# dflemin3/approxposterior

Hardware: AMD Instinct MI355X
Metric: GP-predict+acquisition candidates/sec (N_train, D fixed) (higher is better)
Workload: dtype f64

## Files before the change

### approxposterior_amd/_lib.py

```python
import ctypes
import os

_HERE = os.path.dirname(os.path.abspath(__file__))
LIB_PATH = os.path.join(_HERE, "csrc", "libapgp.so")
ABI_VERSION = 8
MAX_DIM = 32
MAX_FANTASY = 32
MAX_DRAWS = 32
MAX_FEATURES = 65536
MAX_REFS = 4096
INTEGRATED_MAX_DIM = 16

UTIL_AGP, UTIL_BAPE, UTIL_JONES, UTIL_NONE = 0, 1, 2, 3
UTIL_NEG_MEAN = 4
NM_MAX_RESTARTS = 4096
NM_MAX_FEV = 1 << 20
NM_STEPS = {1: "reflect", 2: "expand", 3: "reflect_exp", 4: "contract_out", 5: "contract_in",
            6: "shrink_out", 7: "shrink_in", 8: "maxfev"}
GMM_EM, GMM_SCORE, GMM_KMEANS = 0, 1, 2
GMM_MAX_COMP = 16
IMP_BLOCK = 256
IMP_MAX_BLOCKS = 2048


class ApgpError(RuntimeError):
    pass


class KernelStruct(ctypes.Structure):
    _fields_ = [("ndim", ctypes.c_int32), ("lin_order", ctypes.c_int32),
                ("amp", ctypes.c_double), ("diag_add", ctypes.c_double),
                ("inv_metric", ctypes.c_double * MAX_DIM), ("lin_coef", ctypes.c_double)]


class BestStruct(ctypes.Structure):
    _fields_ = [("u", ctypes.c_double), ("index", ctypes.c_int64)]


class NmOptions(ctypes.Structure):
    _fields_ = [("kind", ctypes.c_int32), ("maxiter", ctypes.c_int32), ("maxfev", ctypes.c_int32),
                ("reserved", ctypes.c_int32), ("zeta", ctypes.c_double), ("ybest", ctypes.c_double),
                ("xatol", ctypes.c_double), ("fatol", ctypes.c_double), ("rho", ctypes.c_double),
                ("chi", ctypes.c_double), ("psi", ctypes.c_double), ("sigma", ctypes.c_double)]


class EnsMove(ctypes.Structure):
    _fields_ = [("kind", ctypes.c_int32), ("weight", ctypes.c_double), ("p0", ctypes.c_double), ("p1", ctypes.c_double)]


ENS_MOVE_STRETCH, ENS_MOVE_DE, ENS_MOVE_SNOOKER = 0, 1, 2
ENS_MAX_MOVES = 8
PT_MAX_TEMPS = 64
HMC_MAX_LEAP = 1024
HMC_G_ROWS = (1, 4)
NESTED_MAX_LIVE = 4096
NESTED_MAX_BATCH = 16


class HmcOptions(ctypes.Structure):
    _fields_ = [("eps", ctypes.c_double), ("jitter", ctypes.c_double), ("nleap", ctypes.c_int32),
                ("g_rows", ctypes.c_int32), ("iteration0", ctypes.c_int64), ("mass", ctypes.c_double * MAX_DIM)]

_P = ctypes.c_void_p
_I64 = ctypes.c_int64
_I32 = ctypes.c_int32
_F64 = ctypes.c_double
_KP = ctypes.POINTER(KernelStruct)

SIGNATURES = {
    "apgp_abi_version": (ctypes.c_int, []),
    "apgp_last_error": (ctypes.c_char_p, []),
    "apgp_npad": (_I64, [_I64]),
    "apgp_packed_linv_len": (_I64, [_I64]),
    "apgp_acquire_work_len": (_I64, [_I64, _I64]),
    "apgp_packed_train_len": (_I64, [_I64, _I32]),
    "apgp_trtri_work_len": (_I64, [_I64]),
    "apgp_grad_work_len": (_I64, [_I64]),
    "apgp_gram": (ctypes.c_int, [_P, _I64, _KP, _P, _I64, _P]),
    "apgp_kernel_cross": (ctypes.c_int, [_P, _I64, _P, _I64, _KP, _P, _I64, _P]),
    "apgp_potrf": (ctypes.c_int, [_P, _I64, _I64, _P, _F64, _P, _P, _P]),
    "apgp_logdet": (ctypes.c_int, [_P, _I64, _I64, _P, _P]),
    "apgp_fit_summary": (ctypes.c_int, [_P, _I64, _I64, _P, _P, _P, _P]),
    "apgp_nll_eval": (ctypes.c_int, [_P, _I64, _KP, _P, _F64, _P, _P, _P, _P, _P, _P]),
    "apgp_potrf_mode": (ctypes.c_int, [ctypes.c_int]),
    "apgp_potrf_fallbacks": (_I64, []),
    "apgp_potrf_backoff_skips": (_I64, []),
    "apgp_nll_side_batches": (_I64, []),
    "apgp_nll_eval_batch": (ctypes.c_int, [_P, _I64, _I64, _P, _P, _P, _P, _P, _P, _P, _P, _P]),
    "apgp_trsv": (ctypes.c_int, [_P, _I64, _I64, _P, _F64, ctypes.c_int, _P, _P, _P]),
    "apgp_trsv_ex": (ctypes.c_int, [_P, _I64, _I64, _P, _F64, ctypes.c_int, _P, _P, ctypes.c_int, _P]),
    "apgp_trsv_mode": (ctypes.c_int, [ctypes.c_int]),
    "apgp_append_diag": (ctypes.c_int, [_P, _P, _F64, _P, _I64, _P]),
    "apgp_winv_apply_work_len": (_I64, [_I64]),
    "apgp_winv_apply": (ctypes.c_int, [_P, _I64, _I64, _P, _F64, ctypes.c_int, _P, _P, _P, _P]),
    "apgp_trtri_pack": (ctypes.c_int, [_P, _I64, _I64, _P, _P, _P, _P]),
    "apgp_pack_train": (ctypes.c_int, [_P, _P, _I64, _KP, _P, _P]),
    "apgp_acquire": (ctypes.c_int, [_P, _I64, _I64, _P, _P, _I64, _KP, _F64, _I32,
                                    ctypes.POINTER(_F64), ctypes.POINTER(_F64), _P,
                                    _F64, _F64, _P, _P, _P, _P, _P, _P]),
    "apgp_packed_lsolve_len": (_I64, [_I64]),
    "apgp_pack_lsolve": (ctypes.c_int, [_P, _I64, _I64, _P, _P]),
    "apgp_acquire_solve": (ctypes.c_int, [_P, _I64, _I64, _P, _P, _I64, _KP, _F64, _I32,
                                          ctypes.POINTER(_F64), ctypes.POINTER(_F64), _P,
                                          _F64, _F64, _P, _P, _P, _P, _P, _P]),
    "apgp_set_sweep_prune": (ctypes.c_int, [ctypes.c_int]),
    "apgp_get_sweep_prune": (ctypes.c_int, []),
    "apgp_set_seed_rowsplit": (ctypes.c_int, [ctypes.c_int]),
    "apgp_get_seed_rowsplit": (ctypes.c_int, []),
    "apgp_set_seed_park": (ctypes.c_int, [ctypes.c_int]),
    "apgp_get_seed_park": (ctypes.c_int, []),
    "apgp_set_seed_first": (ctypes.c_int, [ctypes.c_int]),
    "apgp_get_seed_first": (ctypes.c_int, []),
    "apgp_set_seed_parts": (ctypes.c_int, [ctypes.c_int]),
    "apgp_get_seed_parts": (ctypes.c_int, []),
    "apgp_sweep_prune_counts_offset": (_I64, [_I64, _I64]),
    "apgp_sweep_prune_select": (ctypes.c_int, [_P, _I64, _P, _P, _F64, _P, _P]),
    "apgp_prune_bounds": (ctypes.c_int, [_P, _I64, _P, _I64, _KP, _F64, _I32, ctypes.POINTER(_F64), ctypes.POINTER(_F64),
                                         _P, _F64, _F64, ctypes.c_int, _P, _P]),
    "apgp_sweep_prune_seeds": (ctypes.c_int, [_P, _I64, _P, _P, _P]),
    "apgp_prune_rows_len": (_I64, [_I64, _I32]),
    "apgp_pack_prune_rows": (ctypes.c_int, [_P, _I64, _KP, _P, _P]),
    "apgp_acquire_rows": (ctypes.c_int, [_P, _I64, _I64, _P, _P, _I64, _KP, _F64, _I32,
                                         ctypes.POINTER(_F64), ctypes.POINTER(_F64), _P,
                                         _F64, _F64, _P, _P, _P, _P, _P, _P, _P]),
    "apgp_acquire_solve_rows": (ctypes.c_int, [_P, _I64, _I64, _P, _P, _I64, _KP, _F64, _I32,
                                               ctypes.POINTER(_F64), ctypes.POINTER(_F64), _P,
                                               _F64, _F64, _P, _P, _P, _P, _P, _P, _P]),
    "apgp_prune_bounds_rows": (ctypes.c_int, [_P, _I64, _P, _I64, _KP, _F64, _I32, ctypes.POINTER(_F64),
                                              ctypes.POINTER(_F64), _P, _F64, _F64, ctypes.c_int, _P, _P, _P]),
    "apgp_acquire_fantasy_work_len": (_I64, [_I64]),
    "apgp_acquire_fantasy": (ctypes.c_int, [_P, _I64, _I64, _P, _I64, _KP, _P, _I64, _I32, _P, _I64,
                                            _P, _P, _P, _I32, ctypes.POINTER(_F64), ctypes.POINTER(_F64), _P,
                                            _F64, _F64, _P, _P, _P, _P]),
    "apgp_path_draws_work_len": (_I64, [_I64, _I32]),
    "apgp_path_draws_mode": (ctypes.c_int, [ctypes.c_int]),
    "apgp_path_draws": (ctypes.c_int, [_P, _I64, _I64, _P, _I64, _KP, _F64, _P, _P, _P, _P, _P, _I32, _I32,
                                       ctypes.POINTER(_F64), ctypes.POINTER(_F64), _P, _P, _P, _P, _P]),
    "apgp_integrated_work_len": (_I64, [_I64, _I32]),
    "apgp_integrated_mode": (ctypes.c_int, [ctypes.c_int]),
    "apgp_acquire_integrated": (ctypes.c_int, [_P, _I64, _I64, _P, _I64, _KP, _P, _I32, _P, _P, _P,
                                               ctypes.POINTER(_F64), ctypes.POINTER(_F64), _P, _P, _I64, _P, _P, _P, _P]),
    "apgp_predict1_work_len": (_I64, [_I64]),
    "apgp_predict1_host": (ctypes.c_int, [_P, _P, _I64, _KP, _F64, _P, _I64, _P, _I64, _P, _P, _P]),
    "apgp_nm_search_work_len": (_I64, [_I64, _I64]),
    "apgp_nm_search": (ctypes.c_int, [_P, _I64, _P, _I64, _KP, _F64, _P, _I64, _P, _I64,
                                      ctypes.POINTER(_F64), ctypes.POINTER(_F64), ctypes.POINTER(NmOptions),
                                      _P, _P, _P, _P, _P, _P, _P]),
    "apgp_predict_grad_work_len": (_I64, [_I64, _I64]),
    "apgp_predict_grad": (ctypes.c_int, [_P, _I64, _P, _I64, _KP, _F64, _P, _I64, _P, _I64, _I32,
                                         ctypes.POINTER(_F64), ctypes.POINTER(_F64), _F64, _F64,
                                         _P, _P, _P, _P, _P, _P, _P, _P]),
    "apgp_predict_mean": (ctypes.c_int, [_P, _I64, _P, _I64, _KP, _F64, _P, _P]),
    "apgp_predict_mean_host": (ctypes.c_int, [_P, _I64, _P, _I64, _KP, _F64, _P, _P, _P]),
    "apgp_ensemble_sample": (ctypes.c_int, [_P, _I64, _KP, _F64, ctypes.POINTER(_F64), ctypes.POINTER(_F64),
                                            _I32, _I32, _I64, _F64, ctypes.c_uint64, _P, _P, _P, _P, _P, _P]),
    "apgp_ensemble_sample_ex": (ctypes.c_int, [_P, _I64, _KP, _F64, ctypes.POINTER(_F64), ctypes.POINTER(_F64),
                                               _I32, _I32, _I64, _F64, ctypes.c_uint64, _P, _P, _P, _P, _P, ctypes.c_int, _P]),
    "apgp_ensemble_sample_moves": (ctypes.c_int, [_P, _I64, _KP, _F64, ctypes.POINTER(_F64), ctypes.POINTER(_F64),
                                                  _I32, _I32, _I64, _F64, ctypes.c_uint64, _P, _P, _P, _P, _P, ctypes.c_int,
                                                  ctypes.POINTER(EnsMove), _I32, _P]),
    "apgp_ensemble_mode": (ctypes.c_int, [ctypes.c_int]),
    "apgp_tempered_work_len": (_I64, [_I32, _I32, _I32, _I32]),
    "apgp_tempered_sample": (ctypes.c_int, [_P, _I64, _KP, _F64, ctypes.POINTER(_F64), ctypes.POINTER(_F64), _I32, _I32, _I32,
                                            ctypes.POINTER(_F64), _I64, _I64, ctypes.c_uint64, _P, _P, _P, _I32, _P, _P, _P,
                                            _P, _P, ctypes.POINTER(EnsMove), _I32, _P, _P]),
    "apgp_hmc_sample": (ctypes.c_int, [_P, _I64, _KP, _F64, ctypes.POINTER(_F64), ctypes.POINTER(_F64), _I32, _I64,
                                       ctypes.POINTER(HmcOptions), ctypes.c_uint64, _P, _P, _P, _P, _P, _P, _P, _P, _P, _P, _P]),
    "apgp_hmc_rule": (ctypes.c_int, [_I32, _I64, _I32]),
    "apgp_nested_work_len": (_I64, [_I32, _I32, _I32]),
    "apgp_nested_xlds": (ctypes.c_int, [_I64, _I32]),
    "apgp_nested_sample": (ctypes.c_int, [_P, _I64, _KP, _F64, ctypes.POINTER(_F64), ctypes.POINTER(_F64), _I32, _I32, _I32,
                                          _I32, _F64, _F64, _F64, _I32, ctypes.c_uint64, _P, _P, _P, _P, _P, _P, _P, _P, _P]),
    "apgp_box_candidates": (ctypes.c_int, [_P, _I64, _I32, ctypes.POINTER(_F64), ctypes.POINTER(_F64), ctypes.c_uint64,
                                           _I64, _P]),
    "apgp_prior_candidates": (ctypes.c_int, [_P, _I64, _I32, _P, _P, _P, ctypes.c_uint64, _I64, _P]),
    "apgp_prior_lnprior": (ctypes.c_int, [_P, _I64, _I32, _P, _P, _P, _P, _P]),
    "apgp_release_scratch": (ctypes.c_int, [_P]),
    "apgp_kinv_solve_work_len": (_I64, [_I64]),
    "apgp_kinv_solve": (ctypes.c_int, [_P, _I64, _I64, _P, _P, _P]),
    "apgp_grad_loglik": (ctypes.c_int, [_P, _P, _P, _I64, _I64, _KP, _P, _P, _P]),
    "apgp_gmm_params_len": (_I64, [_I32, _I32]),
    "apgp_gmm_stats_len": (_I64, [_I32, _I32]),
    "apgp_gmm_pass": (ctypes.c_int, [_P, _I64, _I32, _I32, _P, _I32, _P, _P, _P, _P]),
    "apgp_mix_params_len": (_I64, [_I32, _I32]),
    "apgp_mix_candidates": (ctypes.c_int, [_P, _P, _I64, _I32, _I32, _P, ctypes.c_uint64, _I64, _P]),
    "apgp_sobol_direction": (_I32, [_I32, _I32]),
    "apgp_sobol_box_candidates": (ctypes.c_int, [_P, _I64, _I32, ctypes.POINTER(_F64), ctypes.POINTER(_F64), ctypes.c_uint64,
                                                 _I32, _I32, _I64, _P]),
    "apgp_sobol_prior_candidates": (ctypes.c_int, [_P, _I64, _I32, _P, _P, _P, ctypes.c_uint64, _I32, _I32, _I64, _P]),
    "apgp_sobol_mix_candidates": (ctypes.c_int, [_P, _P, _I64, _I32, _I32, _P, ctypes.c_uint64, _I32, _I32, _I64, _P]),
    "apgp_importance_stats_len": (_I64, [_I32]),
    "apgp_importance_work_len": (_I64, [_I64]),
    "apgp_importance_pass": (ctypes.c_int, [_P, _I64, _P, _P, _I64, _KP, _F64, ctypes.POINTER(_F64), ctypes.POINTER(_F64),
                                            _P, _P, _P, _P, _P]),
    "apgp_path_importance_work_len": (_I64, [_I64, _I32]),
    "apgp_path_importance": (ctypes.c_int, [_P, _I64, _P, _P, _I64, _KP, _F64, _P, _P, _P, _P, _P, _I32, _I32,
                                            ctypes.POINTER(_F64), ctypes.POINTER(_F64), _P, _P, _P, _P, _P]),
    "apgp_autocorr_work_len": (_I64, [_I64, _I64, _I32]),
    "apgp_autocorr_block": (ctypes.c_int, [_P, _I64, _I64, _I32, _I64, _I64, _I64, _I64, _I32, _P, _P, _P]),
}

_lib = None


def load():
    global _lib
    if _lib is not None:
        return _lib
    if not os.path.exists(LIB_PATH):
        raise ApgpError(
            "libapgp.so not found at %s -- build it with "
            "`make -C approxposterior_amd/csrc` (or __graft_entry__.build()). "
            "There is no CPU fallback." % LIB_PATH)
    import torch
    lib = ctypes.CDLL(LIB_PATH)
    for name, (res, args) in SIGNATURES.items():
        fn = getattr(lib, name)
        fn.restype = res
        fn.argtypes = args
    v = lib.apgp_abi_version()
    if v != ABI_VERSION:
        raise ApgpError("libapgp.so ABI %d != expected %d" % (v, ABI_VERSION))
    _lib = lib
    return lib


def check(status, what):
    if status != 0:
        msg = load().apgp_last_error()
        raise ApgpError("%s failed (%d): %s" % (what, status, msg.decode() if msg else ""))
```

### approxposterior_amd/csrc/prune_mm32.h

```cpp
#pragma once
#include <utility>

#ifndef PMM_G
#define PMM_G 4
#endif
#define PMM_ROWS 128
typedef float f32x16 __attribute__((ext_vector_type(16)));
typedef __bf16 bf16x8 __attribute__((ext_vector_type(8)));

struct PmmSlot { int e, pp, qp; };

template <int DPAD>
struct PmmShape {
    static constexpr int K = DPAD + 2;
    static constexpr int NS = 5 * DPAD + 4;
    static constexpr int NIS = (NS + 15) / 16, NI = NIS + 1;
    static constexpr int PITCH = 16 * NI + 8;
    static_assert(K <= 16, "the big products stand in one instruction");
    static constexpr int XPIECES = PMM_ROWS * PITCH / 8, APIECES = PMM_ROWS / 4, PIECES = XPIECES + APIECES;
    static constexpr PmmSlot slot(int i) {
        if (i >= 16 * NIS) return i - 16 * NIS < K ? PmmSlot{i - 16 * NIS, 0, 0} : PmmSlot{-1, 0, 0};
        if (i < 2 * DPAD) return PmmSlot{2 + i / 2, (i & 1) ? 2 : 0, (i & 1) ? 0 : 2};
        i -= 2 * DPAD;
        if (i < 2) return i == 0 ? PmmSlot{0, 2, 0} : PmmSlot{1, 0, 2};
        i -= 2;
        if (i < DPAD) return PmmSlot{2 + i, 1, 1};
        i -= DPAD;
        if (i < 2 * DPAD) return PmmSlot{2 + i / 2, (i & 1) ? 1 : 0, (i & 1) ? 0 : 1};
        i -= 2 * DPAD;
        if (i < 2) return i == 0 ? PmmSlot{0, 1, 0} : PmmSlot{1, 0, 1};
        return PmmSlot{-1, 0, 0};
    }
};

template <int PART>
__device__ __forceinline__ float pmm_part(float p) {
    const float h = (float)(__bf16)p;
    if constexpr (PART == 0) return h;
    const float r = p - h, m = (float)(__bf16)r;
    return PART == 1 ? m : r - m;
}

template <int DPAD, int SIDE, int I>
__device__ __forceinline__ __bf16 pmm_slot_value(const float (&entry)[DPAD + 2]) {
    constexpr PmmSlot s = PmmShape<DPAD>::slot(I);
    if constexpr (s.e < 0) return (__bf16)0.0f;
    else return (__bf16)pmm_part<SIDE ? s.qp : s.pp>(entry[s.e]);
}
template <int DPAD, int SIDE, int F, int... J>
__device__ __forceinline__ bf16x8 pmm_frag(const float (&entry)[DPAD + 2], std::integer_sequence<int, J...>) {
    return bf16x8{pmm_slot_value<DPAD, SIDE, 8 * F + J>(entry)...};
}
template <int DPAD, int... F>
__device__ __forceinline__ void pmm_store_row(__bf16* dst, const float (&entry)[DPAD + 2],
                                              std::integer_sequence<int, F...>) {
    ((*(bf16x8*)(dst + 8 * F) = pmm_frag<DPAD, 0, F>(entry, std::make_integer_sequence<int, 8>{})), ...);
}
template <int DPAD, int... T>
__device__ __forceinline__ void pmm_cand(bf16x8 (&qop)[PmmShape<DPAD>::NI], const float (&entry)[DPAD + 2], int h,
                                         std::integer_sequence<int, T...>) {
    ((qop[T] = h ? pmm_frag<DPAD, 1, 2 * T + 1>(entry, std::make_integer_sequence<int, 8>{})
                 : pmm_frag<DPAD, 1, 2 * T>(entry, std::make_integer_sequence<int, 8>{})), ...);
}

template <int DPAD>
__global__ __launch_bounds__(PR_THREADS) void pmm_pack_rows_kernel(const double* xs, long long n, unsigned char* rows) {
    using SH = PmmShape<DPAD>;
    constexpr int XS = DPAD + 2, PITCH = SH::PITCH;
    const double kappa = PR32_KAPPA;
    __shared__ double wmax[PR_THREADS / 64], wsal[PR_THREADS / 64];
    const int tid = threadIdx.x, lane = tid & 63, w = tid >> 6, h = lane >> 5, l32 = lane & 31;
    double cen[DPAD];
#pragma unroll
    for (int d = 0; d < DPAD; ++d) cen[d] = xs[d];
    double sal = 0.0, bm2 = 0.0;
    const long long ntile = (n + PMM_ROWS - 1) / PMM_ROWS;
    const int srow = w * 32 + l32;
    if (h == 0) {
        for (long long ti = 0; ti < ntile; ++ti) {
            const f64x2* src = (const f64x2*)(xs + (ti * PMM_ROWS + srow) * XS);
            f64x2 pre[XS / 2];
#pragma unroll
            for (int i = 0; i < XS / 2; ++i) pre[i] = src[i];
            const bool in = ti * PMM_ROWS + srow < n;
            unsigned char* tile = rows + 16 + ti * (16ll * SH::PIECES);
            __bf16* xrow = (__bf16*)tile + srow * PITCH;
            float pe[DPAD + 2];
            double n2 = 0.0, b2 = 0.0;
#pragma unroll
            for (int d = 0; d < DPAD; ++d) {
                const double x = (d & 1) ? pre[d >> 1].y : pre[d >> 1].x;
                const double df = x - cen[d];
                b2 = fma(df, df, b2);
                const float bf = in ? (float)(df * kappa) : 0.0f;
                n2 = fma((double)bf, (double)bf, n2);
                pe[d + 2] = 2.0f * bf;
            }
            if (in) { bm2 = fmax(bm2, b2); sal += fabs(pre[DPAD / 2].x); }
            pe[0] = -(float)n2;
            pe[1] = 1.0f;
            pmm_store_row<DPAD>(xrow, pe, std::make_integer_sequence<int, 2 * SH::NI>{});
            ((float*)(tile + 16 * SH::XPIECES))[srow] = in ? (float)pre[DPAD / 2].x : 0.0f;
            *(bf16x8*)(xrow + 16 * SH::NI) = bf16x8{(__bf16)0.0f, (__bf16)0.0f, (__bf16)0.0f, (__bf16)0.0f,
                                                    (__bf16)0.0f, (__bf16)0.0f, (__bf16)0.0f, (__bf16)0.0f};
        }
    }
    for (int o = 32; o > 0; o >>= 1) { bm2 = fmax(bm2, __shfl_xor(bm2, o)); sal += __shfl_xor(sal, o); }
    if (lane == 0) { wmax[w] = bm2; wsal[w] = sal; }
    __syncthreads();
    if (tid == 0) {
        sal = 0.0;
#pragma unroll
        for (int i = 0; i < PR_THREADS / 64; ++i) { bm2 = fmax(bm2, wmax[i]); sal += wsal[i]; }
        ((double*)rows)[0] = bm2;
        ((double*)rows)[1] = sal;
    }
}

template <int DPAD, bool PRE = false>
__global__ __launch_bounds__(PR_THREADS, PMM_G <= 4 ? 2 : 1) void prune_bound_mm32_kernel(PruneArgs a) {
    using SH = PmmShape<DPAD>;
    constexpr int XS = DPAD + 2;
    constexpr int K = SH::K, NI = SH::NI, PITCH = SH::PITCH, G = PMM_G;
    static_assert(PMM_G % 2 == 0 && PMM_ROWS == 32 * (PR_THREADS / 64), "one 32-row tile staged per wavefront");
    const double kappa = PR32_KAPPA;
    static_assert(SH::XPIECES * 8 == PMM_ROWS * PITCH && SH::APIECES * 4 == PMM_ROWS, "the stream's tile is the LDS image");
    constexpr int NB = PRE ? 2 : 1;
    __shared__ __attribute__((aligned(16))) __bf16 xt[NB * PMM_ROWS * PITCH];
    __shared__ __attribute__((aligned(16))) float at[NB * PMM_ROWS];
    __shared__ double wmax[PR_THREADS / 64], wsal[PR_THREADS / 64];
    const int tid = threadIdx.x, lane = tid & 63, w = tid >> 6, h = lane >> 5, l32 = lane & 31;
    const long long blk0 = ((long long)blockIdx.x * (PR_THREADS / 64) + w) * (G / 2);
    double cen[DPAD], c2 = 0.0;
#pragma unroll
    for (int d = 0; d < DPAD; ++d) { cen[d] = a.xs[d]; c2 = fma(cen[d], cen[d], c2); }
    const double cn = sqrt(c2);
    bf16x8 qop[G][NI];
    double an[G];
    bool adm[G];
#pragma unroll
    for (int g = 0; g < G; ++g) {
        const long long blk = blk0 + (g >> 1);
        const long long row = blk * SW_CAND + (g & 1) * 32 + l32;
        const bool live = blk < a.ncb && row < a.m;
        bool ok = live, has_nan = false;
        double a2 = 0.0, ce[DPAD];
#pragma unroll
        for (int d = 0; d < DPAD; ++d) {
            double v = 0.0;
            if (live && d < a.ndim) {
                v = a.T[row * a.ndim + d];
                if (a.has_box && !(v >= a.lo[d] && v <= a.hi[d])) ok = false;
                if (v != v) has_nan = true;
            }
            ce[d] = v * a.sc[d] - cen[d];
            a2 = fma(ce[d], ce[d], a2);
        }
        if (live && a.mask && a.mask[row] == 0) ok = false;
        adm[g] = ok && !has_nan;
        an[g] = sqrt(a2);
        const bool use = live && !has_nan && a2 <= 0x1p100;
        float q[K];
        double n2 = 0.0;
#pragma unroll
        for (int d = 0; d < DPAD; ++d) {
            q[d + 2] = use ? (float)(ce[d] * kappa) : 0.0f;
            n2 = fma((double)q[d + 2], (double)q[d + 2], n2);
        }
        q[0] = 1.0f;
        q[1] = -(float)n2;
        pmm_cand<DPAD>(qop[g], q, h, std::make_integer_sequence<int, NI>{});
    }
    double accm[G], accs[G], sal = 0.0, bm2 = 0.0;
#pragma unroll
    for (int g = 0; g < G; ++g) { accm[g] = 0.0; accs[g] = 0.0; }
    const long long ntile = (a.n + PMM_ROWS - 1) / PMM_ROWS;
    auto consume = [&](int xo, int ao) {
#pragma unroll 1
        for (int rt = 0; rt < PMM_ROWS / 32; ++rt) {
            const __bf16* xr = xt + xo + (rt * 32 + l32) * PITCH + 8 * h;
            bf16x8 pop[NI];
#pragma unroll
            for (int t = 0; t < NI; ++t) pop[t] = *(const bf16x8*)(xr + 16 * t);
            float al[16];
#pragma unroll
            for (int q = 0; q < 4; ++q) *(f32x4*)(al + 4 * q) = *(const f32x4*)(at + ao + rt * 32 + 8 * q + 4 * h);
            auto product = [&](int g) {
                f32x16 c = {0.0f, 0.0f, 0.0f, 0.0f, 0.0f, 0.0f, 0.0f, 0.0f, 0.0f, 0.0f, 0.0f, 0.0f, 0.0f, 0.0f, 0.0f, 0.0f};
#pragma unroll
                for (int t = 0; t < NI; ++t) c = __builtin_amdgcn_mfma_f32_32x32x16_bf16(pop[t], qop[g][t], c, 0, 0, 0);
                return c;
            };
            f32x16 cur = product(0);
#pragma unroll
            for (int g = 0; g < G; ++g) {
                f32x16 nxt = cur;
                if (g + 1 < G) nxt = product(g + 1);
                float ps = 0.0f, pS = 0.0f;
#pragma unroll
                for (int r = 0; r < 16; ++r) {
                    const float k = __builtin_amdgcn_exp2f(cur[r]);
                    ps = fmaf(k, al[r], ps);
                    pS = fmaf(k, fabsf(al[r]), pS);
                }
                accm[g] += (double)ps;
                accs[g] += (double)pS;
                cur = nxt;
            }
        }
    };
    if constexpr (PRE) {
        typedef unsigned int u32x4 __attribute__((ext_vector_type(4)));
        constexpr int NPC = SH::PIECES, NL = (NPC + PR_THREADS - 1) / PR_THREADS;
        const u32x4* img = (const u32x4*)((const unsigned char*)a.prune_rows + 16);
        u32x4 pre[NL];
        auto fetch = [&](long long ti) {
            const u32x4* src = img + ti * NPC;
#pragma unroll
            for (int j = 0; j < NL; ++j) {
                const int e = tid + j * PR_THREADS;
                pre[j] = src[e < NPC ? e : NPC - 1];
            }
        };
        auto put = [&](int b) {
            u32x4* xd = (u32x4*)(xt + b * PMM_ROWS * PITCH);
            u32x4* ad = (u32x4*)(at + b * PMM_ROWS);
#pragma unroll
            for (int j = 0; j < NL; ++j) {
                const int e = tid + j * PR_THREADS;
                if ((j + 1) * PR_THREADS <= SH::XPIECES || e < SH::XPIECES) xd[e] = pre[j];
                else if (e < NPC) ad[e - SH::XPIECES] = pre[j];
            }
        };
        fetch(0);
        put(0);
        __syncthreads();
        for (long long ti = 0; ti < ntile; ++ti) {
            const int b = (int)(ti & 1);
            fetch(ti + 1 < ntile ? ti + 1 : ntile - 1);
            consume(b * PMM_ROWS * PITCH, b * PMM_ROWS);
            put(b ^ 1);
            __syncthreads();
        }
        bm2 = ((const double*)a.prune_rows)[0];
        sal = ((const double*)a.prune_rows)[1];
    } else {
        const bool stager = h == 0;
        const int srow = w * 32 + l32;
        f64x2 pre[XS / 2];
        auto fetch = [&](long long ti) {
            const f64x2* src = (const f64x2*)(a.xs + (ti * PMM_ROWS + srow) * XS);
#pragma unroll
            for (int i = 0; i < XS / 2; ++i) pre[i] = stager ? src[i] : f64x2{0.0, 0.0};
        };
        fetch(0);
        for (long long ti = 0; ti < ntile; ++ti) {
            if (stager) {
                const bool in = ti * PMM_ROWS + srow < a.n;
                float pe[K];
                double n2 = 0.0, b2 = 0.0;
#pragma unroll
                for (int d = 0; d < DPAD; ++d) {
                    const double x = (d & 1) ? pre[d >> 1].y : pre[d >> 1].x;
                    const double df = x - cen[d];
                    b2 = fma(df, df, b2);
                    const float bf = in ? (float)(df * kappa) : 0.0f;
                    n2 = fma((double)bf, (double)bf, n2);
                    pe[d + 2] = 2.0f * bf;
                }
                if (in) { bm2 = fmax(bm2, b2); sal += fabs(pre[DPAD / 2].x); }
                pe[0] = -(float)n2;
                pe[1] = 1.0f;
                pmm_store_row<DPAD>(xt + srow * PITCH, pe, std::make_integer_sequence<int, 2 * NI>{});
                at[srow] = in ? (float)pre[DPAD / 2].x : 0.0f;
            }
            __syncthreads();
            if (ti + 1 < ntile) fetch(ti + 1);
            consume(0, 0);
            __syncthreads();
        }
        for (int o = 32; o > 0; o >>= 1) { bm2 = fmax(bm2, __shfl_xor(bm2, o)); sal += __shfl_xor(sal, o); }
        if (lane == 0) { wmax[w] = bm2; wsal[w] = sal; }
        __syncthreads();
        sal = 0.0;
#pragma unroll
        for (int i = 0; i < PR_THREADS / 64; ++i) { bm2 = fmax(bm2, wmax[i]); sal += wsal[i]; }
    }
    const double bn = sqrt(bm2);
    const double u32 = 0x1p-24, eps = 0x1p-53;
    const double sa = sal * (1.0 + 0x1p-16);
    double bb = INFINITY, bbe = INFINITY;
#pragma unroll
    for (int g = 0; g < G; ++g) {
        const double sm = accm[g] + __shfl_xor(accm[g], 32);
        const double s32 = (accs[g] + __shfl_xor(accs[g], 32)) * (1.0 + 0x1p-16);
        const double ktt = a.amp;
        const double mu = fma(a.amp, sm, a.mean);
        double b = util_value(a.kind, mu, ktt, a.zeta, a.ybest);
        const double ab = an[g] + bn;
        const double eta = (DPAD + 10.0) * u32 * ab * ab + 2.5 * eps * ab * (cn + an[g]) + 24.0 * u32;
        double e32 = a.amp * (expm1(eta) * (1.0 + 0x1p-20) * s32 + 0x1p-120 * (sa + (double)a.n));
        if (!(eta <= 0x1p-8)) e32 = INFINITY;
        bbe = fmin(bbe, pr_block_min<32>(b, adm[g]));
        bb = fmin(bb, pr_block_min<32>(b - pr_slack<DPAD>(a, 2.0 * e32, a.amp * sa, mu, ktt, b), adm[g]));
        if (g & 1) {
            const long long blk = blk0 + (g >> 1);
            if (lane == 0 && blk < a.ncb) pr_store_block<true>(a, blk, bb, bbe);
            bb = INFINITY; bbe = INFINITY;
        }
    }
}
```

### approxposterior_amd/csrc/sweep.hip

```cpp
#include "apgp_common.h"
#include "mma16.h"
#include "scratch.h"
#include "util_value.h"
#include <mutex>
#include <stdlib.h>
#include <string.h>

#define SW_ROWS APGP_ROW_BLOCK
#define SW_KC APGP_K_CHUNK
#define SW_TILE (SW_ROWS * SW_KC)
#define SW_CAND 64
#define SW_GRID 256
#define SW_BCH 1024
typedef unsigned int u32x4 __attribute__((ext_vector_type(4)));
#ifndef SW_KAUX
#define SW_KAUX 0
#endif

struct SweepArgs {
    const double* T;
    const double* linv;
    const double* xs;
    const unsigned char* mask;
    double* mu;
// ... 1001 lines not shown
        qr[1] = fma(v0.y, v0.y, qr[1]);
        qr[2] = fma(v1.x, v1.x, qr[2]);
        qr[3] = fma(v1.y, v1.y, qr[3]);
    }
    double qtot = 0.0;
    qtot += s2_q_gather(qr, lane);
    if ((lane >> 4) == 0) a.sp_q[((long long)pos * SW_CAND + w * 16 + (lane & 15)) * a.nrb + jb] = qtot;
}

#define SP_NCH 4
template <int DPAD>
__global__ __launch_bounds__(256) void seed_park_kernel(SweepArgs a) {
#pragma clang fp contract(off)
    constexpr int XS = DPAD + 2;
    constexpr int NKK = SW_KC / 4;
    __shared__ double Etab[APGP_EXP_TAB_N];
    const int ngrp = a.ncache / SP_NCH;
    const int pos = S2W_P0(a.split) + (int)blockIdx.x / ngrp, kc0 = (int)blockIdx.x % ngrp * SP_NCH;
    const long long cnt = *a.blk_count;
    if (cnt <= a.list_lo || cnt > a.list_hi || pos >= cnt) return;
    if (s2_wave_skip(a, a.nrb, S2W_P0(a.split), pos)) return;
    apgp_exp_tab_load(Etab);
    __syncthreads();
    const int ht = threadIdx.x, lane = ht & 63, hw = ht >> 6;
    const int cl = lane & 15, kq = lane >> 4;
    const long long blk = a.blk_list[pos];
    const long long crow = blk * SW_CAND + hw * 16 + cl;
    const bool inb = blk < a.blk_end && crow < a.m;
    double tv[DPAD], tt[DPAD];
#pragma unroll
    for (int d = 0; d < DPAD; ++d) {
        double v = 0.0;
        if (inb && d < a.ndim) v = a.T[crow * a.ndim + d];
        tv[d] = v;
        tt[d] = v * a.sc[d];
    }
    for (int kc = kc0; kc < kc0 + SP_NCH; ++kc) {
        const double* Xb = a.xs + (long long)kc * (SW_KC * XS);
        double s2[NKK], s3[NKK];
#pragma unroll
        for (int kk = 0; kk < NKK; ++kk) { s2[kk] = 0.0; s3[kk] = 0.0; }
#pragma unroll
        for (int d = 0; d < DPAD; d += 2)
#pragma unroll
            for (int kk = 0; kk < NKK; ++kk) {
                const f64x2 xa = *(const f64x2*)(Xb + (kk * 4 + kq) * XS + d);
                double df0, df1;
                if (kc == 0) { df0 = fma(tv[d], a.sc[d], -xa.x); df1 = fma(tv[d + 1], a.sc[d + 1], -xa.y); }
                else { df0 = tt[d] - xa.x; df1 = tt[d + 1] - xa.y; }
                s2[kk] = fma(df0, df0, s2[kk]);
                s3[kk] = fma(df1, df1, s3[kk]);
            }
        double ex[NKK], bfv[NKK];
#pragma unroll
        for (int kk = 0; kk < NKK; ++kk) ex[kk] = -(s2[kk] + s3[kk]);
        apgp_exp4(ex, bfv, Etab);
#pragma unroll
        for (int kk = 0; kk < NKK; ++kk) bfv[kk] = bfv[kk] * a.amp;
        f64x2* dst = (f64x2*)(a.kcache + ((long long)pos * a.ncache + kc) * SW_BCH) + ht;
        f64x2 q0, q1;
        q0.x = bfv[0]; q0.y = bfv[1]; q1.x = bfv[2]; q1.y = bfv[3];
        dst[0] = q0; dst[256] = q1;
    }
}


static inline int s2_nrb(int64_t n) { return (int)((n + S2_ROWS - 1) / S2_ROWS); }
static inline long long s2_ncache(int64_t n) { return (long long)S2_CPB * (s2_nrb(n) - 1); }

template <int DPAD>
static constexpr size_t s2_lds_bytes() {
    return (3 * S2_TILE + 2 * 4 * 256 + 3 * ((SW_KC * (DPAD + 2) * 8 + 1023) / 1024 * 128) + APGP_EXP_TAB_N + SW_CAND + 8 +
            4 * APGP_MAX_DIM) * sizeof(double);
}

template <int DPAD>
static int s2_prepare_device() {
    static ApgpLdsOnce once;
    int dev = 0;
    if (hipGetDevice(&dev) != hipSuccess || dev < 0 || dev >= 64) {
        apgp_set_error("apgp_acquire: hipGetDevice failed");
        return -2;
    }
    return apgp_raise_lds(once, "apgp_acquire", dev, (int)s2_lds_bytes<DPAD>(),
                          {(const void*)sweep2_kernel<DPAD, false, 0>, (const void*)sweep2_kernel<DPAD, true, 0>,
                           (const void*)sweep2_kernel<DPAD, false, 1>, (const void*)sweep2_kernel<DPAD, true, 1>,
                           (const void*)sweep2_kernel<DPAD, false, 2>, (const void*)sweep2_kernel<DPAD, true, 2>,
                           (const void*)sweep2_kernel<DPAD, false, 0, true>, (const void*)sweep2_kernel<DPAD, true, 0, true>,
                           (const void*)sweep2_kernel<DPAD, false, 1, true>, (const void*)sweep2_kernel<DPAD, true, 1, true>,
                           (const void*)sweep2_kernel<DPAD, false, 2, true>, (const void*)sweep2_kernel<DPAD, true, 2, true>,
                           (const void*)sweep2_kernel<DPAD, false, 0, true, true>, (const void*)sweep2_kernel<DPAD, true, 0, true, true>});
}

template <int DPAD, bool LIST>
static void s2_launch(const SweepArgs& a, hipStream_t s, bool solve, unsigned grid) {
    const size_t lds = s2_lds_bytes<DPAD>();
    if (solve && a.nrb <= S2_STATIC_DIAG_NRB) {
        if (a.lin_coef != 0.0)
            hipLaunchKernelGGL((sweep2_kernel<DPAD, true, 2, LIST>), dim3(grid), dim3(S2_THREADS), lds, s, a);
        else
            hipLaunchKernelGGL((sweep2_kernel<DPAD, false, 2, LIST>), dim3(grid), dim3(S2_THREADS), lds, s, a);
    } else if (solve) {
        if (a.lin_coef != 0.0)
            hipLaunchKernelGGL((sweep2_kernel<DPAD, true, 1, LIST>), dim3(grid), dim3(S2_THREADS), lds, s, a);
        else
            hipLaunchKernelGGL((sweep2_kernel<DPAD, false, 1, LIST>), dim3(grid), dim3(S2_THREADS), lds, s, a);
    } else if (a.lin_coef != 0.0)
        hipLaunchKernelGGL((sweep2_kernel<DPAD, true, 0, LIST>), dim3(grid), dim3(S2_THREADS), lds, s, a);
    else
        hipLaunchKernelGGL((sweep2_kernel<DPAD, false, 0, LIST>), dim3(grid), dim3(S2_THREADS), lds, s, a);
}

template <int DPAD>
static int launch_sweep(const SweepArgs& a0, hipStream_t s, bool solve) {
    const int rc = s2_prepare_device<DPAD>();
    if (rc != 0) return rc;
    SweepArgs a = a0;
    const long long ncb = (a.m + SW_CAND - 1) / SW_CAND;
    const int nrb2 = s2_nrb(a.n);
    a.nrb = nrb2;
    long long rest = ncb % SW_GRID;
    if (solve || nrb2 < 2 || rest > S2_SPLIT_MAX || a.sp_q == NULL) rest = 0;
    const long long full = ncb - rest;
    if (full > 0) {
        a.blk_begin = 0; a.blk_end = full; a.split = 0;
        s2_launch<DPAD, false>(a, s, solve, (unsigned)(full < SW_GRID ? full : SW_GRID));
    }
    if (rest > 0) {
        a.blk_begin = full; a.blk_end = ncb; a.split = 1;
        a.ncache = 0;
        a.kslot_bytes = SW_BCH * 8;
        s2_launch<DPAD, false>(a, s, solve, (unsigned)(rest * nrb2));
        hipLaunchKernelGGL(sweep_finish_kernel, dim3((unsigned)rest), dim3(64), 0, s, a);
    }
    return 0;
}

static int g_seed_rowsplit = -1;

extern "C" int apgp_set_seed_rowsplit(int v) {
    return __atomic_exchange_n(&g_seed_rowsplit, v < 0 ? -1 : v, __ATOMIC_RELAXED);
}

extern "C" int apgp_get_seed_rowsplit(void) { return __atomic_load_n(&g_seed_rowsplit, __ATOMIC_RELAXED); }

static int g_seed_park = 1;

extern "C" int apgp_set_seed_park(int v) { return __atomic_exchange_n(&g_seed_park, v != 0 ? 1 : 0, __ATOMIC_RELAXED); }

extern "C" int apgp_get_seed_park(void) { return __atomic_load_n(&g_seed_park, __ATOMIC_RELAXED); }

#define S2_SEED_FIRST 4
static int g_seed_first = -1;

extern "C" int apgp_set_seed_first(int v) {
    return __atomic_exchange_n(&g_seed_first, v < 1 ? -1 : (v > 16 ? 16 : v), __ATOMIC_RELAXED);
}

extern "C" int apgp_get_seed_first(void) { return __atomic_load_n(&g_seed_first, __ATOMIC_RELAXED); }

static int g_seed_parts = -1;

extern "C" int apgp_set_seed_parts(int v) {
    return __atomic_exchange_n(&g_seed_parts, (v == 8 || v == 4 || v == 2 || v == 1) ? v : -1, __ATOMIC_RELAXED);
}

extern "C" int apgp_get_seed_parts(void) { return __atomic_load_n(&g_seed_parts, __ATOMIC_RELAXED); }

static long long seed_launch_cost(int nrb, int cap, int n, int j0, int lg, bool parked) {
    static const int gen[4] = {S2P_WHOLE_GEN, S2P_HALF_GEN, S2P_PAIR2_GEN, S2P_PAIR1_GEN};
    static const int park[4] = {S2P_WHOLE_PARK, S2P_HALF_PARK, S2P_PAIR2_PARK, S2P_PAIR1_PARK};
    long long load[SW_GRID] = {0};
    const int nitem = s2_nitems(nrb, j0, n, lg);
    long long last = 0;
    for (int i = 0; i < nitem; ++i) {
        int jb = 0, h = -1;
        s2_row_item(i, nrb, j0, n, lg, jb, h);
        const int kind = h >= 0 ? lg : (n - S2_ROWS * jb <= S2_ROWS / 2 ? 1 : 0);
        const int nkc = s2_nkc_of(jb, n), nre = S2_CPB * jb < nkc ? S2_CPB * jb : nkc;
        const long long c = parked ? (long long)gen[kind] * (nkc - nre) + (long long)park[kind] * nre
                                   : (long long)s2_part_cost(kind) * nkc;
        for (int k = 0; k < cap; ++k) {
            int best = 0;
            for (int q = 1; q < SW_GRID; ++q)
                if (load[q] < load[best]) best = q;
            load[best] += c;
            if (load[best] > last) last = load[best];
        }
    }
    return last;
}

struct SeedPlan { int j0, lg; long long cost; };
static SeedPlan seed_plan(int nrb, int cap, int n, bool parked) {
    const int v = apgp_get_seed_rowsplit(), fp = apgp_get_seed_parts();
    const int flg = fp == 8 ? 0 : fp == 4 ? 1 : fp == 2 ? 2 : fp == 1 ? 3 : -1;
    struct Memo { int nrb, cap, n, parked, v, flg; SeedPlan plan; };
    static std::mutex mu;
    static Memo memo[8];
    static int nmemo = 0, next = 0;
    std::lock_guard<std::mutex> g(mu);
    for (int i = 0; i < nmemo; ++i) {
        const Memo& e = memo[i];
        if (e.nrb == nrb && e.cap == cap && e.n == n && e.parked == (int)parked && e.v == v && e.flg == flg) return e.plan;
    }
    SeedPlan best = {nrb, 1, 0};
    long long best_c = -1;
    for (int lg = 1; lg <= (parked ? 2 : 1); ++lg) {
        if (flg >= 0 && lg != 1) continue;
        const int l = flg >= 0 ? flg : lg;
        for (int j0 : {nrb, nrb / 2, 0}) {
            if (v >= 0 && j0 != nrb) continue;
            const int j = v >= 0 ? (v < nrb ? v : nrb) : j0;
            if (lg > 1 && j == nrb) continue;
            const long long c = seed_launch_cost(nrb, cap, n, j, l, parked);
            if (best_c < 0 || c < best_c) { best = {j, l, c}; best_c = c; }
        }
    }
    memo[next] = {nrb, cap, n, (int)parked, v, flg, best};
    next = (next + 1) % 8;
    if (nmemo < 8) ++nmemo;
    return best;
}

template <int DPAD>
static void launch_sweep_list(const SweepArgs& a0, hipStream_t s, bool solve, const long long* list,
                              const long long* count, long long max_count, long long cap, bool rowsplit = false) {
    SweepArgs a = a0;
    const int nrb2 = s2_nrb(a.n);
    a.nrb = nrb2;
    a.blk_list = list; a.blk_count = count;
    a.blk_begin = 0; a.blk_end = (a.m + SW_CAND - 1) / SW_CAND;
    const bool can_split = !solve && nrb2 >= 2 && a.sp_q != NULL;
    if (cap > max_count) cap = max_count;
    if (can_split) {
        SweepArgs b = a;
        b.split = 1; b.ncache = 0; b.kslot_bytes = SW_BCH * 8;
        b.list_lo = 0; b.list_hi = cap;
        const bool parked = rowsplit && b.lin_coef == 0.0 && apgp_get_seed_park() != 0;
        int first = (int)cap;
        if (rowsplit && b.lin_coef == 0.0) {
            const int v = apgp_get_seed_first();
            first = v > 0 ? v : S2_SEED_FIRST;
            if (first > (int)cap) first = (int)cap;
            if (v <= 0 && first < (int)cap &&
                seed_plan(nrb2, (int)cap, b.n, true).cost - seed_plan(nrb2, first, b.n, true).cost <= S2P_WAVE2)
                first = (int)cap;
        }
        for (int wave = 0; wave < (first < (int)cap ? 2 : 1); ++wave) {
            const int p0 = wave ? first : 0, p1 = wave ? (int)cap : first, nw = p1 - p0;
            const SeedPlan plan = rowsplit ? seed_plan(nrb2, nw, b.n, parked) : SeedPlan{nrb2, 0, 0};
            const int nitem = s2_nitems(nrb2, plan.j0, b.n, plan.lg);
            b.split = S2W_WORD(plan.j0, plan.lg, p0, p1);
            if (parked) {
                b.ncache = (int)s2_ncache(b.n);
                b.kslot_bytes = (unsigned)(b.ncache * (SW_BCH * 8));
                hipLaunchKernelGGL(seed_park_kernel<DPAD>, dim3((unsigned)(nw * (b.ncache / SP_NCH))), dim3(256), 0, s, b);
            }
            if (nitem > nrb2 || parked || first < (int)cap) {
                const size_t lds = s2_lds_bytes<DPAD>();
                const unsigned grid = (unsigned)(nw * nitem);
                if (b.lin_coef != 0.0)
                    hipLaunchKernelGGL((sweep2_kernel<DPAD, true, 0, true, true>), dim3(grid), dim3(S2_THREADS), lds, s, b);
                else
                    hipLaunchKernelGGL((sweep2_kernel<DPAD, false, 0, true, true>), dim3(grid), dim3(S2_THREADS), lds, s, b);
                if (nitem > nrb2) hipLaunchKernelGGL(sweep_fold_kernel, dim3((unsigned)(nw * nrb2)), dim3(256), 0, s, b);
            } else {
                b.split = 1;
                s2_launch<DPAD, true>(b, s, solve, (unsigned)(cap * nrb2));
            }
            SweepArgs f = b;
            f.split = rowsplit ? (S2W_WORD(plan.j0, plan.lg, p0, p1) | S2W_SEED) : 1;
            hipLaunchKernelGGL(sweep_finish_kernel, dim3((unsigned)nw), dim3(64), 0, s, f);
        }
    }
    if (!can_split || max_count > cap) {
        a.split = 0;
        a.list_lo = can_split ? cap : 0; a.list_hi = APGP_MAX_M;
        s2_launch<DPAD, true>(a, s, solve, (unsigned)(max_count < SW_GRID ? max_count : SW_GRID));
    }
}

#define PR_THREADS 256
#define PR_CPT 2
#define PR_ROWS 128
#define PR_SEED 16
static inline int64_t pr_min_m(int64_t n) { return n >= 4096 ? 16384 : 65536; }

struct PruneArgs {
    const double* T;
    const double* xs;
    const unsigned char* mask;
    double* bmin;
    double* part_u;
    long long* part_i;
    long long m, ncb, n;
    int ndim, kind, has_box, lin_order;
    double mean, amp, lin_coef, zeta, ybest;
    double sc[APGP_MAX_DIM], lw[APGP_MAX_DIM], lo[APGP_MAX_DIM], hi[APGP_MAX_DIM];
    const long long* blk_list;
    const long long* blk_count;
    double* est;
    const void* prune_rows;
};

template <int DPAD>
__device__ __forceinline__ double pr_slack(const PruneArgs& a, double base, double S, double mu, double ktt, double b) {
    const double eps = 0x1p-53;
    double slack = base + 2.0 * (4.0 * (double)(a.n + 16) + 8.0 * DPAD + 32.0) * eps * S +
                   64.0 * eps * (1.0 + fabs(mu) + fabs(a.ybest) + fabs(a.zeta) + ktt + fabs(b));
    if (a.kind == APGP_UTIL_BAPE) slack += 16.0 * eps / (1.0 - exp(0.0 - ktt));
    return slack;
}

template <int W>
__device__ __forceinline__ double pr_block_min(double b, bool adm) {
    if (!(b == b)) b = -INFINITY;
    if (!adm) b = INFINITY;
    for (int o = W / 2; o > 0; o >>= 1) b = fmin(b, __shfl_xor(b, o));
    return b;
}

__device__ __forceinline__ void pr_prefill(const PruneArgs& a, long long blk) {
    if (a.part_u) {
        a.part_u[blk] = INFINITY;
        a.part_i[blk] = -1;
    }
}

template <bool PREFILL>
__device__ __forceinline__ void pr_store_block(const PruneArgs& a, long long blk, double b, double be) {
    a.bmin[blk] = b;
    if (a.est) a.est[blk] = be;
    if (PREFILL) pr_prefill(a, blk);
}

template <int DPAD, bool LIST = false>
__global__ __launch_bounds__(PR_THREADS) void prune_bound_kernel(PruneArgs a) {
    constexpr int XS = DPAD + 2;
    constexpr int PIECES = PR_ROWS * XS / 2;
    __shared__ double etab[APGP_EXP_TAB_N];
    __shared__ __attribute__((aligned(16))) double tile[PR_ROWS * XS];
    long long lst_count = 0;
    if (LIST) {
        lst_count = *a.blk_count;
        if ((long long)blockIdx.x * (PR_THREADS / 64) * PR_CPT >= lst_count) return;
    }
    apgp_exp_tab_load(etab);
    const int tid = threadIdx.x, lane = tid & 63, w = tid >> 6;
    const long long blk0 = ((long long)blockIdx.x * (PR_THREADS / 64) + w) * PR_CPT;
    long long blk[PR_CPT];
#pragma unroll
    for (int c = 0; c < PR_CPT; ++c) blk[c] = !LIST ? blk0 + c : (blk0 + c < lst_count ? a.blk_list[blk0 + c] : a.ncb);
    double tt[PR_CPT][DPAD], ktt[PR_CPT];
    bool adm[PR_CPT];
#pragma unroll
    for (int c = 0; c < PR_CPT; ++c) {
        const long long row = blk[c] * SW_CAND + lane;
        const bool live = blk[c] < a.ncb && row < a.m;
        bool ok = live, has_nan = false;
        double ktl = a.lin_order == 0 ? (double)a.ndim : 0.0;
#pragma unroll
        for (int d = 0; d < DPAD; ++d) {
            double v = 0.0;
            if (live && d < a.ndim) {
                v = a.T[row * a.ndim + d];
                if (a.has_box && !(v >= a.lo[d] && v <= a.hi[d])) ok = false;
                if (v != v) has_nan = true;
            }
            tt[c][d] = v * a.sc[d];
            if (a.lin_coef != 0.0 && a.lin_order > 0) {
                const double p = v * v;
                double q = p;
                for (int e = 1; e < a.lin_order; ++e) q *= p;
                ktl += q;
            }
        }
        if (live && a.mask && a.mask[row] == 0) ok = false;
        adm[c] = ok && !has_nan;
        ktt[c] = a.lin_coef != 0.0 ? fma(a.lin_coef, ktl, a.amp) : a.amp;
    }
    double acc[PR_CPT][4], sab[PR_CPT][4];
#pragma unroll
    for (int c = 0; c < PR_CPT; ++c)
#pragma unroll
        for (int q = 0; q < 4; ++q) { acc[c][q] = 0.0; sab[c][q] = 0.0; }
    const long long ntile = (a.n + PR_ROWS - 1) / PR_ROWS;
    for (long long ti = 0; ti < ntile; ++ti) {
        __syncthreads();
        const double* src = a.xs + ti * (PR_ROWS * XS);
        for (int e = tid; e < PIECES; e += PR_THREADS) *((f64x2*)tile + e) = *((const f64x2*)src + e);
        __syncthreads();
        for (int r = 0; r < PR_ROWS; r += 4) {
#pragma unroll
            for (int c = 0; c < PR_CPT; ++c) {
                double ex[4], kv[4];
#pragma unroll
                for (int q = 0; q < 4; ++q) {
                    const double* xr = tile + (r + q) * XS;
                    double s2 = 0.0, s3 = 0.0;
#pragma unroll
                    for (int d = 0; d < DPAD; d += 2) {
                        const double df0 = tt[c][d] - xr[d];
                        const double df1 = tt[c][d + 1] - xr[d + 1];
                        s2 = fma(df0, df0, s2);
                        s3 = fma(df1, df1, s3);
                    }
                    ex[q] = -(s2 + s3);
                }
                apgp_exp4(ex, kv, etab);
#pragma unroll
                for (int q = 0; q < 4; ++q) {
                    const double* xr = tile + (r + q) * XS;
                    double k = kv[q] * a.amp, kabs = k;
                    if (a.lin_coef != 0.0) {
                        double ls = a.lin_order == 0 ? (double)a.ndim : 0.0, la = ls;
                        if (a.lin_order > 0)
#pragma unroll
                            for (int d = 0; d < DPAD; d += 2) {
                                const double p0 = tt[c][d] * xr[d] * a.lw[d], p1 = tt[c][d + 1] * xr[d + 1] * a.lw[d + 1];
                                double q0 = p0, q1 = p1;
                                for (int e = 1; e < a.lin_order; ++e) { q0 *= p0; q1 *= p1; }
                                ls += q0 + q1;
                                la += fabs(q0) + fabs(q1);
                            }
                        kabs = fma(a.lin_coef, la, k);
                        k = fma(a.lin_coef, ls, k);
                    }
                    acc[c][q] = fma(k, xr[DPAD], acc[c][q]);
                    sab[c][q] = fma(kabs, fabs(xr[DPAD]), sab[c][q]);
                }
            }
        }
    }
#pragma unroll
    for (int c = 0; c < PR_CPT; ++c) {
        const double mu = ((acc[c][0] + acc[c][1]) + (acc[c][2] + acc[c][3])) + a.mean;
        const double S = (sab[c][0] + sab[c][1]) + (sab[c][2] + sab[c][3]);
        double b = util_value(a.kind, mu, ktt[c], a.zeta, a.ybest);
        const double eps = 0x1p-53;
        double slack = 2.0 * (4.0 * (double)(a.n + 16) + 8.0 * DPAD + 32.0) * eps * S +
                       64.0 * eps * (1.0 + fabs(mu) + fabs(a.ybest) + fabs(a.zeta) + ktt[c] + fabs(b));
        if (a.kind == APGP_UTIL_BAPE) slack += 16.0 * eps / (1.0 - exp(0.0 - ktt[c]));
        b -= slack;
        b = pr_block_min<64>(b, adm[c]);
        if (lane == 0 && blk[c] < a.ncb) {
            if (LIST) {
                a.bmin[blk[c]] = fmax(a.bmin[blk[c]], b);
            } else {
                a.bmin[blk[c]] = b;
                if (a.part_u) {
                    a.part_u[blk[c]] = INFINITY;
                    a.part_i[blk[c]] = -1;
                }
            }
        }
    }
}

#define PR32_CPT 4
#define PR32_ROWS 128
#define PR32_FLUSH 8
typedef float f32x2 __attribute__((ext_vector_type(2)));
typedef float f32x4 __attribute__((ext_vector_type(4)));
static constexpr double PR32_KAPPA = 0x1.337cc2183b050p+0;
static constexpr int pr32_cpt(int dpad) { return dpad <= 8 ? PR32_CPT : dpad == 16 ? 2 : 1; }

template <int DPAD, bool REDO = false>
__global__ __launch_bounds__(PR_THREADS) void prune_bound32_kernel(PruneArgs a) {
    constexpr int XS = DPAD + 2;
    constexpr int PIECES = PR32_ROWS * XS / 2;
    constexpr int NP = (PIECES + PR_THREADS - 1) / PR_THREADS;
    constexpr int HD = DPAD / 2;
    constexpr int CPT = pr32_cpt(DPAD);
    if (REDO) {
        const long long wg0 = (long long)blockIdx.x * (PR_THREADS / 64) * CPT;
        bool any = false;
        for (int i = 0; i < (PR_THREADS / 64) * CPT; ++i) any |= wg0 + i < a.ncb && a.bmin[wg0 + i] == -INFINITY;
        if (!any) return;
    }
    const double kappa = PR32_KAPPA;
    __shared__ __attribute__((aligned(16))) float xt[PR32_ROWS * DPAD];
    __shared__ __attribute__((aligned(16))) float at[PR32_ROWS];
    __shared__ double cen[DPAD];
    const int tid = threadIdx.x, lane = tid & 63, w = tid >> 6;
    if (tid < DPAD) cen[tid] = a.xs[tid];
    const long long blk0 = ((long long)blockIdx.x * (PR_THREADS / 64) + w) * CPT;
    f32x2 tt[CPT][HD];
    double ktt[CPT], an[CPT];
    bool adm[CPT], redo[CPT];
#pragma unroll
    for (int c = 0; c < CPT; ++c) {
        const long long row = (blk0 + c) * SW_CAND + lane;
        const bool live = blk0 + c < a.ncb && row < a.m;
        redo[c] = !REDO || (blk0 + c < a.ncb && a.bmin[blk0 + c] == -INFINITY);
        bool ok = live, has_nan = false;
        double a2 = 0.0;
#pragma unroll
        for (int d = 0; d < DPAD; ++d) {
            double v = 0.0;
            if (live && d < a.ndim) {
                v = a.T[row * a.ndim + d];
                if (a.has_box && !(v >= a.lo[d] && v <= a.hi[d])) ok = false;
                if (v != v) has_nan = true;
            }
            const double ce = v * a.sc[d] - a.xs[d];
            a2 = fma(ce, ce, a2);
            tt[c][d >> 1][d & 1] = (float)(ce * kappa);
        }
        if (live && a.mask && a.mask[row] == 0) ok = false;
        adm[c] = ok && !has_nan;
        ktt[c] = a.amp;
        an[c] = sqrt(a2);
    }
    double acc[CPT], sal = 0.0, c2 = 0.0;
#pragma unroll
    for (int c = 0; c < CPT; ++c) acc[c] = 0.0;
#pragma unroll
    for (int d = 0; d < DPAD; ++d) c2 = fma(a.xs[d], a.xs[d], c2);
    const double cn = sqrt(c2);
    const long long ntile = (a.n + PR32_ROWS - 1) / PR32_ROWS;
    f64x2 pre[NP];
    auto fetch = [&](long long ti) {
        const f64x2* src = (const f64x2*)(a.xs + ti * (PR32_ROWS * XS));
#pragma unroll
        for (int i = 0; i < NP; ++i) {
            const int e = tid + i * PR_THREADS;
            pre[i] = e < PIECES ? src[e] : f64x2{0.0, 0.0};
        }
    };
    fetch(0);
    __syncthreads();
    for (long long ti = 0; ti < ntile; ++ti) {
#pragma unroll
        for (int i = 0; i < NP; ++i) {
            const int e = tid + i * PR_THREADS;
            if (e < PIECES) {
                const int r = (2 * e) / XS, col = (2 * e) % XS;
                if (col < DPAD)
                    *(f32x2*)(xt + r * DPAD + col) = f32x2{(float)((pre[i].x - cen[col]) * kappa),
                                                           (float)((pre[i].y - cen[col + 1]) * kappa)};
                else
                    at[r] = (float)pre[i].x;
            }
        }
        __syncthreads();
        if (ti + 1 < ntile) fetch(ti + 1);
        for (int r0 = 0; r0 < PR32_ROWS; r0 += PR32_FLUSH) {
            float al[PR32_FLUSH], ps[CPT], pa = 0.0f;
#pragma unroll
            for (int q = 0; q < PR32_FLUSH; q += 4) *(f32x4*)(al + q) = *(const f32x4*)(at + r0 + q);
#pragma unroll
            for (int c = 0; c < CPT; ++c) ps[c] = 0.0f;
#pragma unroll
            for (int q = 0; q < PR32_FLUSH; ++q) {
                f32x2 xr[HD];
                if constexpr (DPAD >= 4) {
#pragma unroll
                    for (int h = 0; h < HD; h += 2) {
                        const f32x4 v = *(const f32x4*)(xt + (r0 + q) * DPAD + 2 * h);
                        xr[h] = f32x2{v.x, v.y};
                        xr[h + 1] = f32x2{v.z, v.w};
                    }
                } else {
                    xr[0] = *(const f32x2*)(xt + (r0 + q) * DPAD);
                }
                pa += fabsf(al[q]);
#pragma unroll
                for (int c = 0; c < CPT; ++c) {
                    f32x2 s2 = f32x2{0.0f, 0.0f};
#pragma unroll
                    for (int h = 0; h < HD; ++h) {
                        const f32x2 df = tt[c][h] - xr[h];
                        s2 = __builtin_elementwise_fma(df, df, s2);
                    }
                    const float k = __builtin_amdgcn_exp2f(-(s2.x + s2.y));
                    ps[c] = fmaf(k, al[q], ps[c]);
                }
            }
#pragma unroll
            for (int c = 0; c < CPT; ++c) acc[c] += (double)ps[c];
            sal += (double)pa;
        }
        __syncthreads();
    }
    const double u32 = 0x1p-24, eps = 0x1p-53;
    const double sa = sal * (1.0 + 0x1p-16);
#pragma unroll
    for (int c = 0; c < CPT; ++c) {
        const double mu = fma(a.amp, acc[c], a.mean);
        double b = util_value(a.kind, mu, ktt[c], a.zeta, a.ybest);
        double e32 = a.amp * ((u32 * (4.0 * an[c] + 0.5 * DPAD + 18.0) + 2.0 * eps * (cn + an[c])) * sa +
                              0x1p-120 * (sa + (double)a.n));
        if (!(u32 * (8.0 * an[c] + DPAD + 8.0) + eps * (cn + an[c]) <= 0x1p-8)) e32 = INFINITY;
        const double be = pr_block_min<64>(b, adm[c]);
        b = pr_block_min<64>(b - pr_slack<DPAD>(a, 2.0 * e32, a.amp * sa, mu, ktt[c], b), adm[c]);
        if (lane == 0 && blk0 + c < a.ncb && redo[c]) pr_store_block<!REDO>(a, blk0 + c, b, be);
    }
}

#include "prune_mm32.h"

__device__ __forceinline__ bool pr_less(double v, long long i, double w, long long j) { return v < w || (v == w && i < j); }

#define PR_NONE 0x7fffffffffffffffll

template <int E>
__device__ __forceinline__ void pr_wave_select(double (&lv)[E], long long (&li)[E], double& mv, long long& mi) {
    const int lane = threadIdx.x & 63;
    mv = INFINITY; mi = PR_NONE;
    for (int r = 0; r < PR_SEED; ++r) {
        double hv = lv[0];
        long long hi = li[0];
#pragma unroll
        for (int j = 1; j < E; ++j)
            if (pr_less(lv[j], li[j], hv, hi)) { hv = lv[j]; hi = li[j]; }
        double bv = hv;
        long long bi = hi;
        for (int o = 32; o > 0; o >>= 1) {
            const double ov = __shfl_xor(bv, o);
            const long long oi = __shfl_xor(bi, o);
            if (pr_less(ov, oi, bv, bi)) { bv = ov; bi = oi; }
        }
        if (bi == PR_NONE) break;
        if (lane == r) { mv = bv; mi = bi; }
        if (hi == bi) {
#pragma unroll
            for (int j = 0; j < E; ++j)
                if (li[j] == bi) { lv[j] = INFINITY; li[j] = PR_NONE; }
        }
    }
}

#define PR_SEED_E 16
#define PR_LIST (16 * PR_SEED)

__global__ __launch_bounds__(1024) void prune_seed_kernel(const double* bmin, long long ncb, long long* seeds,
                                                          long long* counts) {
    __shared__ double sv[PR_LIST], wv[16];
    __shared__ long long si[PR_LIST], wi[16];
    __shared__ int cnt, nsel;
    const int tid = threadIdx.x, lane = tid & 63, w = tid >> 6;
    if (tid == 0) { cnt = 0; nsel = 0; }
    double tv = INFINITY;
    long long ti = PR_NONE;
    for (long long base = 0; base < ncb; base += PR_SEED_E * 1024) {
        double lv[PR_SEED_E], hv = INFINITY;
        long long hp = PR_NONE;
#pragma unroll
        for (int j = 0; j < PR_SEED_E; ++j) {
            const long long p = base + tid + 1024 * j;
            const double v = p < ncb ? bmin[p] : INFINITY;
            lv[j] = v < INFINITY ? v : INFINITY;
            if (lv[j] < hv) { hv = lv[j]; hp = p; }
        }
        for (int o = 32; o > 0; o >>= 1) {
            const double ov = __shfl_xor(hv, o);
            const long long op = __shfl_xor(hp, o);
            if (pr_less(ov, op, hv, hp)) { hv = ov; hp = op; }
        }
        __syncthreads();
        if (lane == 0) { wv[w] = hv; wi[w] = hp; }
        __syncthreads();
        double cv = wv[0];
        long long ci = wi[0];
#pragma unroll
        for (int i = 1; i < 16; ++i)
            if (pr_less(cv, ci, wv[i], wi[i])) { cv = wv[i]; ci = wi[i]; }
        if (pr_less(cv, ci, tv, ti)) { tv = cv; ti = ci; }
#pragma unroll
        for (int j = 0; j < PR_SEED_E; ++j) {
            const long long p = base + tid + 1024 * j;
            if (lv[j] < INFINITY && !pr_less(tv, ti, lv[j], p)) {
                const int slot = atomicAdd(&cnt, 1);
                if (slot < PR_LIST) { sv[slot] = lv[j]; si[slot] = p; }
            }
        }
    }
    __syncthreads();
    int n = cnt;
    if (n > PR_LIST) {
        double lv[PR_SEED_E + 1], mv = INFINITY;
        long long li[PR_SEED_E + 1], mi = PR_NONE;
        for (long long base = 0; base < ncb; base += PR_SEED_E * 1024) {
            const double qv = __shfl(mv, PR_SEED - 1);
            const long long qi = __shfl(mi, PR_SEED - 1);
            bool any = false;
#pragma unroll
            for (int j = 0; j < PR_SEED_E; ++j) {
                const long long p = base + tid + 1024 * j;
                const double v = p < ncb ? bmin[p] : INFINITY;
                const bool in = v < INFINITY && pr_less(v, p, qv, qi);
                lv[j] = in ? v : INFINITY; li[j] = in ? p : PR_NONE;
                any |= in;
            }
            if (!__any(any)) continue;
            lv[PR_SEED_E] = mv; li[PR_SEED_E] = mi;
            pr_wave_select(lv, li, mv, mi);
        }
        if (lane < PR_SEED) { sv[w * PR_SEED + lane] = mv; si[w * PR_SEED + lane] = mi; }
        n = PR_LIST;
        __syncthreads();
    }
    if (tid < n && si[tid] != PR_NONE) {
        const double v = sv[tid];
        const long long p = si[tid];
        int rank = 0;
        for (int e = 0; e < n; ++e) rank += pr_less(sv[e], si[e], v, p) ? 1 : 0;
        if (rank < PR_SEED) { seeds[rank] = p; atomicAdd(&nsel, 1); }
    }
    __syncthreads();
    if (tid == 0) { counts[0] = nsel; counts[1] = 0; counts[3] = 0; }
}

__global__ __launch_bounds__(1024) void prune_select_kernel(const double* bmin, long long ncb, const long long* seeds,
                                                            long long* counts, const double* part_u, double tau_in,
                                                            long long* list, long long* count2) {
    __shared__ long long sd[PR_SEED];
    __shared__ long long cnt[1024];
    const int t = threadIdx.x;
    const int ns = (int)counts[0];
    if (t < PR_SEED) sd[t] = t < ns ? seeds[t] : -1;
    __syncthreads();
    double tau = tau_in;
    if (part_u) {
        tau = INFINITY;
        for (int i = 0; i < ns; ++i) tau = fmin(tau, part_u[sd[i]]);
    }
    auto keep = [&](long long p) {
        const double v = bmin[p];
        if (!(v < INFINITY && v <= tau)) return false;
        for (int i = 0; i < ns; ++i)
            if (sd[i] == p) return false;
        return true;
    };
    const long long per = (ncb + 1023) / 1024;
    const long long p0 = (long long)t * per, p1 = p0 + per < ncb ? p0 + per : ncb;
    long long c = 0;
    for (long long p = p0; p < p1; ++p) c += keep(p) ? 1 : 0;
    cnt[t] = c;
    __syncthreads();
    for (int o = 1; o < 1024; o <<= 1) {
        const long long add = t >= o ? cnt[t - o] : 0;
        __syncthreads();
        cnt[t] += add;
        __syncthreads();
    }
    long long pos = cnt[t] - c;
    for (long long p = p0; p < p1; ++p)
        if (keep(p)) list[pos++] = p;
    if (t == 1023) {
        counts[1] = cnt[1023];
        counts[2] = __double_as_longlong(tau);
        if (count2) *count2 = cnt[1023];
    }
}

static int g_sweep_prune = 1;

extern "C" int apgp_set_sweep_prune(int v) {
    const int old = __atomic_exchange_n(&g_sweep_prune, v < 0 ? 0 : v, __ATOMIC_RELAXED);
    return old;
}

extern "C" int apgp_get_sweep_prune(void) { return __atomic_load_n(&g_sweep_prune, __ATOMIC_RELAXED); }

static inline long long pr_ncb(int64_t m) { return (m + SW_CAND - 1) / SW_CAND; }
static inline long long s2_work_len(int64_t m, int64_t n) {
    const long long ncb = pr_ncb(m);
    const long long slots = ncb < SW_GRID ? ncb : SW_GRID;
    return 2 * ncb + slots * s2_ncache(n) * SW_BCH + 2 * (long long)S2_SPLIT_MAX * SW_CAND * s2_nrb(n);
}

extern "C" int64_t apgp_sweep_prune_counts_offset(int64_t m, int64_t n) {
    if (m < 1 || n < 1 || m > APGP_MAX_M || n > APGP_MAX_N) return -1;
    return s2_work_len(m, n) + 2 * pr_ncb(m) + PR_SEED;
}

extern "C" int apgp_sweep_prune_select(const double* bmin, int64_t ncb, const int64_t* seeds, int64_t* counts,
                                       double tau, int64_t* list, void* stream) {
    APGP_CHECK_ARG(bmin && seeds && counts && list, "null pointer");
    APGP_CHECK_ARG(ncb >= 1 && ncb <= APGP_MAX_M / SW_CAND, "ncb >= 1 required");
    hipLaunchKernelGGL(prune_select_kernel, dim3(1), dim3(1024), 0, (hipStream_t)stream, bmin, (long long)ncb,
                       (const long long*)seeds, (long long*)counts, (const double*)NULL, tau, (long long*)list,
                       (long long*)NULL);
    APGP_CHECK_LAUNCH();
    return 0;
}

template <class Kern>
static PruneArgs pr_args(const double* T, int64_t m, const double* xs, int64_t n, const uint8_t* mask, const Kern& kern,
                         double mean, int32_t kind, const double* lo, const double* hi, double zeta, double ybest,
                         double* bmin, double* part_u, long long* part_i, const void* prune_rows) {
    PruneArgs p;
    p.T = T; p.xs = xs; p.mask = mask; p.bmin = bmin; p.part_u = part_u; p.part_i = part_i;
    p.m = m; p.ncb = pr_ncb(m); p.n = n;
    p.kind = kind; p.mean = mean; p.zeta = zeta; p.ybest = ybest;
    apgp_fill_kernel(p, kern);
    apgp_fill_box(p, p.ndim, lo, hi);
    p.blk_list = NULL; p.blk_count = NULL; p.est = NULL; p.prune_rows = prune_rows;
    return p;
}

template <int DPAD>
static void launch_bound(const PruneArgs& p, hipStream_t s, bool coarse) {
    auto grid_of = [&](int cpt) { return dim3((unsigned)((p.ncb + (PR_THREADS / 64) * cpt - 1) / ((PR_THREADS / 64) * cpt))); };
    const dim3 grid = grid_of(coarse ? pr32_cpt(DPAD) : PR_CPT);
    if (coarse) {
        if constexpr (DPAD <= 8) {
            const dim3 mm_grid = grid_of(PMM_G / 2);
            if (p.prune_rows)
                hipLaunchKernelGGL((prune_bound_mm32_kernel<DPAD, true>), mm_grid, dim3(PR_THREADS), 0, s, p);
            else
                hipLaunchKernelGGL((prune_bound_mm32_kernel<DPAD, false>), mm_grid, dim3(PR_THREADS), 0, s, p);
            hipLaunchKernelGGL((prune_bound32_kernel<DPAD, true>), grid, dim3(PR_THREADS), 0, s, p);
        } else {
            hipLaunchKernelGGL((prune_bound32_kernel<DPAD, false>), grid, dim3(PR_THREADS), 0, s, p);
        }
    } else if (p.blk_list)
        hipLaunchKernelGGL((prune_bound_kernel<DPAD, true>), grid, dim3(PR_THREADS), 0, s, p);
    else
        hipLaunchKernelGGL((prune_bound_kernel<DPAD, false>), grid, dim3(PR_THREADS), 0, s, p);
}

template <int DPAD>
static int launch_pruned(const SweepArgs& a, hipStream_t s, bool solve, void* part, const void* prune_rows) {
    const int rc = s2_prepare_device<DPAD>();
    if (rc != 0) return rc;
    const long long ncb = pr_ncb(a.m);
    double* bmin = (double*)part + s2_work_len(a.m, a.n);
    long long* list = (long long*)(bmin + ncb);
    long long* seeds = list + ncb;
    long long* counts = seeds + PR_SEED;
    const bool coarse = a.lin_coef == 0.0;
    PruneArgs p = pr_args(a.T, a.m, a.xs, a.n, a.mask, a, a.mean, a.kind, a.has_box ? a.lo : NULL, a.has_box ? a.hi : NULL,
                          a.zeta, a.ybest, bmin, a.part_u, a.part_i, prune_rows);
    if (coarse) p.est = (double*)(counts + 8);
    launch_bound<DPAD>(p, s, coarse);
    hipLaunchKernelGGL(prune_seed_kernel, dim3(1), dim3(1024), 0, s, coarse ? (const double*)p.est : (const double*)bmin, ncb,
                       seeds, counts);
    if (solve || s2_nrb(a.n) < 2 || a.sp_q == NULL) (void)hipMemsetAsync(counts + 4, 0, sizeof(long long), s);
    launch_sweep_list<DPAD>(a, s, solve, seeds, counts, ncb < PR_SEED ? ncb : PR_SEED, PR_SEED, true);
    hipLaunchKernelGGL(prune_select_kernel, dim3(1), dim3(1024), 0, s, bmin, ncb, seeds, counts, a.part_u, 0.0, list,
                       counts + 3);
    if (coarse) {
        p.blk_list = list; p.blk_count = counts + 3;
        launch_bound<DPAD>(p, s, false);
        hipLaunchKernelGGL(prune_select_kernel, dim3(1), dim3(1024), 0, s, bmin, ncb, seeds, counts, a.part_u, 0.0, list,
                           (long long*)NULL);
    }
    launch_sweep_list<DPAD>(a, s, solve, list, counts + 1, ncb, S2_SPLIT_MAX);
    return 0;
}

static_assert(S2_PRUNE_WORDS == PR_SEED + 8, "the fold inputs start behind the seed numbers and the counters");
static inline long long pr_work_len(int64_t m, int64_t n) {
    return s2_work_len(m, n) - 2ll * S2_SPLIT_MAX * SW_CAND * s2_nrb(n) + s2_fold_off(s2_nrb(n), pr_ncb(m));
}

extern "C" int64_t apgp_acquire_work_len(int64_t m, int64_t n) {
    if (m < 1 || n < 1) return 0;
    if (m > APGP_MAX_M || n > APGP_MAX_N) return -1;
    return pr_work_len(m, n) + (s2_nrb(n) >= 2 ? (long long)PR_SEED * s2_nrb(n) * (S2_HQ_PRE + S2_HQ_ACC) : 0);
}

static int acquire_impl(bool solve, const double* T, int64_t m, int64_t idx_offset, const double* packed_linv,
                        const double* xs, int64_t n, const apgp_kernel_t* kern, double mean,
                        int32_t kind, const double* lo, const double* hi, const uint8_t* mask,
                        double zeta, double ybest, double* mu, double* var, double* u, void* part,
                        apgp_best_t* best, const void* prune_rows, void* stream) {
    APGP_CHECK_ARG(T && packed_linv && xs && kern, "null pointer");
    APGP_CHECK_ARG(m >= 1 && m <= APGP_MAX_M && n >= 1 && n <= APGP_MAX_N, "m >= 1 and n >= 1 required");
    APGP_CHECK_ARG(kind >= APGP_UTIL_AGP && kind <= APGP_UTIL_NONE, "unknown utility kind");
    APGP_CHECK_ARG(kind == APGP_UTIL_NONE || best, "best required for an acquisition");
    APGP_CHECK_ARG(part || (kind == APGP_UTIL_NONE && n <= S2_ROWS),
                   "part (apgp_acquire_work_len doubles) required");
    APGP_CHECK_ARG((lo == NULL) == (hi == NULL), "lo and hi must be given together");
    KernConst kc;
    APGP_CHECK_ARG(apgp_make_kernconst(kern, &kc) == 0, "kernel parameters");
    SweepArgs a;
    a.T = T; a.linv = packed_linv; a.xs = xs; a.mask = mask;
    a.mu = mu; a.var = var; a.u = u;
    const long long nblk = (m + SW_CAND - 1) / SW_CAND;
    const long long slots = nblk < SW_GRID ? nblk : SW_GRID;
    a.part_u = (double*)part;
    a.part_i = part ? (long long*)((double*)part + nblk) : NULL;
    a.ncache = (int)s2_ncache(n);
    a.kcache = a.ncache > 0 ? (double*)part + 2 * nblk : (double*)packed_linv;
    a.sp_q = part ? (double*)part + 2 * nblk + slots * s2_ncache(n) * SW_BCH : NULL;
    a.sp_mu = a.sp_q ? a.sp_q + (long long)S2_SPLIT_MAX * SW_CAND * s2_nrb(n) : NULL;
    a.blk_begin = 0; a.blk_end = nblk; a.split = 0;
    {
        const long long wb = apgp_packed_linv_len(n) * 8, xb = apgp_packed_train_len(n, kc.ndim) * 8;
        const long long kb = (long long)(a.ncache > 0 ? a.ncache : 1) * SW_BCH * 8;
        APGP_CHECK_ARG(wb < (1ll << 31) && kb < (1ll << 31), "n too large for the sweep's 32-bit stream offsets");
        a.linv_bytes = (unsigned)wb; a.xs_bytes = (unsigned)xb; a.kslot_bytes = (unsigned)kb;
    }
    a.m = m; a.idx_offset = idx_offset;
    a.nrb = s2_nrb(n); a.kind = kind; a.n = (int)n;
    a.mean = mean; a.zeta = zeta; a.ybest = ybest;
    apgp_fill_kernel(a, kc);
    apgp_fill_box(a, kc.ndim, lo, hi);
    a.blk_list = NULL; a.blk_count = NULL; a.list_lo = 0; a.list_hi = 0;
    hipStream_t s = (hipStream_t)stream;
    const int pr_mode = apgp_get_sweep_prune();
    const bool prune = pr_mode > 0 && kind != APGP_UTIL_NONE && !mu && !var && !u && part &&
                       m >= (pr_mode == 1 ? pr_min_m(n) : (int64_t)pr_mode);
    const int rc = apgp_by_dpad(kc.dpad, [&](auto dp) {
        return prune ? launch_pruned<decltype(dp)::value>(a, s, solve, part, prune_rows)
                     : launch_sweep<decltype(dp)::value>(a, s, solve);
    });
    if (rc != 0) return rc;
    if (kind != APGP_UTIL_NONE)
        hipLaunchKernelGGL(argmin_final_kernel, dim3(1), dim3(1024), 0, s, a.part_u, a.part_i, nblk, best);
    APGP_CHECK_LAUNCH();
    return 0;
}

extern "C" int apgp_acquire(const double* T, int64_t m, int64_t idx_offset, const double* packed_linv,
                            const double* xs, int64_t n, const apgp_kernel_t* kern, double mean,
                            int32_t kind, const double* lo, const double* hi, const uint8_t* mask,
                            double zeta, double ybest, double* mu, double* var, double* u, void* part,
                            apgp_best_t* best, void* stream) {
    return acquire_impl(false, T, m, idx_offset, packed_linv, xs, n, kern, mean, kind, lo, hi, mask, zeta, ybest,
                        mu, var, u, part, best, NULL, stream);
}

extern "C" int apgp_acquire_rows(const double* T, int64_t m, int64_t idx_offset, const double* packed_linv,
                                 const double* xs, int64_t n, const apgp_kernel_t* kern, double mean,
                                 int32_t kind, const double* lo, const double* hi, const uint8_t* mask,
                                 double zeta, double ybest, double* mu, double* var, double* u, void* part,
                                 apgp_best_t* best, const void* prune_rows, void* stream) {
    return acquire_impl(false, T, m, idx_offset, packed_linv, xs, n, kern, mean, kind, lo, hi, mask, zeta, ybest,
                        mu, var, u, part, best, prune_rows, stream);
}

extern "C" int64_t apgp_prune_rows_len(int64_t n, int32_t ndim) {
    if (n < 0 || n > APGP_MAX_N || ndim < 1 || ndim > APGP_MAX_DIM) return -1;
    const int dpad = apgp_dpad(ndim);
    if (n == 0 || dpad > 8) return 0;
    const int64_t ntile = (n + PMM_ROWS - 1) / PMM_ROWS;
    return apgp_by_dpad(dpad, [&](auto dp) -> int64_t {
        if constexpr (decltype(dp)::value <= 8) return 2 + ntile * 2 * PmmShape<decltype(dp)::value>::PIECES;
        else return 0;
    });
}

extern "C" int apgp_pack_prune_rows(const double* xs, int64_t n, const apgp_kernel_t* kern, void* rows, void* stream) {
    APGP_CHECK_ARG(xs && kern && rows, "null pointer");
    APGP_CHECK_ARG(n >= 1 && n <= APGP_MAX_N, "n >= 1 required");
    KernConst kc;
    APGP_CHECK_ARG(apgp_make_kernconst(kern, &kc) == 0, "kernel parameters");
    APGP_CHECK_ARG(kc.dpad <= 8, "no pre-split rows beyond 8 dimensions (apgp_prune_rows_len is 0)");
    apgp_by_dpad(kc.dpad, [&](auto dp) {
        if constexpr (decltype(dp)::value <= 8)
            hipLaunchKernelGGL(pmm_pack_rows_kernel<decltype(dp)::value>, dim3(1), dim3(PR_THREADS), 0, (hipStream_t)stream,
                               xs, (long long)n, (unsigned char*)rows);
    });
    APGP_CHECK_LAUNCH();
    return 0;
}

static int prune_bounds_impl(const char* who, const double* T, int64_t m, const double* xs, int64_t n,
                             const apgp_kernel_t* kern, double mean, int32_t kind, const double* lo, const double* hi,
                             const uint8_t* mask, double zeta, double ybest, int coarse, double* bmin_out,
                             const void* prune_rows, void* stream) {
#define PB_CHECK_ARG(cond, msg)                                     \
    do {                                                            \
        if (!(cond)) {                                              \
            apgp_set_error("%s: bad argument: %s", who, msg);       \
            return -1;                                              \
        }                                                           \
    } while (0)
    PB_CHECK_ARG(T && xs && kern && bmin_out, "null pointer");
    PB_CHECK_ARG(m >= 1 && m <= APGP_MAX_M && n >= 1 && n <= APGP_MAX_N, "m >= 1 and n >= 1 required");
    PB_CHECK_ARG(kind >= APGP_UTIL_AGP && kind < APGP_UTIL_NONE, "unknown utility kind");
    PB_CHECK_ARG((lo == NULL) == (hi == NULL), "lo and hi must be given together");
    KernConst kc;
    PB_CHECK_ARG(apgp_make_kernconst(kern, &kc) == 0, "kernel parameters");
    PB_CHECK_ARG(!coarse || kc.lin_coef == 0.0, "the coarse bound takes pure squared-exponential kernels only");
#undef PB_CHECK_ARG
    const PruneArgs p = pr_args(T, m, xs, n, mask, kc, mean, kind, lo, hi, zeta, ybest, bmin_out, NULL, NULL, prune_rows);
    hipStream_t s = (hipStream_t)stream;
    apgp_by_dpad(kc.dpad, [&](auto dp) { launch_bound<decltype(dp)::value>(p, s, coarse != 0); });
    APGP_CHECK_LAUNCH();
    return 0;
}

extern "C" int apgp_prune_bounds(const double* T, int64_t m, const double* xs, int64_t n, const apgp_kernel_t* kern,
                                 double mean, int32_t kind, const double* lo, const double* hi, const uint8_t* mask,
                                 double zeta, double ybest, int coarse, double* bmin_out, void* stream) {
    return prune_bounds_impl(__func__, T, m, xs, n, kern, mean, kind, lo, hi, mask, zeta, ybest, coarse, bmin_out, NULL,
                             stream);
}

extern "C" int apgp_prune_bounds_rows(const double* T, int64_t m, const double* xs, int64_t n, const apgp_kernel_t* kern,
                                      double mean, int32_t kind, const double* lo, const double* hi, const uint8_t* mask,
                                      double zeta, double ybest, int coarse, double* bmin_out, const void* prune_rows,
                                      void* stream) {
    return prune_bounds_impl(__func__, T, m, xs, n, kern, mean, kind, lo, hi, mask, zeta, ybest, coarse, bmin_out,
                             prune_rows, stream);
}

extern "C" int apgp_sweep_prune_seeds(const double* bmin, int64_t ncb, int64_t* seeds, int64_t* counts, void* stream) {
    APGP_CHECK_ARG(bmin && seeds && counts, "null pointer");
    APGP_CHECK_ARG(ncb >= 1 && ncb <= APGP_MAX_M / SW_CAND, "ncb >= 1 required");
    hipLaunchKernelGGL(prune_seed_kernel, dim3(1), dim3(1024), 0, (hipStream_t)stream, bmin, (long long)ncb,
                       (long long*)seeds, (long long*)counts);
    APGP_CHECK_LAUNCH();
    return 0;
}

extern "C" int apgp_acquire_solve(const double* T, int64_t m, int64_t idx_offset, const double* packed_lsolve,
                                  const double* xs, int64_t n, const apgp_kernel_t* kern, double mean,
                                  int32_t kind, const double* lo, const double* hi, const uint8_t* mask,
                                  double zeta, double ybest, double* mu, double* var, double* u, void* part,
                                  apgp_best_t* best, void* stream) {
    return acquire_impl(true, T, m, idx_offset, packed_lsolve, xs, n, kern, mean, kind, lo, hi, mask, zeta, ybest,
                        mu, var, u, part, best, NULL, stream);
}

extern "C" int apgp_acquire_solve_rows(const double* T, int64_t m, int64_t idx_offset, const double* packed_lsolve,
                                       const double* xs, int64_t n, const apgp_kernel_t* kern, double mean,
                                       int32_t kind, const double* lo, const double* hi, const uint8_t* mask,
                                       double zeta, double ybest, double* mu, double* var, double* u, void* part,
                                       apgp_best_t* best, const void* prune_rows, void* stream) {
    return acquire_impl(true, T, m, idx_offset, packed_lsolve, xs, n, kern, mean, kind, lo, hi, mask, zeta, ybest,
                        mu, var, u, part, best, prune_rows, stream);
}

#define FT_THREADS 256
#define FT_ROWS 128

struct FantasyArgs {
    const double* T;
    const double* xs;
    const double* beta;
    double* C;
    const double* mu;
    const double* var_in;
    double* var_out;
    double* u;
    const unsigned char* mask;
    double* part_u;
    long long* part_i;
    long long m, idx_offset, ldc, pick_row, n;
    int ndim, j, kind, has_box, lin_order;
    double amp, diag_add, lin_coef, zeta, ybest;
    double sc[APGP_MAX_DIM], lw[APGP_MAX_DIM], lo[APGP_MAX_DIM], hi[APGP_MAX_DIM];
};

template <int DPAD>
__global__ __launch_bounds__(FT_THREADS) void fantasy_kernel(FantasyArgs a) {
    constexpr int XS = DPAD + 2;
    constexpr int PIECES = FT_ROWS * XS / 2;
    __shared__ double etab[APGP_EXP_TAB_N];
    __shared__ __attribute__((aligned(16))) double tile[FT_ROWS * XS];
    __shared__ double cx[APGP_MAX_FANTASY];
    __shared__ double su[FT_THREADS / 64];
    __shared__ long long si[FT_THREADS / 64];
    apgp_exp_tab_load(etab);
    const int tid = threadIdx.x;
    if (tid < a.j - 1) cx[tid] = a.C[(long long)tid * a.ldc + a.pick_row];
    const long long row = (long long)blockIdx.x * FT_THREADS + tid;
    const bool live = row < a.m;
    double tt[DPAD];
#pragma unroll
    for (int d = 0; d < DPAD; ++d) tt[d] = (live && d < a.ndim) ? a.T[row * a.ndim + d] * a.sc[d] : 0.0;
    double acc[4] = {0.0, 0.0, 0.0, 0.0};
    const long long ntile = (a.n + FT_ROWS - 1) / FT_ROWS;
    for (long long ti = 0; ti < ntile; ++ti) {
        __syncthreads();
        const long long r0 = ti * FT_ROWS;
        for (int e = tid; e < PIECES; e += FT_THREADS) {
            const int r = e / (XS / 2), p = e - r * (XS / 2);
            f64x2 v;
            if (p == DPAD / 2) {
                v.x = (r0 + r < a.n) ? a.beta[r0 + r] : 0.0;
                v.y = 0.0;
            } else {
                v = *(const f64x2*)(a.xs + (r0 + r) * XS + 2 * p);
            }
            *(f64x2*)(tile + r * XS + 2 * p) = v;
        }
        __syncthreads();
        for (int r = 0; r < FT_ROWS; r += 4) {
            double ex[4], kv[4];
#pragma unroll
            for (int q = 0; q < 4; ++q) {
                const double* xr = tile + (r + q) * XS;
                double s = 0.0, s3 = 0.0;
#pragma unroll
                for (int d = 0; d < DPAD; d += 2) {
                    const double df0 = tt[d] - xr[d];
                    const double df1 = tt[d + 1] - xr[d + 1];
                    s = fma(df0, df0, s);
                    s3 = fma(df1, df1, s3);
                }
                ex[q] = -(s + s3);
            }
            apgp_exp4(ex, kv, etab);
#pragma unroll
            for (int q = 0; q < 4; ++q) {
                const double* xr = tile + (r + q) * XS;
                double k = a.amp * kv[q];
                if (a.lin_coef != 0.0) {
                    double ls;
                    APGP_LIN_SUM(ls, DPAD, a.ndim, a.lin_order, tt[d_] * xr[d_] * a.lw[d_]);
                    k = fma(a.lin_coef, ls, k);
                }
                acc[q] = fma(k, xr[DPAD], acc[q]);
            }
        }
    }
    double bu = INFINITY;
    long long bi = -1;
    if (live) {
        double xj[DPAD];
#pragma unroll
        for (int d = 0; d < DPAD; ++d) xj[d] = d < a.ndim ? a.T[a.pick_row * a.ndim + d] * a.sc[d] : 0.0;
        double s = 0.0, s3 = 0.0;
#pragma unroll
        for (int d = 0; d < DPAD; d += 2) {
            const double df0 = tt[d] - xj[d];
            const double df1 = tt[d + 1] - xj[d + 1];
            s = fma(df0, df0, s);
            s3 = fma(df1, df1, s3);
        }
        double kx = a.amp * apgp_exp(-(s + s3), etab);
        if (a.lin_coef != 0.0) {
            double ls;
            APGP_LIN_SUM(ls, DPAD, a.ndim, a.lin_order, tt[d_] * xj[d_] * a.lw[d_]);
            kx = fma(a.lin_coef, ls, kx);
        }
        double c = kx - ((acc[0] + acc[1]) + (acc[2] + acc[3]));
        for (int i = 0; i < a.j - 1; ++i) c = fma(-a.C[(long long)i * a.ldc + row], cx[i], c);
        const double ch = c / sqrt(a.var_in[a.pick_row] + a.diag_add);
        a.C[(long long)(a.j - 1) * a.ldc + row] = ch;
        const double v = fma(-ch, ch, a.var_in[row]);
        a.var_out[row] = v;
        bool adm = !(a.mask && a.mask[row] == 0);
        if (a.has_box)
            for (int d = 0; d < a.ndim; ++d) {
                const double x = a.T[row * a.ndim + d];
                if (!(x >= a.lo[d] && x <= a.hi[d])) adm = false;
            }
#pragma unroll
        for (int d = 0; d < DPAD; ++d)
            if (tt[d] != tt[d]) adm = false;
        const double uu = adm ? util_value(a.kind, a.mu[row], v, a.zeta, a.ybest) : INFINITY;
        if (a.u) a.u[row] = uu;
        best_merge(bu, bi, uu, a.idx_offset + row);
    }
    for (int o = 32; o > 0; o >>= 1) {
        double ou = __shfl_xor(bu, o);
        long long oi = __shfl_xor(bi, o);
        best_merge(bu, bi, ou, oi);
    }
    if ((tid & 63) == 0) { su[tid >> 6] = bu; si[tid >> 6] = bi; }
    __syncthreads();
    if (tid == 0) {
        for (int w = 1; w < FT_THREADS / 64; ++w) best_merge(bu, bi, su[w], si[w]);
        a.part_u[blockIdx.x] = bu;
        a.part_i[blockIdx.x] = bi;
    }
}

extern "C" int64_t apgp_acquire_fantasy_work_len(int64_t m) {
    if (m < 1) return 0;
    if (m > APGP_MAX_M) return -1;
    return 2 * ((m + FT_THREADS - 1) / FT_THREADS);
}

extern "C" int apgp_acquire_fantasy(const double* T, int64_t m, int64_t idx_offset, const double* xs, int64_t n,
                                    const apgp_kernel_t* kern, const double* beta, int64_t pick_row, int32_t j,
                                    double* C, int64_t ldc, const double* mu, const double* var_in, double* var_out,
                                    int32_t kind, const double* lo, const double* hi, const uint8_t* mask,
                                    double zeta, double ybest, double* u, void* part, apgp_best_t* best,
                                    void* stream) {
    APGP_CHECK_ARG(T && xs && kern && beta && C && mu && var_in && var_out && part && best, "null pointer");
    APGP_CHECK_ARG(m >= 1 && m <= APGP_MAX_M && n >= 1 && n <= APGP_MAX_N, "m >= 1 and n >= 1 required");
    APGP_CHECK_ARG((m + FT_THREADS - 1) / FT_THREADS < (1ll << 31), "m too large for one grid");
    APGP_CHECK_ARG(j >= 1 && j < APGP_MAX_FANTASY, "1 <= j < APGP_MAX_FANTASY required");
    APGP_CHECK_ARG(pick_row >= 0 && pick_row < m, "0 <= pick_row < m required");
    APGP_CHECK_ARG(ldc >= m, "ldc >= m required");
    APGP_CHECK_ARG(var_in + m <= var_out || var_out + m <= var_in, "var_in and var_out must not overlap");
    APGP_CHECK_ARG(kind >= APGP_UTIL_AGP && kind <= APGP_UTIL_JONES, "kind must be AGP, BAPE or JONES");
    APGP_CHECK_ARG((lo == NULL) == (hi == NULL), "lo and hi must be given together");
    KernConst kc;
    APGP_CHECK_ARG(apgp_make_kernconst(kern, &kc) == 0, "kernel parameters");
    FantasyArgs a;
    a.T = T; a.xs = xs; a.beta = beta; a.C = C; a.mu = mu; a.var_in = var_in; a.var_out = var_out; a.u = u;
    a.mask = mask;
    const long long nblk = (m + FT_THREADS - 1) / FT_THREADS;
    a.part_u = (double*)part;
    a.part_i = (long long*)((double*)part + nblk);
    a.m = m; a.idx_offset = idx_offset; a.ldc = ldc; a.pick_row = pick_row; a.n = n;
    a.j = j; a.kind = kind; a.diag_add = kc.diag_add; a.zeta = zeta; a.ybest = ybest;
    apgp_fill_kernel(a, kc);
    apgp_fill_box(a, kc.ndim, lo, hi);
    hipStream_t s = (hipStream_t)stream;
    const dim3 grid((unsigned)nblk), block(FT_THREADS);
    apgp_by_dpad(kc.dpad, [&](auto dp) { hipLaunchKernelGGL(fantasy_kernel<decltype(dp)::value>, grid, block, 0, s, a); });
    hipLaunchKernelGGL(argmin_final_kernel, dim3(1), dim3(1024), 0, s, a.part_u, a.part_i, nblk, best);
    APGP_CHECK_LAUNCH();
    return 0;
}

__global__ __launch_bounds__(256) void pack_lsolve_kernel(const double* L, long long ldl, long long n,
                                                          double* packed) {
    constexpr int CPB = APGP_ROW_BLOCK / APGP_K_CHUNK;
    const long long tile = blockIdx.x;
    long long ib = (long long)((sqrt(8.0 * (double)tile / CPB + 1.0) - 1.0) * 0.5);
    while (CPB * (ib + 1) * (ib + 2) / 2 <= tile) ++ib;
    while (CPB * ib * (ib + 1) / 2 > tile) --ib;
    const long long kc = tile - CPB * ib * (ib + 1) / 2;
    double* out = packed + tile * (long long)(APGP_ROW_BLOCK * APGP_K_CHUNK);
    const long long sdiag = kc - ib * CPB;
    for (int e = threadIdx.x; e < APGP_ROW_BLOCK * APGP_K_CHUNK; e += 256) {
        const int s = e >> 8;
        double v = 0.0;
        if (s == sdiag) {
            const int f = e & 255, q = f >> 6, q2 = (f >> 4) & 3, i = (f >> 2) & 3, k = f & 3;
            const long long r0 = kc * APGP_K_CHUNK + 4 * q, c0 = kc * APGP_K_CHUNK + 4 * q2;
            if (q2 < q) {
                if (r0 + i < n) v = -L[(r0 + i) * ldl + c0 + k];
            } else if (q2 == q && k <= i && r0 + i < n) {
                double x[4] = {0.0, 0.0, 0.0, 0.0};
                x[k] = 1.0 / L[(r0 + k) * ldl + r0 + k];
                for (int r = k + 1; r <= i; ++r) {
                    double sacc = 0.0;
                    for (int c = k; c < r; ++c) sacc = fma(L[(r0 + r) * ldl + r0 + c], x[c], sacc);
                    x[r] = -sacc * (1.0 / L[(r0 + r) * ldl + r0 + r]);
                }
                v = x[i];
            }
        } else {
            const int q = e & 1, lane = (e >> 1) & 63, kp = (e >> 7) & 1;
            const int kk = 2 * kp + q;
            const long long row = ib * APGP_ROW_BLOCK + 16 * s + (lane & 15);
            const long long col = kc * APGP_K_CHUNK + 4 * kk + (lane >> 4);
            if (row < n && (col >> 4) < (row >> 4)) v = -L[row * ldl + col];
        }
        out[e] = v;
    }
}

extern "C" int64_t apgp_packed_lsolve_len(int64_t n) { return apgp_packed_linv_len(n); }

extern "C" int apgp_pack_lsolve(const double* L, int64_t n, int64_t ldl, double* packed, void* stream) {
    APGP_CHECK_ARG(L && packed, "null pointer");
    APGP_CHECK_ARG(n >= 1 && n <= APGP_MAX_N && ldl >= n, "n >= 1 and ldl >= n required");
    const long long nrb = apgp_npad(n) / APGP_ROW_BLOCK;
    const long long ntiles = (APGP_ROW_BLOCK / APGP_K_CHUNK) * nrb * (nrb + 1) / 2;
    hipLaunchKernelGGL(pack_lsolve_kernel, dim3((unsigned)ntiles), dim3(256), 0, (hipStream_t)stream, L,
                       (long long)ldl, (long long)n, packed);
    APGP_CHECK_LAUNCH();
    return 0;
}

struct MeanArgs {
    const double* T;
    const double* xs;
    double* mu;
    long long m, npad;
    int ndim, lin_order;
    double mean, amp, lin_coef;
    double sc[APGP_MAX_DIM], lw[APGP_MAX_DIM];
};

template <int DPAD>
__global__ __launch_bounds__(256) void predict_mean_kernel(MeanArgs a) {
    constexpr int XS = DPAD + 2;
    __shared__ double etab[APGP_EXP_TAB_N];
    apgp_exp_tab_load(etab);
    __syncthreads();
    const int lane = threadIdx.x & 63, w = threadIdx.x >> 6;
    const long long row = (long long)blockIdx.x * 4 + w;
    if (row >= a.m) return;
    double tt[DPAD];
#pragma unroll
    for (int d = 0; d < DPAD; ++d) tt[d] = d < a.ndim ? a.T[row * a.ndim + d] * a.sc[d] : 0.0;
    double acc = 0.0;
    for (long long k = lane; k < a.npad; k += 64) {
        const double* xr = a.xs + k * XS;
        double s = 0.0, s3 = 0.0;
#pragma unroll
        for (int d = 0; d < DPAD; d += 2) {
            double df0 = tt[d] - xr[d];
            double df1 = tt[d + 1] - xr[d + 1];
            s = fma(df0, df0, s);
            s3 = fma(df1, df1, s3);
        }
        double kv = a.amp * apgp_exp(-(s + s3), etab);
        if (a.lin_coef != 0.0) {
            double ls;
            APGP_LIN_SUM(ls, DPAD, a.ndim, a.lin_order, tt[d_] * xr[d_] * a.lw[d_]);
            kv = fma(a.lin_coef, ls, kv);
        }
        acc = fma(kv, xr[DPAD], acc);
    }
    for (int o = 32; o > 0; o >>= 1) acc += __shfl_xor(acc, o);
    bool bad = false;
    for (int d = 0; d < DPAD; ++d) bad = bad || (tt[d] != tt[d]);
    if (lane == 0) a.mu[row] = bad ? NAN : acc + a.mean;
}

extern "C" int apgp_predict_mean(const double* T, int64_t m, const double* xs, int64_t n,
                                 const apgp_kernel_t* kern, double mean, double* mu, void* stream) {
    APGP_CHECK_ARG(T && xs && kern && mu, "null pointer");
    APGP_CHECK_ARG(m >= 1 && m <= APGP_MAX_M && n >= 1 && n <= APGP_MAX_N, "m >= 1 and n >= 1 required");
    KernConst kc;
    APGP_CHECK_ARG(apgp_make_kernconst(kern, &kc) == 0, "kernel parameters");
    MeanArgs a;
    a.T = T; a.xs = xs; a.mu = mu; a.m = m; a.npad = apgp_npad(n); a.mean = mean;
    apgp_fill_kernel(a, kc);
    dim3 grid((unsigned)((m + 3) / 4)), block(256);
    hipStream_t s = (hipStream_t)stream;
    apgp_by_dpad(kc.dpad, [&](auto dp) { hipLaunchKernelGGL(predict_mean_kernel<decltype(dp)::value>, grid, block, 0, s, a); });
    APGP_CHECK_LAUNCH();
    return 0;
}

__global__ void mailbox_post_kernel(double* mail, long long seq) {
    __hip_atomic_store((long long*)(mail + 5), seq, __ATOMIC_RELEASE, __HIP_MEMORY_SCOPE_SYSTEM);
}

extern "C" int apgp_predict_mean_host(const double* T_host, int64_t m, const double* xs, int64_t n,
                                      const apgp_kernel_t* kern, double mean, double* mu_host,
                                      double* work, void* stream) {
    APGP_CHECK_ARG(T_host && mu_host && work && kern, "null pointer");
// ... 41 lines not shown
```

### approxposterior_amd/gp.py

```python

import collections
import ctypes
import math
from operator import is_

import numpy as np
from numpy.linalg import LinAlgError
from scipy.linalg import solve_triangular

from . import _lib
from .george_extras import GeorgeExtras

__all__ = ["GP", "ExpSquaredKernel", "ConstantKernel", "Product", "ConstantModel",
           "kernels", "UTILITY_KINDS", "sobolSample"]

UTILITY_KINDS = {"agp": _lib.UTIL_AGP, "bape": _lib.UTIL_BAPE, "jones": _lib.UTIL_JONES}
SEARCH_KINDS = dict(UTILITY_KINDS, negmean=_lib.UTIL_NEG_MEAN)
NM_OPTIONS = ("adaptive", "maxiter", "maxfev", "xatol", "fatol")


def nm_coefficients(ndim, adaptive):
    if adaptive:
        dim = float(ndim)
        return 1.0, 1 + 2 / dim, 0.75 - 1 / (2 * dim), 1 - 1 / dim
# ... 75 lines not shown
        if not hasattr(other, "is_kernel"):
            raise NotImplementedError("only kernel + kernel sums are on the MI355X hot path")
        return Sum(other, self)

    def __len__(self):
        return len(self.get_parameter_vector())


class ConstantKernel(Kernel):
    def __init__(self, log_constant, ndim=1):
        self.log_constant = float(log_constant)
        self.ndim = int(ndim)
        self.dirty = True

    def get_parameter_names(self):
        return ("log_constant",)

    def get_parameter_vector(self):
        return np.array([self.log_constant])

    def set_parameter_vector(self, v):
        self.log_constant = float(v[0])
        self.dirty = True

    def __len__(self):
        return 1


class ExpSquaredKernel(Kernel):

    def __init__(self, metric, ndim=1):
        self.ndim = int(ndim)
        metric = np.atleast_1d(np.asarray(metric, dtype=np.float64))
        if metric.size == 1 and self.ndim > 1:
            metric = np.full(self.ndim, float(metric[0]))
        if metric.size != self.ndim:
            raise ValueError("Dimension mismatch")
        self.log_M = np.log(metric)
        self.dirty = True

    def get_parameter_names(self):
        return tuple("metric:log_M_%d_%d" % (d, d) for d in range(self.ndim))

    def get_parameter_vector(self):
        return np.array(self.log_M)

    def set_parameter_vector(self, v):
        self.log_M = np.array(v, dtype=np.float64)
        self.dirty = True

    def __len__(self):
        return len(self.log_M)


class LinearKernel(Kernel):

    def __init__(self, log_gamma2=None, order=None, bounds=None, ndim=1, axes=None):
        if log_gamma2 is None or order is None:
            raise ValueError("log_gamma2 and order are required")
        if axes is not None:
            raise NotImplementedError("axes subsets are not on the MI355X hot path")
        if int(order) != order or order < 0 or order > 16:
            raise NotImplementedError("LinearKernel order must be an integer in [0, 16] on the device path")
        self.log_gamma2 = float(log_gamma2)
        self.order = int(order)
        self.ndim = int(ndim)
        self.dirty = True

    def get_parameter_names(self):
        return ("log_gamma2",)

    def get_parameter_vector(self):
        return np.array([self.log_gamma2])

    def set_parameter_vector(self, v):
        self.log_gamma2 = float(v[0])
        self.dirty = True

    def __len__(self):
        return 1


class Product(Kernel):
    def __init__(self, k1, k2):
        self.k1 = k1
        self.k2 = k2
        self.ndim = k2.ndim

    @property
    def dirty(self):
        return self.k1.dirty or self.k2.dirty

    @dirty.setter
    def dirty(self, v):
        self.k1.dirty = v
        self.k2.dirty = v

    def get_parameter_names(self):
        return tuple(["k1:" + n for n in self.k1.get_parameter_names()] +
                     ["k2:" + n for n in self.k2.get_parameter_names()])

    def get_parameter_vector(self):
        return np.concatenate([self.k1.get_parameter_vector(),
                               self.k2.get_parameter_vector()])

    def set_parameter_vector(self, v):
        n1 = len(self.k1)
        self.k1.set_parameter_vector(v[:n1])
        self.k2.set_parameter_vector(v[n1:])

    def __len__(self):
        return len(self.k1) + len(self.k2)


class Sum(Product):
    """george.kernels.Sum: same parameter protocol as Product (k1:..., k2:...)."""


class _KernelsNamespace(object):
    ExpSquaredKernel = ExpSquaredKernel
    ConstantKernel = ConstantKernel
    LinearKernel = LinearKernel
    Product = Product
    Sum = Sum


kernels = _KernelsNamespace()


def _flatten_term(kernel):
    amp, se, lin = 1.0, None, None
    stack = [kernel]
    while stack:
        k = stack.pop()
        if isinstance(k, Sum):
            raise NotImplementedError("nested kernel sums are not on the MI355X hot path")
        if isinstance(k, Product):
            stack += [k.k1, k.k2]
        elif isinstance(k, ConstantKernel):
            amp *= k.ndim * np.exp(k.log_constant)
        elif isinstance(k, ExpSquaredKernel):
            if se is not None or lin is not None:
                raise NotImplementedError("product of two non-constant kernels")
            se = k
        elif isinstance(k, LinearKernel):
            if se is not None or lin is not None:
                raise NotImplementedError("product of two non-constant kernels")
            lin = k
        else:
            raise NotImplementedError("kernel type %r is not on the MI355X hot path" % type(k))
    return float(amp), se, lin


def _flatten_kernel(kernel, with_linear=False):
    tk = type(kernel)
    if tk is ExpSquaredKernel:
        return (1.0, kernel.log_M, 0.0, 0) if with_linear else (1.0, kernel.log_M)
    if tk is Product and type(kernel.k1) is ConstantKernel and type(kernel.k2) is ExpSquaredKernel:
        amp = float(kernel.k1.ndim * np.exp(kernel.k1.log_constant))
        return (amp, kernel.k2.log_M, 0.0, 0) if with_linear else (amp, kernel.k2.log_M)
    terms = [kernel.k1, kernel.k2] if isinstance(kernel, Sum) else [kernel]
    amp = log_M = None
    lin_coef, lin_order = 0.0, 0
    for term in terms:
        c, se, lin = _flatten_term(term)
        if se is not None:
            if amp is not None:
                raise NotImplementedError("sum of two ExpSquaredKernel terms")
            amp, log_M = c, np.asarray(se.log_M, dtype=np.float64)
        elif lin is not None:
            if lin_coef != 0.0:
                raise NotImplementedError("sum of two LinearKernel terms")
            lin_coef, lin_order = c * float(np.exp(-lin.log_gamma2)), lin.order
        else:
            raise NotImplementedError("a purely constant kernel term is not on the MI355X hot path")
    if amp is None:
        raise NotImplementedError("an ExpSquaredKernel term is required")
    if with_linear:
        return amp, log_M, float(lin_coef), int(lin_order)
    return amp, log_M


class _Replay(object):
    __slots__ = ("fn", "args", "data", "device", "stream", "ybytes", "n", "deps", "current_device", "raw_stream")

    def __init__(self, fn, args, device, stream, y, deps, queries, data=None):
        self.fn, self.args, self.data = fn, args, data
        self.device, self.stream = device, stream
        self.ybytes, self.n = y.tobytes(), y.size
        self.deps = deps
        self.current_device, self.raw_stream = queries

    def fits(self, y, deps):
        if not all(map(is_, deps, self.deps)):
            return False
        if type(y) is not np.ndarray or y.dtype != _F64 or y.size != self.n or not y.flags.c_contiguous:
            return False
        cur = self.current_device()
        if cur != self.device or self.raw_stream is None or self.raw_stream(cur) != self.stream:
            return False
        return y.tobytes() == self.ybytes


def _box(bounds, D, optional=True):
    if bounds is None and optional:
        return None, None
    b = np.asarray(bounds, dtype=np.float64).reshape(-1, 2)
    if len(b) != D:
        raise ValueError("bounds must have one (lo, hi) pair per dimension")
    arr = ctypes.c_double * _lib.MAX_DIM
    return arr(*b[:, 0]), arr(*b[:, 1])


def _triu_colmajor(D):
    j = np.repeat(np.arange(D), np.arange(1, D + 1))
    i = np.concatenate([np.arange(c + 1) for c in range(D)])
    return i, j


def _seed64(seed):
    return int(seed) & 0xFFFFFFFFFFFFFFFF


def _ptr(tensor):
    return None if tensor is None else tensor.data_ptr()


def _best_record(best):
    bb = best.cpu().numpy()
    return int(bb[1:2].view(np.int64)[0]), float(bb[0])


_Swept = collections.namedtuple("_Swept", "best mu var u")

_BatchWork = collections.namedtuple("_BatchWork", "x x_d stream ybytes y_d bufs means")


def _records_nll(o, n):
    with np.errstate(all="ignore"):
        ll = (-0.5 * (n * _LOG_2PI + o[:, 0])) - 0.5 * o[:, 3]
    bad = (o[:, 4] != 0.0) | ~np.isfinite(o[:, 0]) | ~np.isfinite(ll)
    return np.where(bad, np.inf, -ll)


class PathDraws(object):

    def __init__(self, gp, Z, b, W, Wl):
        self.gp, self.Z, self.b, self.W, self.Wl, self.V = gp, Z, b, W, Wl, None
        self.size, self.nFeatures = int(W.shape[0]), int(W.shape[1])
        if Z.shape != (self.nFeatures, gp.kernel.ndim) or b.shape != (self.nFeatures,) \
                or Wl.shape != (self.size, gp.kernel.ndim):
            raise ValueError("Z (R, D), b (R,), W (S, R) and Wl (S, D) do not fit together")
        self.ks = gp._kernel_struct()
        self.mean = float(gp.mean.value)
        self._key, self._x = (gp._factor_key(), self.mean), gp._x

    def _check_current(self):
        gp = self.gp
        if not gp.computed or gp._x is not self._x or (gp._factor_key(), float(gp.mean.value)) != self._key:
            raise RuntimeError("these draws belong to a factor the GP no longer holds: call sample_paths again")

    def _call(self, t, bounds, mask, idx_offset, with_f):
        gp = self.gp
        self._check_current()
        lo, hi = _box(bounds, gp.kernel.ndim)
        T = gp._candidates(t)
        mask_d = mask if hasattr(mask, "data_ptr") else gp._mask(mask, T.shape[0])
        if mask_d is not None and (tuple(mask_d.shape) != (T.shape[0],) or str(mask_d.dtype) != "torch.uint8"):
            raise ValueError("a device mask must be a (M,) uint8 tensor")
        if T.shape[0] == 0:
            return np.empty((self.size, 0)), np.full(self.size, -1, dtype=np.int64), np.full(self.size, np.inf)
        return gp._path_call(T, self.ks, self.mean, self, self.V, lo, hi, mask_d, idx_offset, with_f)

    def evaluate(self, t):
        F = self._call(t, None, None, 0, True)[0]
        return F if isinstance(F, np.ndarray) else F.cpu().numpy()

    def argmax(self, t, bounds=None, mask=None, idx_offset=0):
        _, idx, u = self._call(t, bounds, mask, idx_offset, False)
        return idx, -u



class GP(GeorgeExtras):

    def __init__(self, kernel=None, fit_kernel=True, mean=None, fit_mean=None,
                 white_noise=None, fit_white_noise=None, solver=None, device=None,
                 **kwargs):
        if kernel is None:
            raise ValueError("a kernel is required")
        self.kernel = kernel
        self.mean = _as_model(mean, 0.0)
        self.white_noise = _as_model(white_noise, np.log(1.25e-12))
        self.fit_mean = bool(fit_mean)
        self.fit_white_noise = bool(fit_white_noise)
        self._device_arg = device
        self.variance_mode = None
        self.extend_max_rows = None
        self.sweep_prune = None
        self.seed_rowsplit = None
        self.seed_park = None
        self.seed_first = None
        self.seed_parts = None
        self.sweep_prune_stats = False
        self.last_prune_counts = None
        self._computed = False
        self._x = None
        self._yerr2 = 0.0
        self._nllMemo = None
        self._rt_cache = None
        self._queries = None
        self._x_d = None
        self._mean_work = None
        self._p1_work = None
        self._imp_work = None
        self._pimp_work = None
        self._pg_work = None
        self._nll_scratch = None
        self._nll_stream = None
        self._batch = None
        self._replays = {}
        self._reset_device_state()

    def _reset_device_state(self):
        self._L = None
        self._L_store = None
        self._ld = None
        self._nll_owned = False
        self._alpha_y = None
        self._alpha_mean = None
        self._y_d = None
        self._ztz_host = None
        self._z = None
        self._alpha = None
        self._packed = None
        self._packed_solve = None
        self._work = None
        self._xs = None
        self._prune_rows = None
        self._xs_key = None
        for key in ("nll", "one", "mean", "pgrad"):
            self._replays.pop(key, None)
        self.cond_estimate = None
        self.log_determinant = None

    def _rt(self):
        if self._rt_cache is not None:
            return self._rt_cache
        import torch
        lib = _lib.load()
        if not torch.cuda.is_available():
            raise _lib.ApgpError("no MI355X visible: approxposterior_amd has no CPU fallback")
        dev = self._device_arg
        if dev is None:
            dev = torch.device("cuda", torch.cuda.current_device())
        elif not isinstance(dev, torch.device):
            dev = torch.device(dev)
        self._queries = (torch.cuda.current_device, getattr(torch._C, "_cuda_getCurrentRawStream", None))
        self._rt_cache = (torch, dev, lib)
        return self._rt_cache

    @staticmethod
    def _on(torch, dev):
        if torch.cuda.current_device() == dev.index:
            return _NULL_CONTEXT
        return torch.cuda.device(dev)

    @staticmethod
    def _stream(torch):
        raw = getattr(torch._C, "_cuda_getCurrentRawStream", None)
        if raw is not None:
            return ctypes.c_void_p(raw(torch.cuda.current_device()))
        return ctypes.c_void_p(torch.cuda.current_stream().cuda_stream)

    def _kernel_struct(self, ks=None):
        amp, log_M, lin_coef, lin_order = _flatten_kernel(self.kernel, with_linear=True)
        if ks is None:
            ks = _lib.KernelStruct()
        elif ks.ndim != len(log_M):
            raise ValueError("dimension mismatch")
        ks.ndim = len(log_M)
        ks.amp = amp
        ks.lin_coef = lin_coef
        ks.lin_order = lin_order
        ks.diag_add = float(self._yerr2) + float(np.exp(self.white_noise.value))
        ks.inv_metric[:len(log_M)] = np.exp(-np.asarray(log_M, dtype=np.float64)).tolist()
        return ks

    def get_parameter_names(self):
        names = []
        if self.fit_mean:
            names.append("mean:value")
        if self.fit_white_noise:
            names.append("white_noise:value")
        names += ["kernel:" + n for n in self.kernel.get_parameter_names()]
        return tuple(names)

    def get_parameter_vector(self):
        v = []
        if self.fit_mean:
            v.append(self.mean.value)
        if self.fit_white_noise:
            v.append(self.white_noise.value)
        return np.concatenate([np.array(v, dtype=np.float64),
                               self.kernel.get_parameter_vector()])

    def set_parameter_vector(self, p):
        p = np.asarray(p, dtype=np.float64).ravel()
        if len(p) != len(self):
            raise ValueError("dimension mismatch")
        n = 0
        if self.fit_mean:
            self.mean.value = float(p[n]); n += 1
        if self.fit_white_noise:
            self.white_noise.value = float(p[n]); n += 1
        self.kernel.set_parameter_vector(p[n:])
        self.kernel.dirty = True

    def __len__(self):
        return int(self.fit_mean) + int(self.fit_white_noise) + len(self.kernel)

    @property
    def computed(self):
        return self._computed and not self.kernel.dirty

    def parse_samples(self, t):
        t = np.atleast_1d(np.asarray(t, dtype=np.float64))
        if t.ndim == 1:
            t = t[:, None]
        if t.ndim != 2 or t.shape[1] != self.kernel.ndim:
            raise ValueError("Dimension mismatch")
        return np.ascontiguousarray(t)

    def _check_dimensions(self, y):
        y = np.atleast_1d(np.asarray(y, dtype=np.float64))
        if self._x is None or y.shape[0] != len(self._x):
            raise ValueError("Dimension mismatch")
        return np.ascontiguousarray(y)

    def compute(self, x, yerr=0.0, previous=None, **kwargs):
        x_in = x
        x = self.parse_samples(x)
        if x.shape[1] > _lib.MAX_DIM:
            raise ValueError("approxposterior_amd supports at most %d input dimensions (APGP_MAX_DIM in include/apgp.h: the "
                             "kernels keep a point's coordinates in registers); got %d" % (_lib.MAX_DIM, x.shape[1]))
        if not np.isfinite(x).all():
            raise ValueError("array must not contain infs or NaNs")
        if x is x_in or (isinstance(x_in, np.ndarray) and np.shares_memory(x, x_in)):
            x = x.copy()
        same_x = self._x is not None and self._x.shape == x.shape and np.array_equal(self._x, x)
        self._x = x
        self._nllMemo = None
        self._yerr2 = float(yerr) ** 2
        if previous is not None and self._try_extend(previous):
            return
        self._factor(None, upload_x=not same_x)

    def _trust_inverse(self):
        mode = (self.variance_mode or "").lower()
        if mode == "inverse":
            return True
        if mode == "solve":
            return False
        return self.cond_estimate is not None and self.cond_estimate <= COND_SOLVE

    def _factor_key(self):
        return bytes(self._kernel_struct())

    def _try_extend(self, prev):
        if getattr(prev, "_L", None) is None or getattr(prev, "_x", None) is None:
            return False
        if getattr(prev, "_factored_key", None) != self._factor_key():
            return False
        n0, n1 = len(prev._x), len(self._x)
        limit = self.extend_max_rows if self.extend_max_rows is not None else (1 if n1 >= 512 else 2)
        if not (0 < n0 < n1 and n1 - n0 <= min(64, int(limit)) and prev._x.shape[1] == self._x.shape[1]
                and np.array_equal(prev._x, self._x[:n0])):
            return False
        torch, dev, lib = self._rt()
        ks = self._kernel_struct()
        w_prev = None
        if getattr(prev, "_work", None) is not None and prev._trust_inverse():
            w_prev = prev._work
        prev_L, prev_store = prev._L, getattr(prev, "_L_store", None)
        self._reset_device_state()
        self._computed = False
        with self._on(torch, dev):
            st = self._stream(torch)
            self._x_d = torch.from_numpy(self._x).to(dev)
            if prev_store is not None and prev_store["used"] == n0 and prev_store["buf"].shape[0] >= n1:
                store = prev_store
            else:
                cap = ((max(n1 + 63, int(1.5 * n1)) + 63) // 64) * 64
                store = {"buf": torch.zeros((cap, cap), dtype=torch.float64, device=dev), "used": n0}
                store["buf"][:n0, :n0].copy_(prev_L[:n0, :n0])
            buf = store["buf"]
            ld = buf.shape[1]
            L = buf[:n1, :n1]
            row = torch.empty(n1, dtype=torch.float64, device=dev)
            ss = torch.empty(1, dtype=torch.float64, device=dev)
            info = torch.zeros(1, dtype=torch.int32, device=dev)
            for j in range(n0, n1):
                _lib.check(lib.apgp_kernel_cross(self._x_d[j:].data_ptr(), 1, self._x_d.data_ptr(), j,
                                                 ctypes.byref(ks), row.data_ptr(), n1, st), "apgp_kernel_cross")
                if j == n0 and w_prev is not None:
                    _lib.check(lib.apgp_winv_apply(w_prev.data_ptr(), (n0 + 63) // 64 * 64, n0, row.data_ptr(), 0.0,
                                                   0, L[j].data_ptr(), ss.data_ptr(), None, st),
                               "apgp_winv_apply(append)")
                else:
                    _lib.check(lib.apgp_trsv(L.data_ptr(), j, ld, row.data_ptr(), 0.0, 0, L[j].data_ptr(),
                                             ss.data_ptr(), st), "apgp_trsv(append)")
                kxx = ks.amp
                if ks.lin_coef != 0.0:
                    kxx += ks.lin_coef * float(np.sum((self._x[j] * self._x[j]) ** ks.lin_order))
                _lib.check(lib.apgp_append_diag(L[j, j:].data_ptr(), ss.data_ptr(), kxx + ks.diag_add,
                                                info.data_ptr(), j + 1, st), "apgp_append_diag")
            store["used"] = n1
            out5 = torch.empty(5, dtype=torch.float64, device=dev)
            _lib.check(lib.apgp_fit_summary(L.data_ptr(), n1, ld, None, info.data_ptr(), out5.data_ptr(), st),
                       "apgp_fit_summary")
            o = out5.cpu().numpy()
        try:
            self._take_record(o, n1, bytes(ks))
        except LinAlgError:
            store["used"] = -1
            self._reset_device_state()
            raise
        self._L = L
        self._L_store = store
        self._ld = ld
        return True

    def _take_record(self, o, n, key):
        if o[4] != 0.0:
            raise LinAlgError("%d-th leading minor of the array is not positive definite" % int(o[4]))
        if not math.isfinite(o[0]):
            raise LinAlgError("non-finite log-determinant")
        self.log_determinant = float(o[0])
        self.cond_estimate = float((o[2] / o[1]) ** 2)
        self._const = -0.5 * (n * _LOG_2PI + self.log_determinant)
        self._computed = True
        self.kernel.dirty = False
        self._factored_key = key

    def _factor(self, y, upload_x=False):
        r = self._replays.get("nll")
        if (r is not None and y is not None and not upload_x
                and r.fits(y, (self._x, self._x_d, self._y_d, self._L, self._z))):
            ks, o = r.data
            self._kernel_struct(ks)
            self._alpha = self._packed = self._packed_solve = self._work = self._xs = self._xs_key = None
            self._prune_rows = None
            self._computed = False
            r.args[4] = float(self.mean.value)
            try:
                _lib.check(r.fn(*r.args), "apgp_nll_eval")
                self._take_record(o, r.n, bytes(ks))
            except Exception:
                self._reset_device_state()
                raise
            self._ztz_host = float(o[3])
            self._alpha_mean = self.mean.value
            return
        torch, dev, lib = self._rt()
        x = self._x
        n = len(x)
        yv = None if y is None else self._check_dimensions(y)
        keep_x = None if upload_x else self._x_d
        keep_y = self._y_d if (yv is not None and self._alpha_y is not None
                               and np.array_equal(self._alpha_y, yv)) else None
        keep_nll = (self._L, self._z) if (self._L is not None and self._z is not None and self._L_store is None
                                          and self._nll_owned) else None
        keep_stream = self._nll_stream
        self._reset_device_state()
        self._computed = False
        ks = self._kernel_struct()
        with self._on(torch, dev):
            st = self._stream(torch)
            self._x_d = keep_x if keep_x is not None else torch.from_numpy(x).to(dev)
            reuse = keep_nll if (keep_nll is not None and yv is not None and keep_nll[0].shape[0] == n
                                 and keep_stream == st.value) else None
            if reuse is not None:
                K, z = reuse
            else:
                K = (torch.empty if (yv is not None and n <= 64) else torch.zeros)((n, n), dtype=torch.float64, device=dev)
                z = None
            y_d = None
            if yv is not None:
                y_d = keep_y if keep_y is not None else torch.from_numpy(yv).to(dev)
                if z is None:
                    z = torch.empty(n, dtype=torch.float64, device=dev)
            scr = self._nll_scratch
            if scr is None:
                scr = self._nll_scratch = (torch.empty(1, dtype=torch.int32, device=dev),
                                           torch.empty(5, dtype=torch.float64, device=dev))
            o = np.empty(5, dtype=np.float64)
            args = [self._x_d.data_ptr(), n, ctypes.byref(ks), y_d.data_ptr() if y_d is not None else None,
                    float(self.mean.value), K.data_ptr(), z.data_ptr() if yv is not None else None,
                    scr[0].data_ptr(), scr[1].data_ptr(), o.ctypes.data, st]
            _lib.check(lib.apgp_nll_eval(*args), "apgp_nll_eval")
            if yv is None:
                z = None
            L = K
        self._take_record(o, n, bytes(ks))
        self._L = L
        self._ld = n
        if z is not None:
            self._z = z
            self._ztz_host = float(o[3])
            self._y_d = y_d
            self._alpha_y = np.array(yv, copy=True)
            self._alpha_mean = self.mean.value
            self._nll_owned = True
            self._nll_stream = st.value
            self._replays["nll"] = _Replay(lib.apgp_nll_eval, args, dev.index, st.value or 0, yv,
                                           (x, self._x_d, y_d, K, z), self._queries, data=(ks, o))

    def recompute(self, quiet=False, **kwargs):
        if self.kernel.dirty or not self._computed:
            if self._x is None:
                raise RuntimeError("You need to compute the model first")
            try:
                self._factor(None)
            except (ValueError, LinAlgError):
                if quiet:
                    return False
                raise
        return True

    def _candidates(self, t):
        if hasattr(t, "data_ptr"):
            if t.dim() != 2 or t.shape[1] != self.kernel.ndim or not t.is_contiguous() \
                    or str(t.dtype) != "torch.float64" or not t.is_cuda:
                raise ValueError("device candidates must be a contiguous (M, D) float64 CUDA tensor")
            return t
        torch, dev, _ = self._rt()
        return torch.from_numpy(self.parse_samples(t)).to(dev)

    def _mask(self, mask, m):
        if mask is None:
            return None
        mk = np.ascontiguousarray(np.asarray(mask).astype(np.uint8))
        if mk.shape != (m,):
            raise ValueError("mask must have one entry per candidate")
        torch, dev, _ = self._rt()
        return torch.from_numpy(mk).to(dev)

    def _variance_operand(self, use_solve):
        if use_solve:
            return (None, 0, self._L.data_ptr(), self._ld), self._L
        return (self._work.data_ptr(), (len(self._x) + 63) // 64 * 64, None, 0), self._work

    def _trsv(self, st, src, shift, trans, dst, ss, what, retry_ss=None):
        lib = self._rt()[2]
        solve = (self._L.data_ptr(), len(self._x), self._ld, src.data_ptr(), shift, trans, dst.data_ptr())
        _lib.check(lib.apgp_trsv(*solve, ss.data_ptr(), st), "apgp_trsv(%s)" % what)
        norm2 = float(ss.item())
        if norm2 != norm2:
            _lib.check(lib.apgp_trsv_ex(*solve, _ptr(retry_ss), 1, st), "apgp_trsv(%s, multi-launch)" % what)
            if retry_ss is not None:
                norm2 = float(retry_ss.item())
        return norm2

    def _solve(self, y, need_alpha):
        torch, dev, lib = self._rt()
        y = self._check_dimensions(y)
        n = len(y)
        same = (self._alpha_y is not None and self._alpha_mean == self.mean.value
                and np.array_equal(self._alpha_y, y))
        trust_w = self._trust_inverse()
        need_solve = (not same or self._z is None) or (need_alpha and self._alpha is None)
        if trust_w and need_solve and need_alpha and self._work is None and n >= W_FIRST_MIN_N:
            self._ensure_linv()
        via_w = self._work is not None and trust_w
        np64 = (n + 63) // 64 * 64
        with self._on(torch, dev):
            st = self._stream(torch)
            if not same or self._z is None:
                self._y_d = torch.from_numpy(y).to(dev)
                self._z = torch.empty(n, dtype=torch.float64, device=dev)
                ztz = torch.empty(1, dtype=torch.float64, device=dev)
                if via_w:
                    _lib.check(lib.apgp_winv_apply(self._work.data_ptr(), np64, n, self._y_d.data_ptr(),
                                                   float(self.mean.value), 0, self._z.data_ptr(),
                                                   ztz.data_ptr(), None, st), "apgp_winv_apply(forward)")
                    self._ztz_host = float(ztz.item())
                else:
                    self._ztz_host = self._trsv(st, self._y_d, float(self.mean.value), 0, self._z, ztz, "forward",
                                                retry_ss=ztz)
                self._alpha = None
                self._xs = self._prune_rows = None
                self._alpha_y = np.array(y, copy=True)
                self._alpha_mean = self.mean.value
            if need_alpha and self._alpha is None:
                self._alpha = torch.empty(n, dtype=torch.float64, device=dev)
                if via_w:
                    wk = torch.empty(int(lib.apgp_winv_apply_work_len(n)), dtype=torch.float64, device=dev)
                    _lib.check(lib.apgp_winv_apply(self._work.data_ptr(), np64, n, self._z.data_ptr(), 0.0, 1,
                                                   self._alpha.data_ptr(), None, wk.data_ptr(), st),
                               "apgp_winv_apply(backward)")
                else:
                    self._trsv(st, self._z, 0.0, 1, self._alpha, torch.empty(1, dtype=torch.float64, device=dev), "backward")
                self._xs = self._prune_rows = None
        return self._ztz_host

    def log_likelihood(self, y, quiet=False):
        try:
            if self.kernel.dirty or not self._computed:
                if self._x is None:
                    raise RuntimeError("You need to compute the model first")
                self._factor(y)
                ztz = self._ztz_host
            else:
                ztz = self._solve(y, need_alpha=False)
            ll = self._const - 0.5 * ztz
        except (ValueError, LinAlgError):
            if quiet:
                return -np.inf
            raise
        return ll if np.isfinite(ll) else -np.inf

    lookahead = None

    def lookahead_width(self):
        if self.lookahead is not None:
            return int(self.lookahead)
        n = 0 if self._x is None else len(self._x)
        if n <= 0:
            return 0
        return 5 if n <= 1216 else (3 if n <= 1728 else (1 if n <= 2112 else 0))

    def _fast_structs(self, P, out):
        k = self.kernel
        tk = type(k)
        if tk is ExpSquaredKernel:
            amp_dim, d = 0, k.ndim
        elif tk is Product and type(k.k1) is ConstantKernel and type(k.k2) is ExpSquaredKernel:
            amp_dim, d = k.k1.ndim, k.k2.ndim
        else:
            return None
        at = 0
        if self.fit_mean:
            means = P[:, 0].copy(); at += 1
        else:
            means = np.full(len(P), float(self.mean.value))
        ints = out.view(np.int32)
        out[:] = 0.0
        ints[:, 0] = d
        c = at + int(self.fit_white_noise)
        if self.fit_white_noise:
            out[:, 2] = float(self._yerr2) + np.exp(np.ascontiguousarray(P[:, at]))
        else:
            out[:, 2] = float(self._yerr2) + float(np.exp(self.white_noise.value))
        if amp_dim:
            out[:, 1] = amp_dim * np.exp(np.ascontiguousarray(P[:, c]))
            c += 1
        else:
            out[:, 1] = 1.0
        out[:, 3:3 + d] = np.exp(-P[:, c:c + d])
        return means

    def nll_batch(self, P, y):
        torch, dev, lib = self._rt()
        if self._x is None:
            raise RuntimeError("You need to compute the model first")
        P = np.atleast_2d(np.asarray(P, dtype=np.float64))
        B, n = len(P), len(self._x)
        if P.shape[1] != len(self):
            raise ValueError("dimension mismatch")
        r = self._replays.get(("batch", B))
        if r is not None and r.fits(y, (self._x, self._batch)):
            karr, o = r.data
            means = self._fast_structs(P, karr)
            if means is not None:
                self._batch.means[:B] = means
                self.kernel.dirty = True
                self._computed = False
                _lib.check(r.fn(*r.args), "apgp_nll_eval_batch")
                return _records_nll(o, n)
        yv = self._check_dimensions(y)
        out = np.full(B, np.inf)
        saved = self.get_parameter_vector()
        structs, means, live = [], [], []
        try:
            for b in range(B):
                try:
                    self.set_parameter_vector(P[b])
                    ks = self._kernel_struct()
                except (LinAlgError, ValueError, OverflowError):
                    continue
                structs.append(ks)
                means.append(float(self.mean.value))
                live.append(b)
        finally:
            self.set_parameter_vector(saved)
        if not live:
            return out
        per = max(1, int((2 << 30) // (8 * n * n)))
        with self._on(torch, dev):
            st = self._stream(torch)
            if self._x_d is None:
                self._x_d = torch.from_numpy(self._x).to(dev)
            ybytes = yv.tobytes()
            work = self._batch
            if (work is None or work.x_d is not self._x_d or work.stream != (st.value or 0) or work.ybytes != ybytes
                    or work.x is not self._x):
                work = self._batch = _BatchWork(self._x, self._x_d, st.value or 0, ybytes, torch.from_numpy(yv).to(dev),
                                                {}, np.empty(8, dtype=np.float64))
                self._replays = {k: v for k, v in self._replays.items() if type(k) is not tuple}
            for c0 in range(0, len(live), per):
                idx = live[c0:c0 + per]
                nb = len(idx)
                karr = (_lib.KernelStruct * nb)(*structs[c0:c0 + nb])
                marr = np.array(means[c0:c0 + nb], dtype=np.float64)
                bufs = work.bufs.get(nb)
                if bufs is None:
                    bufs = (torch.empty((nb, n, n), dtype=torch.float64, device=dev),
                            torch.empty((nb, n), dtype=torch.float64, device=dev),
                            torch.empty(nb, dtype=torch.int32, device=dev),
                            torch.empty((nb, 5), dtype=torch.float64, device=dev))
                    if 8 * nb * n * n <= (256 << 20):
                        work.bufs[nb] = bufs
                K, z, info, o_d = bufs
                o = np.empty((nb, 5), dtype=np.float64)
                _lib.check(lib.apgp_nll_eval_batch(self._x_d.data_ptr(), n, nb, ctypes.addressof(karr),
                                                   work.y_d.data_ptr(), marr.ctypes.data, K.data_ptr(), z.data_ptr(),
                                                   info.data_ptr(), o_d.data_ptr(), o.ctypes.data, st),
                           "apgp_nll_eval_batch")
                if nb == B and B <= 8 and nb in work.bufs and ctypes.sizeof(_lib.KernelStruct) == 36 * 8:
                    ka = np.zeros((B, 36), dtype=np.float64)
                    oo = np.empty((B, 5), dtype=np.float64)
                    args = [self._x_d.data_ptr(), n, B, ka.ctypes.data, work.y_d.data_ptr(), work.means.ctypes.data,
                            K.data_ptr(), z.data_ptr(), info.data_ptr(), o_d.data_ptr(), oo.ctypes.data, st]
                    self._replays[("batch", B)] = _Replay(lib.apgp_nll_eval_batch, args, dev.index, st.value or 0, yv,
                                                          (self._x, work), self._queries, data=(ka, oo))
                out[idx] = _records_nll(o, n)
        return out

    def _ensure_linv(self):
        torch, dev, lib = self._rt()
        if self._packed is not None:
            return
        n = len(self._x)
        with self._on(torch, dev):
            st = self._stream(torch)
            self._work = torch.empty(lib.apgp_trtri_work_len(n), dtype=torch.float64, device=dev)
            self._packed = torch.empty(lib.apgp_packed_linv_len(n), dtype=torch.float64, device=dev)
            _lib.check(lib.apgp_trtri_pack(self._L.data_ptr(), n, self._ld, self._work.data_ptr(),
                                           self._packed.data_ptr(), None, st), "apgp_trtri_pack")

    def _ensure_lsolve(self):
        torch, dev, lib = self._rt()
        if self._packed_solve is not None:
            return
        n = len(self._x)
        with self._on(torch, dev):
            st = self._stream(torch)
            self._packed_solve = torch.empty(lib.apgp_packed_lsolve_len(n), dtype=torch.float64, device=dev)
            _lib.check(lib.apgp_pack_lsolve(self._L.data_ptr(), n, self._ld, self._packed_solve.data_ptr(), st),
                       "apgp_pack_lsolve")

    def _ensure_xs(self, y):
        torch, dev, lib = self._rt()
        self._solve(y, need_alpha=True)
        if self._xs is not None:
            return
        n = len(self._x)
        ks = self._kernel_struct()
        with self._on(torch, dev):
            st = self._stream(torch)
            self._xs = torch.empty(lib.apgp_packed_train_len(n, ks.ndim), dtype=torch.float64,
                                   device=dev)
            _lib.check(lib.apgp_pack_train(self._x_d.data_ptr(), self._alpha.data_ptr(), n,
                                           ctypes.byref(ks), self._xs.data_ptr(), st),
                       "apgp_pack_train")
            rows_len = int(lib.apgp_prune_rows_len(n, ks.ndim))
            self._prune_rows = None
            if rows_len > 0:
                self._prune_rows = torch.empty(rows_len, dtype=torch.float64, device=dev)
                _lib.check(lib.apgp_pack_prune_rows(self._xs.data_ptr(), n, ctypes.byref(ks),
                                                    self._prune_rows.data_ptr(), st), "apgp_pack_prune_rows")

    def predict(self, y, t, return_cov=True, return_var=False, cache=True, **kwargs):
        if (self._computed and not self.kernel.dirty and type(t) is np.ndarray and t.dtype == _F64
                and t.ndim == 2 and t.flags.c_contiguous):
            if return_var:
                r = self._replays.get("one")
                if (r is not None and t.shape == r.data[1] and r.args[4] == self.mean.value
                        and r.fits(y, (self._xs, self._p1_work, self._work if self._trust_inverse() else self._L))):
                    r.args[0] = t.ctypes.data
                    _lib.check(r.fn(*r.args), "apgp_predict1_host")
                    o2 = r.data[0]
                    return np.array([o2[0]]), np.array([o2[1]])
            elif not return_cov:
                r = self._replays.get("mean")
                m, d = t.shape
                if (r is not None and d == r.data[0] and 0 < m <= r.data[1] and r.args[5] == self.mean.value
                        and r.fits(y, (self._xs, self._mean_work))):
                    mu_h = np.empty(m)
                    r.args[0], r.args[1], r.args[6] = t.ctypes.data, m, mu_h.ctypes.data
                    _lib.check(r.fn(*r.args), "apgp_predict_mean_host")
                    return mu_h
        self.recompute()
        xs = self.parse_samples(t)
        if return_cov and not return_var:
            return self._predict_cov(y, xs)
        if not return_var:
            return self._mean(y, xs)
        if len(xs) == 1:
            return self._predict_one(y, xs)
        y = self._check_dimensions(y)
        if len(xs) == 0:
            return np.empty(0), np.empty(0)
        torch, dev, _ = self._rt()
        s = self._sweep(y, torch.from_numpy(xs).to(dev), _lib.UTIL_NONE, with_mu=True, with_var=True)
        return s.mu.cpu().numpy(), s.var.cpu().numpy()

    def _mean(self, y, xs):
        if len(xs) == 0:
            self._check_dimensions(y)
            return np.empty(0)
        if len(xs) <= 4096:
            return self._mean_host(y, xs)
        torch, dev, _ = self._rt()
        return self._mean_device(y, torch.from_numpy(xs).to(dev)).cpu().numpy()

    def _mean_host(self, y, xs):
        torch, dev, lib = self._rt()
        y = self._check_dimensions(y)
        n, m = len(self._x), len(xs)
        ks = self._kernel_struct()
        with self._on(torch, dev):
            st = self._stream(torch)
            self._ensure_xs(y)
            need = m * (ks.ndim + 1)
            if self._mean_work is None or self._mean_work.numel() < need:
                self._mean_work = torch.empty(max(need, 1024), dtype=torch.float64, device=dev)
            mu_h = np.empty(m, dtype=np.float64)
            args = [xs.ctypes.data, m, self._xs.data_ptr(), n, ctypes.byref(ks), float(self.mean.value),
                    mu_h.ctypes.data, self._mean_work.data_ptr(), st]
            _lib.check(lib.apgp_predict_mean_host(*args), "apgp_predict_mean_host")
            max_m = min(4096, self._mean_work.numel() // (ks.ndim + 1))
            self._replays["mean"] = _Replay(lib.apgp_predict_mean_host, args, dev.index, st.value or 0, y,
                                            (self._xs, self._mean_work), self._queries, data=(ks.ndim, max_m))
        return mu_h

    def _mean_device(self, y, T):
        torch, dev, lib = self._rt()
        y = self._check_dimensions(y)
        ks = self._kernel_struct()
        with self._on(torch, dev):
            self._ensure_xs(y)
            mu = torch.empty(T.shape[0], dtype=torch.float64, device=dev)
            _lib.check(lib.apgp_predict_mean(T.data_ptr(), T.shape[0], self._xs.data_ptr(), len(self._x),
                                             ctypes.byref(ks), float(self.mean.value), mu.data_ptr(),
                                             self._stream(torch)), "apgp_predict_mean")
        return mu

    def _predict_one(self, y, xs):
        torch, dev, lib = self._rt()
        y = self._check_dimensions(y)
        n = len(self._x)
        ks = self._kernel_struct()
        use_solve = not self._trust_inverse()
        with self._on(torch, dev):
            st = self._stream(torch)
            if not use_solve:
                self._ensure_linv()
            self._ensure_xs(y)
            if self._p1_work is None or self._p1_work.numel() < int(lib.apgp_predict1_work_len(n)):
                self._p1_work = torch.empty(int(lib.apgp_predict1_work_len(n)), dtype=torch.float64, device=dev)
            o2 = np.empty(2, dtype=np.float64)
            inv, factor = self._variance_operand(use_solve)
            args = [xs.ctypes.data, self._xs.data_ptr(), n, ctypes.byref(ks), float(self.mean.value), *inv,
                    self._p1_work.data_ptr(), o2.ctypes.data, st]
            _lib.check(lib.apgp_predict1_host(*args), "apgp_predict1_host")
            self._replays["one"] = _Replay(lib.apgp_predict1_host, args, dev.index, st.value or 0, y,
                                           (self._xs, self._p1_work, factor), self._queries, data=(o2, (1, ks.ndim)))
        return np.array([o2[0]]), np.array([o2[1]])

    def predict_grad(self, y, t, kind=None, bounds=None, zeta=0.01, return_device=False):
        if not self.computed:
            raise RuntimeError("ERROR: Need to compute GP before using it!")
        if kind is None:
            kid = _lib.UTIL_NONE
        else:
            try:
                kid = SEARCH_KINDS[str(kind).lower()]
            except KeyError:
                raise ValueError("kind must be None or one of %s" % sorted(SEARCH_KINDS))
        D = self.kernel.ndim
        bkey = None if bounds is None else np.asarray(bounds, dtype=np.float64).tobytes()
        host_point = (type(t) is np.ndarray and t.dtype == _F64 and t.size == D and t.ndim in (1, 2)
                      and t.flags.c_contiguous and not return_device)
        if host_point:
            r = self._replays.get("pgrad")
            if (r is not None and r.data[0] == (kid, bkey, float(zeta), self.mean.value)
                    and r.fits(y, (self._xs, self._pg_work, self._work if self._trust_inverse() else self._L))):
                _, torch, T_d, out = r.data
                T_d.copy_(torch.from_numpy(t.reshape(1, D)))
                _lib.check(r.fn(*r.args), "apgp_predict_grad")
                return self._pgrad_split(out.cpu().numpy(), 1, D, kid)
        torch, dev, lib = self._rt()
        lo, hi = _box(bounds, D)
        if hasattr(t, "data_ptr"):
            T = self._candidates(t)
        else:
            arr = np.asarray(t, dtype=np.float64)
            if arr.ndim == 1:
                if arr.size != D:
                    raise ValueError("Dimension mismatch")
                arr = arr.reshape(1, D)
            if arr.ndim != 2 or arr.shape[1] != D:
                raise ValueError("Dimension mismatch")
            T = None
        y = self._check_dimensions(y)
        n = len(self._x)
        m = int(T.shape[0] if T is not None else arr.shape[0])
        ks = self._kernel_struct()
        use_solve = not self._trust_inverse()
        with self._on(torch, dev):
            st = self._stream(torch)
            if T is None:
                T = torch.from_numpy(np.ascontiguousarray(arr)).to(dev)
            out = torch.empty(m * (3 + 3 * D), dtype=torch.float64, device=dev)
            if m == 0:
                res = self._pgrad_split(out, 0, D, kid)
                return res if return_device else tuple(o.cpu().numpy() for o in res)
            if not use_solve:
                self._ensure_linv()
            self._ensure_xs(y)
            need = int(lib.apgp_predict_grad_work_len(m, n))
            if self._pg_work is None or self._pg_work.numel() < need:
                self._pg_work = torch.empty(need, dtype=torch.float64, device=dev)
            inv, factor = self._variance_operand(use_solve)
            p0 = out.data_ptr()
            with_u = kid != _lib.UTIL_NONE
            args = [T.data_ptr(), m, self._xs.data_ptr(), n, ctypes.byref(ks), float(self.mean.value), *inv, kid,
                    lo, hi, float(zeta), float(np.max(y)),
                    p0, p0 + 8 * m, p0 + 16 * m if with_u else None, p0 + 24 * m, p0 + 8 * m * (3 + D),
                    p0 + 8 * m * (3 + 2 * D) if with_u else None, self._pg_work.data_ptr(), st]
            _lib.check(lib.apgp_predict_grad(*args), "apgp_predict_grad")
            if host_point:
                self._replays["pgrad"] = _Replay(
                    lib.apgp_predict_grad, args, dev.index, st.value or 0, y, (self._xs, self._pg_work, factor),
                    self._queries, data=((kid, bkey, float(zeta), self.mean.value), torch, T, out))
            if return_device:
                return self._pgrad_split(out, m, D, kid)
            return self._pgrad_split(out.cpu().numpy(), m, D, kid)

    @staticmethod
    def _pgrad_split(out, m, D, kid):
        mu, var, u = out[:m], out[m:2 * m], out[2 * m:3 * m]
        dmu, dvar, du = (out[m * (3 + j * D):m * (3 + (j + 1) * D)].reshape(m, D) for j in range(3))
        if kid == _lib.UTIL_NONE:
            return mu, var, dmu, dvar
        return u, du, mu, var

    def _sweep(self, y, T, kind_id, lo=None, hi=None, mask_d=None, zeta=0.01, idx_offset=0,
               with_mu=False, with_var=False, with_u=False):
        torch, dev, lib = self._rt()
        y = self._check_dimensions(y)
        n, m = len(self._x), T.shape[0]
        ks = self._kernel_struct()
        use_solve = not self._trust_inverse()
        with self._on(torch, dev):
            st = self._stream(torch)
            if use_solve:
                self._ensure_lsolve()
            else:
                self._ensure_linv()
            self._ensure_xs(y)
            f64 = dict(dtype=torch.float64, device=dev)
            mu, var, u = (torch.empty(m, **f64) if keep else None for keep in (with_mu, with_var, with_u))
            part = torch.empty(max(int(lib.apgp_acquire_work_len(m, n)), 2), **f64)
            best = torch.empty(2, **f64)
            ev = getattr(self, "kernel_events", None)
            if ev is not None:
                e0 = torch.cuda.Event(enable_timing=True)
                e0.record()
            args = (self._xs.data_ptr(), n, ctypes.byref(ks), float(self.mean.value), kind_id, lo, hi, _ptr(mask_d),
                    float(zeta), float(np.max(y)), _ptr(mu), _ptr(var), _ptr(u), part.data_ptr(), best.data_ptr(),
                    _ptr(self._prune_rows), st)
            prune_was = None if self.sweep_prune is None else lib.apgp_set_sweep_prune(int(self.sweep_prune))
            rowsplit_was = None if self.seed_rowsplit is None else lib.apgp_set_seed_rowsplit(int(self.seed_rowsplit))
            park_was = None if self.seed_park is None else lib.apgp_set_seed_park(int(self.seed_park))
            first_was = None if self.seed_first is None else lib.apgp_set_seed_first(int(self.seed_first))
            parts_was = None if self.seed_parts is None else lib.apgp_set_seed_parts(int(self.seed_parts))
            try:
                if use_solve:
                    _lib.check(lib.apgp_acquire_solve_rows(T.data_ptr(), m, int(idx_offset),
                                                           self._packed_solve.data_ptr(), *args), "apgp_acquire_solve_rows")
                else:
                    _lib.check(lib.apgp_acquire_rows(T.data_ptr(), m, int(idx_offset), self._packed.data_ptr(), *args),
                               "apgp_acquire_rows")
            finally:
                if prune_was is not None:
                    lib.apgp_set_sweep_prune(prune_was)
                if rowsplit_was is not None:
                    lib.apgp_set_seed_rowsplit(rowsplit_was)
                if park_was is not None:
                    lib.apgp_set_seed_park(park_was)
                if first_was is not None:
                    lib.apgp_set_seed_first(first_was)
                if parts_was is not None:
                    lib.apgp_set_seed_parts(parts_was)
            if self.sweep_prune_stats and kind_id != _lib.UTIL_NONE and mu is None and var is None and u is None:
                off = int(lib.apgp_sweep_prune_counts_offset(m, n))
                self.last_prune_counts = part[off:off + 5].view(torch.int64).clone()
            if ev is not None:
                e1 = torch.cuda.Event(enable_timing=True)
                e1.record()
                ev.append((e0, e1))
        return _Swept(best, mu, var, u)

    def acquire(self, y, t, kind, bounds=None, mask=None, zeta=0.01, return_all=False,
                idx_offset=0, device_record=False):
        if not self.computed:
            raise RuntimeError("ERROR: Need to compute GP before using it!")
        kind_id = UTILITY_KINDS[str(kind).lower()]
        if device_record and return_all:
            raise ValueError("device_record returns the arg-min record only")
        torch, dev, _ = self._rt()
        lo, hi = _box(bounds, self.kernel.ndim)
        T = self._candidates(t)
        mask_d = self._mask(mask, T.shape[0])
        y = self._check_dimensions(y)
        if T.shape[0] == 0:
            if device_record:
                return torch.tensor([int(np.float64(np.inf).view(np.int64)), -1], dtype=torch.int64, device=dev)
            return (-1, float("inf")) + ((np.empty(0),) * 3 if return_all else ())
        s = self._sweep(y, T, kind_id, lo, hi, mask_d, zeta, idx_offset, with_mu=return_all, with_var=return_all,
                        with_u=return_all)
        if device_record:
            return s.best.view(torch.int64)
        if not return_all:
            return _best_record(s.best)
        return _best_record(s.best) + (s.u.cpu().numpy(), s.mu.cpu().numpy(), s.var.cpu().numpy())

    def prune_bounds(self, y, t, kind, coarse=True, bounds=None, mask=None, zeta=0.01):
        if not self.computed:
            raise RuntimeError("ERROR: Need to compute GP before using it!")
        kind_id = UTILITY_KINDS[str(kind).lower()]
        torch, dev, lib = self._rt()
        lo, hi = _box(bounds, self.kernel.ndim)
        T = self._candidates(t)
        m = T.shape[0]
        mask_d = self._mask(mask, m)
        y = self._check_dimensions(y)
        ks = self._kernel_struct()
        with self._on(torch, dev):
            self._ensure_xs(y)
            bmin = torch.empty((m + 63) // 64, dtype=torch.float64, device=dev)
            _lib.check(lib.apgp_prune_bounds_rows(T.data_ptr(), m, self._xs.data_ptr(), len(self._x), ctypes.byref(ks),
                                                  float(self.mean.value), kind_id, lo, hi, _ptr(mask_d), float(zeta),
                                                  float(np.max(y)), int(bool(coarse)), bmin.data_ptr(),
                                                  _ptr(self._prune_rows), self._stream(torch)),
                       "apgp_prune_bounds_rows")
        return bmin.cpu().numpy()

    def nelder_mead_search(self, y, starts, kind, bounds=None, zeta=0.01, options=None, trace=False):
        try:
            kid = SEARCH_KINDS[str(kind).lower()]
        except KeyError:
            raise ValueError("kind must be one of %s" % sorted(SEARCH_KINDS))
        opts = dict(options or {})
        unknown = sorted(set(opts) - set(NM_OPTIONS))
        if unknown:
            raise ValueError("the device Nelder-Mead search does not take the option(s) %s (it takes %s)"
                             % (unknown, ", ".join(NM_OPTIONS)))
        if not self.computed:
            raise RuntimeError("ERROR: Need to compute GP before using it!")
        y = self._check_dimensions(y)
        D = self.kernel.ndim
        lo, hi = _box(bounds, D)
        X0 = np.ascontiguousarray(np.asarray(starts, dtype=np.float64).reshape(-1, D))
        R = len(X0)
        if not 1 <= R <= _lib.NM_MAX_RESTARTS:
            raise ValueError("between 1 and %d restarts per call" % _lib.NM_MAX_RESTARTS)
        rho, chi, psi, sigma = nm_coefficients(D, bool(opts.get("adaptive", False)))
        maxiter, maxfev = nm_limits(D, opts.get("maxiter"), opts.get("maxfev"))
        if not (1 <= maxiter <= _lib.NM_MAX_FEV and 1 <= maxfev <= _lib.NM_MAX_FEV):
            raise ValueError("maxiter and maxfev must lie between 1 and %d" % _lib.NM_MAX_FEV)
        opt = _lib.NmOptions(kind=kid, maxiter=maxiter, maxfev=maxfev, reserved=0, zeta=float(zeta),
                             ybest=float(np.max(y)), xatol=float(opts.get("xatol", 1e-4)),
                             fatol=float(opts.get("fatol", 1e-4)), rho=rho, chi=chi, psi=psi, sigma=sigma)
        torch, dev, lib = self._rt()
        n = len(self._x)
        ks = self._kernel_struct()
        use_solve = not self._trust_inverse()
        with self._on(torch, dev):
            st = self._stream(torch)
            if not use_solve:
                self._ensure_linv()
            self._ensure_xs(y)
            f64 = dict(dtype=torch.float64, device=dev)
            i32 = dict(dtype=torch.int32, device=dev)
            starts_d = torch.from_numpy(X0).to(dev)
            x_out = torch.empty((R, D), **f64)
            f_out = torch.empty(R, **f64)
            stats = torch.zeros((R, 3), **i32)
            work = torch.empty(int(lib.apgp_nm_search_work_len(R, n)), **f64)
            tr = torch.empty(R * maxfev * (D + 3), **f64) if trace else None
            steps = torch.zeros(R * maxiter, **i32) if trace else None
            inv, _ = self._variance_operand(use_solve)
            _lib.check(lib.apgp_nm_search(starts_d.data_ptr(), R, self._xs.data_ptr(), n, ctypes.byref(ks),
                                          float(self.mean.value), *inv, lo, hi, ctypes.byref(opt),
                                          x_out.data_ptr(), f_out.data_ptr(), stats.data_ptr(),
                                          _ptr(tr), _ptr(steps), work.data_ptr(), st),
                       "apgp_nm_search")
            x = x_out.cpu().numpy()
            fun = f_out.cpu().numpy()
            sts = stats.cpu().numpy()
            if trace:
                trh = tr.cpu().numpy().reshape(R, maxfev, D + 3)
                sth = steps.cpu().numpy().reshape(R, maxiter)
        nfev, nit, status = sts[:, 0].copy(), sts[:, 1].copy(), sts[:, 2].copy()
        if not trace:
            return x, fun, nfev, nit, status
        recs = []
        for r in range(R):
            rec = trh[r, :nfev[r]]
            recs.append({"x": rec[:, :D].copy(), "mu": rec[:, D].copy(), "var": rec[:, D + 1].copy(),
                         "u": rec[:, D + 2].copy(), "steps": [int(s) for s in sth[r] if s != 0]})
        return x, fun, nfev, nit, status, recs

    def acquire_batch(self, y, t, kind, q, bounds=None, mask=None, zeta=0.01, idx_offset=0, return_all=False):
        if not self.computed:
            raise RuntimeError("ERROR: Need to compute GP before using it!")
        q = int(q)
        if not 1 <= q <= _lib.MAX_FANTASY:
            raise ValueError("q must be between 1 and %d (APGP_MAX_FANTASY)" % _lib.MAX_FANTASY)
        kinds = [kind] * q if isinstance(kind, str) else list(kind)
        if len(kinds) != q:
            raise ValueError("kind must be one utility name or a sequence of q names")
        kind_ids = [UTILITY_KINDS[str(k).lower()] for k in kinds]
        torch, dev, lib = self._rt()
        y = self._check_dimensions(y)
        n, D = len(self._x), self.kernel.ndim
        lo, hi = _box(bounds, D)
        T = self._candidates(t)
        m = T.shape[0]
        mask_d = self._mask(mask, m)
        idx = np.full(q, -1, dtype=np.int64)
        ub = np.full(q, np.inf)
        if m == 0:
            return (idx, ub, np.empty(0), np.empty(0), np.empty(0)) if return_all else (idx, ub)
        s = self._sweep(y, T, kind_ids[0], lo, hi, mask_d, zeta, idx_offset, with_mu=True, with_var=True,
                        with_u=return_all)
        best, mu, u = s.best, s.mu, s.u
        ks = self._kernel_struct()
        ybest = float(np.max(y))
        with self._on(torch, dev):
            st = self._stream(torch)
            f64 = dict(dtype=torch.float64, device=dev)
            var = [s.var, torch.empty(m, **f64) if q > 1 else None]
            if q > 1:
                C = torch.empty((q - 1) * m, **f64)
                fpart = torch.empty(max(int(lib.apgp_acquire_fantasy_work_len(m)), 2), **f64)
                krow = torch.empty(n, **f64)
                z = torch.empty(n, **f64)
                beta = torch.empty(n, **f64)
                ss = torch.empty(1, **f64)
            cur = 0
            for j in range(q):
                bi, bu = _best_record(best)
                if bi < 0:
                    break
                idx[j], ub[j] = bi, bu
                if j == q - 1:
                    break
                r = bi - int(idx_offset)
                ybest = max(ybest, float(mu[r].item()))
                _lib.check(lib.apgp_kernel_cross(T.data_ptr() + 8 * r * D, 1, self._x_d.data_ptr(), n,
                                                 ctypes.byref(ks), krow.data_ptr(), n, st), "apgp_kernel_cross")
                self._trsv(st, krow, 0.0, 0, z, ss, "fantasy")
                self._trsv(st, z, 0.0, 1, beta, ss, "fantasy")
                _lib.check(lib.apgp_acquire_fantasy(T.data_ptr(), m, int(idx_offset), self._xs.data_ptr(), n,
                                                    ctypes.byref(ks), beta.data_ptr(), r, j + 1, C.data_ptr(), m,
                                                    mu.data_ptr(), var[cur].data_ptr(), var[1 - cur].data_ptr(),
                                                    kind_ids[j + 1], lo, hi, _ptr(mask_d), float(zeta), ybest,
                                                    _ptr(u), fpart.data_ptr(), best.data_ptr(), st),
                           "apgp_acquire_fantasy")
                cur = 1 - cur
            if return_all:
                return idx, ub, u.cpu().numpy(), mu.cpu().numpy(), var[cur].cpu().numpy()
        return idx, ub

    def _references(self, refs):
        R = np.ascontiguousarray(np.asarray(refs, dtype=np.float64))
        if R.ndim != 2 or R.shape[1] != self.kernel.ndim or not 1 <= len(R) <= _lib.MAX_REFS:
            raise ValueError("refs must be a (J, D) array of 1 <= J <= %d reference points (APGP_MAX_REFS)" % _lib.MAX_REFS)
        if not np.all(np.isfinite(R)):
            raise ValueError("refs must be finite")
        return R

    def integration_weights(self, y, refs, density="posterior"):
        if density not in ("posterior", "uniform"):
            raise ValueError("density must be 'posterior' or 'uniform'")
        R = self._references(refs)
        mu, var = self.predict(y, R, return_cov=False, return_var=True)
        mu, var = np.asarray(mu, dtype=np.float64), np.asarray(var, dtype=np.float64)
        return (mu if density == "posterior" else 2.0 * mu) + var

    def acquire_integrated(self, y, t, refs, logWeights=None, bounds=None, mask=None, idx_offset=0, return_all=False):
        if not self.computed:
            raise RuntimeError("ERROR: Need to compute GP before using it!")
        if self.kernel.ndim > _lib.INTEGRATED_MAX_DIM:
            raise NotImplementedError("the integrated acquisition pass takes at most %d dimensions" % _lib.INTEGRATED_MAX_DIM)
        R = self._references(refs)
        J = len(R)
        if logWeights is None:
            a = self.integration_weights(y, R, "posterior")
        else:
            a = np.ascontiguousarray(np.asarray(logWeights, dtype=np.float64)).reshape(-1)
            if a.shape != (J,):
                raise ValueError("logWeights must have one entry per reference point")
        if np.any(np.isnan(a)) or np.any(a == np.inf) or not np.any(a > -np.inf):
            raise ValueError("logWeights must not be NaN or +inf, and not all -inf")
        torch, dev, lib = self._rt()
        y = self._check_dimensions(y)
        n, D = len(self._x), self.kernel.ndim
        lo, hi = _box(bounds, D)
        T = self._candidates(t)
        m = T.shape[0]
        mask_d = self._mask(mask, m)
        if m == 0:
            return (-1, float("inf")) + ((np.empty(0),) * 3 if return_all else ())
        s = self._sweep(y, T, _lib.UTIL_NONE, idx_offset=idx_offset, with_mu=return_all, with_var=True)
        ks = self._kernel_struct()
        with self._on(torch, dev):
            st = self._stream(torch)
            f64 = dict(dtype=torch.float64, device=dev)
            R_d = torch.from_numpy(R).to(dev)
            a_d = torch.from_numpy(a).to(dev)
            kxr = torch.empty((n, J), **f64)
            if self._x_d is None or self._x_d.shape[0] != n:
                self._x_d = torch.from_numpy(self._x).to(dev)
            _lib.check(lib.apgp_kernel_cross(self._x_d.data_ptr(), n, R_d.data_ptr(), J, ctypes.byref(ks),
                                             kxr.data_ptr(), J, st), "apgp_kernel_cross")
            L = torch.tril(self._L[:n, :n])
            z = torch.linalg.solve_triangular(L, kxr, upper=False)
            B = torch.linalg.solve_triangular(L.t(), z, upper=True).contiguous()
            u = torch.empty(m, **f64) if return_all else None
            part = torch.empty(max(int(lib.apgp_integrated_work_len(m, J)), 2), **f64)
            best = torch.empty(2, **f64)
            _lib.check(lib.apgp_acquire_integrated(T.data_ptr(), m, int(idx_offset), self._xs.data_ptr(), n,
                                                   ctypes.byref(ks), R_d.data_ptr(), J, B.data_ptr(), a_d.data_ptr(),
                                                   s.var.data_ptr(), lo, hi, _ptr(mask_d), None, 0, _ptr(u),
                                                   part.data_ptr(), best.data_ptr(), st), "apgp_acquire_integrated")
            rec = _best_record(best)
            if return_all:
                return rec + (u.cpu().numpy(), s.mu.cpu().numpy(), s.var.cpu().numpy())
        return rec

    def _path_call(self, T, ks, mean, paths, V, lo=None, hi=None, mask_d=None, idx_offset=0, with_f=False):
        torch, dev, lib = self._rt()
        m, S = T.shape[0], paths.size
        with self._on(torch, dev):
            st = self._stream(torch)
            f64 = dict(dtype=torch.float64, device=dev)
            F = torch.empty((S, m), **f64) if with_f else None
            part = torch.empty(max(int(lib.apgp_path_draws_work_len(m, S)), 2), **f64)
            best = torch.empty(2 * S, **f64)
            _lib.check(lib.apgp_path_draws(T.data_ptr(), m, int(idx_offset), _ptr(self._xs if V is not None else None),
                                           len(self._x), ctypes.byref(ks), float(mean), _ptr(V), paths.Z.data_ptr(),
                                           paths.b.data_ptr(), paths.W.data_ptr(), paths.Wl.data_ptr(),
                                           paths.nFeatures, S, lo, hi, _ptr(mask_d), _ptr(F), part.data_ptr(),
                                           best.data_ptr(), st), "apgp_path_draws")
            bb = best.cpu().numpy().reshape(S, 2)
        return F, bb[:, 1].copy().view(np.int64), bb[:, 0].copy()

    def sample_paths(self, y, size, nFeatures=2048):
        if not self.computed:
            raise RuntimeError("ERROR: Need to compute GP before using it!")
        size, nFeatures = int(size), int(nFeatures)
        if not 1 <= size <= _lib.MAX_DRAWS:
            raise ValueError("size must be between 1 and %d (APGP_MAX_DRAWS)" % _lib.MAX_DRAWS)
        if not 1 <= nFeatures <= _lib.MAX_FEATURES:
            raise ValueError("nFeatures must be between 1 and %d (APGP_MAX_FEATURES)" % _lib.MAX_FEATURES)
        y = self._check_dimensions(y)
        n, D = len(self._x), self.kernel.ndim
        diag_add = self._kernel_struct().diag_add
        Z = np.random.standard_normal((nFeatures, D))
        b = np.random.uniform(0.0, 2.0 * np.pi, nFeatures)
        W = np.random.standard_normal((size, nFeatures))
        Wl = np.random.standard_normal((size, D))
        eps = np.sqrt(diag_add) * np.random.standard_normal((size, n))
        return self._paths_from(y, Z, b, W, Wl, eps)

    def _paths_from(self, y, Z, b, W, Wl, eps):
        torch, dev, lib = self._rt()
        y = self._check_dimensions(y)
        n = len(self._x)
        self._ensure_xs(y)
        up = lambda a: torch.from_numpy(np.ascontiguousarray(a, dtype=np.float64)).to(dev)
        paths = PathDraws(self, up(Z), up(b), up(W), up(Wl))
        S = paths.size
        via_w = self._work is not None and self._trust_inverse()
        np64 = (n + 63) // 64 * 64
        with self._on(torch, dev):
            st = self._stream(torch)
            f64 = dict(dtype=torch.float64, device=dev)
            G, _, _ = self._path_call(self._x_d, paths.ks, 0.0, paths, None, with_f=True)
            rhs = (up(y) - float(self.mean.value)).unsqueeze(0) - G - up(eps)
            Vt = torch.empty((S, n), **f64)
            z, ss = torch.empty(n, **f64), torch.empty(1, **f64)
            wk = torch.empty(int(lib.apgp_winv_apply_work_len(n)), **f64) if via_w else None
            for s in range(S):
                if via_w:
                    w = self._work.data_ptr()
                    _lib.check(lib.apgp_winv_apply(w, np64, n, rhs[s].data_ptr(), 0.0, 0, z.data_ptr(), None, None, st),
                               "apgp_winv_apply(paths, forward)")
                    _lib.check(lib.apgp_winv_apply(w, np64, n, z.data_ptr(), 0.0, 1, Vt[s].data_ptr(), None,
                                                   wk.data_ptr(), st), "apgp_winv_apply(paths, backward)")
                else:
                    self._trsv(st, rhs[s], 0.0, 0, z, ss, "paths")
                    self._trsv(st, z, 0.0, 1, Vt[s], ss, "paths")
            paths.V = Vt.t().contiguous()
        return paths

    def thompson_batch(self, y, t, q, bounds=None, mask=None, idx_offset=0, nFeatures=2048, maxRounds=4,
                       return_draws=False):
        q = int(q)
        if not 1 <= q <= _lib.MAX_DRAWS:
            raise ValueError("q must be between 1 and %d (APGP_MAX_DRAWS)" % _lib.MAX_DRAWS)
        if not self.computed:
            raise RuntimeError("ERROR: Need to compute GP before using it!")
        T = self._candidates(t)
        mask_d = self._mask(mask, T.shape[0])
        idx, draws = [], []
        for rnd in range(int(maxRounds)):
            if len(idx) == q or T.shape[0] == 0:
                break
            paths = self.sample_paths(y, min(_lib.MAX_DRAWS, 2 * (q - len(idx))), nFeatures)
            winners, _ = paths.argmax(T, bounds=bounds, mask=mask_d, idx_offset=idx_offset)
            for s, g in enumerate(winners.tolist()):
                if g >= 0 and g not in idx and len(idx) < q:
                    idx.append(g)
                    draws.append((rnd, s))
        out = np.full(q, -1, dtype=np.int64)
        out[:len(idx)] = idx
        return (out, draws) if return_draws else out

    def box_candidates(self, m, bounds, seed, idx_offset=0):
        torch, dev, lib = self._rt()
        D = self.kernel.ndim
        lo, hi = _box(bounds, D, optional=False)
        with self._on(torch, dev):
            T = torch.empty((int(m), D), dtype=torch.float64, device=dev)
            if int(m) == 0:
                return T
            _lib.check(lib.apgp_box_candidates(T.data_ptr(), int(m), D, lo, hi, _seed64(seed),
                                               int(idx_offset), self._stream(torch)), "apgp_box_candidates")
        return T

    @staticmethod
    def _prior_records(prior, D):
        kind, p0, p1 = prior.records()
        if len(kind) != D:
            raise ValueError("the prior must have one factor per dimension")
# ... 637 lines not shown
```

### include/apgp.h

```cpp
#ifndef APGP_H
#define APGP_H

#include <stddef.h>
#include <stdint.h>

#ifdef __cplusplus
extern "C" {
#endif

#define APGP_ABI_VERSION 8
#define APGP_MAX_DIM 32
#define APGP_ROW_BLOCK 512
#define APGP_K_CHUNK 16
#define APGP_CAND_BLOCK 64

#define APGP_UTIL_AGP 0
#define APGP_UTIL_BAPE 1
#define APGP_UTIL_JONES 2
#define APGP_UTIL_NONE 3
#define APGP_UTIL_NEG_MEAN 4

typedef struct apgp_kernel {
    int32_t ndim;
    int32_t lin_order;
    double amp;
    double diag_add;
    double inv_metric[APGP_MAX_DIM];
    double lin_coef;
} apgp_kernel_t;

typedef struct apgp_best {
    double u;
    int64_t index;
} apgp_best_t;

int apgp_abi_version(void);
const char* apgp_last_error(void);

int64_t apgp_npad(int64_t n);
int64_t apgp_packed_linv_len(int64_t n);
int64_t apgp_packed_train_len(int64_t n, int32_t ndim);
int64_t apgp_trtri_work_len(int64_t n);

int apgp_gram(const double* X, int64_t n, const apgp_kernel_t* kern ,
              double* K, int64_t ldk, void* stream);

int apgp_kernel_cross(const double* X1, int64_t m, const double* X2, int64_t n,
                      const apgp_kernel_t* kern , double* C, int64_t ldc, void* stream);

int apgp_potrf(double* A, int64_t n, int64_t lda, const double* y, double shift, double* z,
               int32_t* info_dev, void* stream);

int apgp_logdet(const double* L, int64_t n, int64_t ldl, double* out5, void* stream);
int apgp_fit_summary(const double* L, int64_t n, int64_t ldl, const double* z,
                     const int32_t* info_dev, double* out5, void* stream);

int apgp_release_scratch(void* stream);

int apgp_nll_eval(const double* X, int64_t n, const apgp_kernel_t* kern ,
                  const double* y, double mean, double* K, double* z,
                  int32_t* info_dev, double* out5_dev, double* out5_host ,
                  void* stream);

int apgp_potrf_mode(int mode);
int64_t apgp_potrf_fallbacks(void);
int64_t apgp_potrf_backoff_skips(void);

int64_t apgp_nll_side_batches(void);
int apgp_nll_eval_batch(const double* X, int64_t n, int64_t batch,
                        const apgp_kernel_t* kerns , const double* y,
                        const double* means , double* K, double* z,
                        int32_t* info_dev, double* out5_dev, double* out5_host ,
                        void* stream);

int apgp_trsv(const double* L, int64_t n, int64_t ldl, const double* b, double shift,
              int trans, double* x, double* sumsq, void* stream);
int apgp_trsv_mode(int multi_launch);
int apgp_trsv_ex(const double* L, int64_t n, int64_t ldl, const double* b, double shift,
                 int trans, double* x, double* sumsq, int mode, void* stream);

int apgp_append_diag(double* ljj, const double* ss, double kdiag, int32_t* info_dev, int64_t order,
                     void* stream);

int64_t apgp_winv_apply_work_len(int64_t n);
int apgp_winv_apply(const double* winv, int64_t ldw, int64_t n, const double* b, double shift,
                    int trans, double* x, double* sumsq, double* work, void* stream);

int apgp_trtri_pack(const double* L, int64_t n, int64_t ldl, double* work,
                    double* packed, double* winv_dense, void* stream);

int apgp_pack_train(const double* X, const double* alpha, int64_t n,
                    const apgp_kernel_t* kern , double* xs, void* stream);

int64_t apgp_acquire_work_len(int64_t m, int64_t n);
int apgp_acquire(const double* T, int64_t m, int64_t idx_offset,
                 const double* packed_linv, const double* xs, int64_t n,
                 const apgp_kernel_t* kern , double mean, int32_t kind,
                 const double* lo , const double* hi ,
                 const uint8_t* mask, double zeta, double ybest,
                 double* mu, double* var, double* u,
                 void* part, apgp_best_t* best, void* stream);

int64_t apgp_packed_lsolve_len(int64_t n);
int apgp_pack_lsolve(const double* L, int64_t n, int64_t ldl, double* packed, void* stream);
int apgp_acquire_solve(const double* T, int64_t m, int64_t idx_offset,
                       const double* packed_lsolve, const double* xs, int64_t n,
                       const apgp_kernel_t* kern , double mean, int32_t kind,
                       const double* lo , const double* hi ,
                       const uint8_t* mask, double zeta, double ybest,
                       double* mu, double* var, double* u,
                       void* part, apgp_best_t* best, void* stream);

int apgp_set_sweep_prune(int v);
int apgp_get_sweep_prune(void);
int apgp_set_seed_rowsplit(int v);
int apgp_get_seed_rowsplit(void);
int apgp_set_seed_park(int v);
int apgp_get_seed_park(void);
int apgp_set_seed_first(int v);
int apgp_get_seed_first(void);
int apgp_set_seed_parts(int v);
int apgp_get_seed_parts(void);
int64_t apgp_sweep_prune_counts_offset(int64_t m, int64_t n);
int apgp_sweep_prune_select(const double* bmin, int64_t ncb, const int64_t* seeds, int64_t* counts,
                            double tau, int64_t* list, void* stream);
int apgp_prune_bounds(const double* T, int64_t m, const double* xs, int64_t n,
                      const apgp_kernel_t* kern , double mean, int32_t kind,
                      const double* lo , const double* hi , const uint8_t* mask,
                      double zeta, double ybest, int coarse, double* bmin_out, void* stream);
int apgp_sweep_prune_seeds(const double* bmin, int64_t ncb, int64_t* seeds, int64_t* counts, void* stream);

int64_t apgp_prune_rows_len(int64_t n, int32_t ndim);
int apgp_pack_prune_rows(const double* xs, int64_t n, const apgp_kernel_t* kern , void* rows, void* stream);
int apgp_acquire_rows(const double* T, int64_t m, int64_t idx_offset,
                      const double* packed_linv, const double* xs, int64_t n,
                      const apgp_kernel_t* kern , double mean, int32_t kind,
                      const double* lo , const double* hi ,
                      const uint8_t* mask, double zeta, double ybest,
                      double* mu, double* var, double* u,
                      void* part, apgp_best_t* best, const void* prune_rows, void* stream);
int apgp_acquire_solve_rows(const double* T, int64_t m, int64_t idx_offset,
                            const double* packed_lsolve, const double* xs, int64_t n,
                            const apgp_kernel_t* kern , double mean, int32_t kind,
                            const double* lo , const double* hi ,
                            const uint8_t* mask, double zeta, double ybest,
                            double* mu, double* var, double* u,
                            void* part, apgp_best_t* best, const void* prune_rows, void* stream);
int apgp_prune_bounds_rows(const double* T, int64_t m, const double* xs, int64_t n,
                           const apgp_kernel_t* kern , double mean, int32_t kind,
                           const double* lo , const double* hi , const uint8_t* mask,
                           double zeta, double ybest, int coarse, double* bmin_out, const void* prune_rows,
                           void* stream);

#define APGP_MAX_FANTASY 32
int64_t apgp_acquire_fantasy_work_len(int64_t m);
int apgp_acquire_fantasy(const double* T, int64_t m, int64_t idx_offset,
                         const double* xs, int64_t n, const apgp_kernel_t* kern ,
                         const double* beta, int64_t pick_row, int32_t j, double* C, int64_t ldc,
                         const double* mu, const double* var_in, double* var_out,
                         int32_t kind, const double* lo , const double* hi ,
                         const uint8_t* mask, double zeta, double ybest,
                         double* u, void* part, apgp_best_t* best, void* stream);

#define APGP_MAX_DRAWS 32
#define APGP_MAX_FEATURES 65536
int64_t apgp_path_draws_work_len(int64_t m, int32_t ndraws);
int apgp_path_draws_mode(int mode);
int apgp_path_draws(const double* T, int64_t m, int64_t idx_offset, const double* xs, int64_t n,
                    const apgp_kernel_t* kern , double mean, const double* V, const double* Z,
                    const double* b, const double* W, const double* Wl, int32_t nfeat, int32_t ndraws,
                    const double* lo , const double* hi , const uint8_t* mask, double* F,
                    void* part, apgp_best_t* best, void* stream);

#define APGP_MAX_REFS 4096
#define APGP_INTEGRATED_MAX_DIM 16
int64_t apgp_integrated_work_len(int64_t m, int32_t nref);
int apgp_integrated_mode(int mode);
int apgp_acquire_integrated(const double* T, int64_t m, int64_t idx_offset,
                            const double* xs, int64_t n, const apgp_kernel_t* kern ,
                            const double* R, int32_t nref, const double* B, const double* a,
                            const double* var, const double* lo , const double* hi ,
                            const uint8_t* mask, double* C, int64_t ldc, double* u,
                            void* part, apgp_best_t* best, void* stream);

int64_t apgp_predict1_work_len(int64_t n);
int apgp_predict1_host(const double* t_host , const double* xs, int64_t n,
                       const apgp_kernel_t* kern , double mean,
                       const double* winv, int64_t ldw, const double* L, int64_t ldl,
                       double* work, double* out2_host , void* stream);

#define APGP_NM_MAX_RESTARTS 4096
#define APGP_NM_MAX_FEV (1 << 20)
#define APGP_NM_STEP_REFLECT 1
#define APGP_NM_STEP_EXPAND 2
#define APGP_NM_STEP_REFLECT_EXP 3
#define APGP_NM_STEP_CONTRACT_OUT 4
#define APGP_NM_STEP_CONTRACT_IN 5
#define APGP_NM_STEP_SHRINK_OUT 6
#define APGP_NM_STEP_SHRINK_IN 7
#define APGP_NM_STEP_MAXFEV 8
typedef struct apgp_nm_options {
    int32_t kind;
    int32_t maxiter;
    int32_t maxfev;
    int32_t reserved;
    double zeta, ybest;
    double xatol, fatol;
    double rho, chi, psi, sigma;
} apgp_nm_options_t;
int64_t apgp_nm_search_work_len(int64_t restarts, int64_t n);
int apgp_nm_search(const double* starts, int64_t restarts, const double* xs, int64_t n,
                   const apgp_kernel_t* kern , double mean,
                   const double* winv, int64_t ldw, const double* L, int64_t ldl,
                   const double* lo , const double* hi , const apgp_nm_options_t* opt ,
                   double* x_out, double* f_out, int32_t* stats, double* trace, int32_t* steps,
                   double* work, void* stream);

int64_t apgp_predict_grad_work_len(int64_t m, int64_t n);
int apgp_predict_grad(const double* T, int64_t m, const double* xs, int64_t n,
                      const apgp_kernel_t* kern , double mean,
                      const double* winv, int64_t ldw, const double* L, int64_t ldl,
                      int32_t kind, const double* lo , const double* hi , double zeta, double ybest,
                      double* mu, double* var, double* u, double* dmu, double* dvar, double* du,
                      double* work, void* stream);

int apgp_predict_mean(const double* T, int64_t m, const double* xs, int64_t n,
                      const apgp_kernel_t* kern , double mean,
                      double* mu, void* stream);

int apgp_predict_mean_host(const double* T_host, int64_t m, const double* xs, int64_t n,
                           const apgp_kernel_t* kern , double mean,
                           double* mu_host, double* work, void* stream);

int apgp_ensemble_mode(int mode);
int apgp_ensemble_sample_ex(const double* xs, int64_t n, const apgp_kernel_t* kern , double mean,
                            const double* lo , const double* hi ,
                            int32_t nwalkers, int32_t nensembles, int64_t iterations, double a_stretch,
                            uint64_t seed, double* coords, double* logp, double* chain,
                            double* logp_chain, int64_t* naccept, int mode, void* stream);
int apgp_ensemble_sample(const double* xs, int64_t n, const apgp_kernel_t* kern , double mean,
                         const double* lo , const double* hi ,
                         int32_t nwalkers, int32_t nensembles, int64_t iterations,
                         double a_stretch, uint64_t seed,
                         double* coords, double* logp, double* chain, double* logp_chain,
                         int64_t* naccept, void* stream);

#define APGP_ENS_MOVE_STRETCH 0
#define APGP_ENS_MOVE_DE 1
#define APGP_ENS_MOVE_SNOOKER 2
#define APGP_ENS_MAX_MOVES 8
typedef struct apgp_ens_move {
    int32_t kind;
    double weight, p0, p1;
} apgp_ens_move_t;
int apgp_ensemble_sample_moves(const double* xs, int64_t n, const apgp_kernel_t* kern , double mean,
                               const double* lo , const double* hi ,
                               int32_t nwalkers, int32_t nensembles, int64_t iterations, double a_stretch,
                               uint64_t seed, double* coords, double* logp, double* chain,
                               double* logp_chain, int64_t* naccept, int mode,
                               const apgp_ens_move_t* moves , int32_t nmoves, void* stream);

#define APGP_PT_MAX_TEMPS 64
int64_t apgp_tempered_work_len(int32_t nwalkers, int32_t ntemps, int32_t nladders, int32_t ndim);
int apgp_tempered_sample(const double* xs, int64_t n, const apgp_kernel_t* kern , double mean,
                         const double* lo , const double* hi ,
                         int32_t nwalkers, int32_t ntemps, int32_t nladders, const double* betas ,
                         int64_t iterations, int64_t swap_every, uint64_t seed, double* coords, double* logp,
                         double* chain, int32_t nstore, double* logp_chain, int64_t* naccept, int64_t* swap_prop,
                         int64_t* swap_acc, uint8_t* swap_log, const apgp_ens_move_t* moves , int32_t nmoves,
                         double* work, void* stream);

#define APGP_HMC_MAX_LEAP 1024
typedef struct apgp_hmc_options {
    double eps, jitter;
    int32_t nleap;
    int32_t g_rows;
    int64_t iteration0;
    double mass[APGP_MAX_DIM];
} apgp_hmc_options_t;
int apgp_hmc_sample(const double* xs, int64_t n, const apgp_kernel_t* kern , double mean,
                    const double* lo , const double* hi , int32_t nchains,
                    int64_t iterations, const apgp_hmc_options_t* opt , uint64_t seed,
                    double* coords, double* logp, double* chain, double* logp_chain, int64_t* naccept, double* accprob,
                    int64_t* ndiverge, double* prop, double* dH, double* trace, void* stream);
int apgp_hmc_rule(int32_t nchains, int64_t n, int32_t ndim);

int64_t apgp_nested_work_len(int32_t ndim, int32_t nlive, int32_t nruns);
int apgp_nested_xlds(int64_t n, int32_t ndim);
int apgp_nested_sample(const double* xs, int64_t n, const apgp_kernel_t* kern , double mean,
                       const double* lo , const double* hi , int32_t nlive,
                       int32_t batch, int32_t nsteps, int32_t max_batches, double dlogz, double sigma, double gamma0,
                       int32_t nruns, uint64_t seed, double* work, double* points, double* logl, double* birth,
                       int32_t* rec, int64_t* counts, double* logz, double* trace, void* stream);

int apgp_box_candidates(double* T, int64_t m, int32_t ndim, const double* lo ,
                        const double* hi , uint64_t seed, int64_t idx_offset, void* stream);

int apgp_prior_candidates(double* T, int64_t m, int32_t ndim, const int32_t* kind ,
                          const double* p0 , const double* p1 , uint64_t seed,
                          int64_t idx_offset, void* stream);
int apgp_prior_lnprior(const double* X, int64_t m, int32_t ndim, const int32_t* kind ,
                       const double* p0 , const double* p1 , double* out, void* stream);

#define APGP_GMM_EM 0
#define APGP_GMM_SCORE 1
#define APGP_GMM_KMEANS 2
int64_t apgp_gmm_params_len(int32_t ndim, int32_t ncomp);
int64_t apgp_gmm_stats_len(int32_t ndim, int32_t ncomp);
int apgp_gmm_pass(const double* X, int64_t n, int32_t ndim, int32_t ncomp, const double* params, int32_t mode,
                  double* stats_out, double* row_lp, int32_t* row_label, void* stream);

#define APGP_IMP_BLOCK 256
#define APGP_IMP_MAX_BLOCKS 2048
int64_t apgp_mix_params_len(int32_t ndim, int32_t ncomp);
int apgp_mix_candidates(double* T, double* lnq, int64_t m, int32_t ndim, int32_t ncomp, const double* params ,
                        uint64_t seed, int64_t idx_offset, void* stream);
int64_t apgp_importance_stats_len(int32_t ndim);
int64_t apgp_importance_work_len(int64_t m);
int apgp_importance_pass(const double* T, int64_t m, const double* lnq, const double* xs, int64_t n,
                         const apgp_kernel_t* kern , double mean, const double* lo ,
                         const double* hi , const double* centre , double* logw_out,
                         double* stats_out, double* work, void* stream);

int32_t apgp_sobol_direction(int32_t d, int32_t b);
int apgp_sobol_box_candidates(double* T, int64_t m, int32_t ndim, const double* lo , const double* hi ,
                              uint64_t seed, int32_t replicate, int32_t scramble, int64_t idx_offset, void* stream);
int apgp_sobol_prior_candidates(double* T, int64_t m, int32_t ndim, const int32_t* kind ,
                                const double* p0 , const double* p1 , uint64_t seed, int32_t replicate,
                                int32_t scramble, int64_t idx_offset, void* stream);
int apgp_sobol_mix_candidates(double* T, double* lnq, int64_t m, int32_t ndim, int32_t ncomp,
                              const double* params , uint64_t seed, int32_t replicate, int32_t scramble,
                              int64_t idx_offset, void* stream);

int64_t apgp_path_importance_work_len(int64_t m, int32_t ndraws);
int apgp_path_importance(const double* T, int64_t m, const double* lnq,
                         const double* xs, int64_t n, const apgp_kernel_t* kern , double mean,
                         const double* V, const double* Z, const double* b, const double* W, const double* Wl,
                         int32_t nfeat, int32_t ndraws,
                         const double* lo , const double* hi , const double* centre ,
                         double* logw_out ,
                         double* stats_out ,
                         double* work, void* stream);

int64_t apgp_autocorr_work_len(int64_t n_t, int64_t n_w, int32_t n_d);
int apgp_autocorr_block(const double* x, int64_t n_t, int64_t n_w, int32_t n_d, int64_t row0, int64_t row_stride,
                        int64_t lag0, int64_t nlags, int32_t reuse_stats, double* work, double* f, void* stream);

int64_t apgp_grad_work_len(int64_t n);
int64_t apgp_kinv_solve_work_len(int64_t n);
int apgp_kinv_solve(const double* L, int64_t n, int64_t ldl, double* xwork, double* kinv, void* stream);
int apgp_grad_loglik(const double* X, const double* alpha, const double* winv, int64_t ldw,
                     int64_t n, const apgp_kernel_t* kern ,
                     double* work, double* out, void* stream);

#ifdef __cplusplus
}
#endif
#endif
```

Measured before the change: 867.9 million.

## Add sign-sorted packed training rows for the coarse pruning bound kernel

```diff
diff --git a/approxposterior_amd/_lib.py b/approxposterior_amd/_lib.py
--- a/approxposterior_amd/_lib.py
+++ b/approxposterior_amd/_lib.py
@@ -17,6 +17,7 @@
 NM_MAX_FEV = 1 << 20
 NM_STEPS = {1: "reflect", 2: "expand", 3: "reflect_exp", 4: "contract_out", 5: "contract_in",
             6: "shrink_out", 7: "shrink_in", 8: "maxfev"}
+PRUNE_ROWS_SPLIT, PRUNE_ROWS_SIGNED = 0, 1
 GMM_EM, GMM_SCORE, GMM_KMEANS = 0, 1, 2
 GMM_MAX_COMP = 16
 IMP_BLOCK = 256
@@ -128,6 +129,16 @@
                                                _F64, _F64, _P, _P, _P, _P, _P, _P, _P]),
     "apgp_prune_bounds_rows": (ctypes.c_int, [_P, _I64, _P, _I64, _KP, _F64, _I32, ctypes.POINTER(_F64),
                                               ctypes.POINTER(_F64), _P, _F64, _F64, ctypes.c_int, _P, _P, _P]),
+    "apgp_prune_srows_len": (_I64, [_I64, _I32]),
+    "apgp_pack_prune_srows": (ctypes.c_int, [_P, _I64, _KP, _P, _P]),
+    "apgp_acquire_rows2": (ctypes.c_int, [_P, _I64, _I64, _P, _P, _I64, _KP, _F64, _I32,
+                                          ctypes.POINTER(_F64), ctypes.POINTER(_F64), _P,
+                                          _F64, _F64, _P, _P, _P, _P, _P, _P, _I32, _P]),
+    "apgp_acquire_solve_rows2": (ctypes.c_int, [_P, _I64, _I64, _P, _P, _I64, _KP, _F64, _I32,
+                                                ctypes.POINTER(_F64), ctypes.POINTER(_F64), _P,
+                                                _F64, _F64, _P, _P, _P, _P, _P, _P, _I32, _P]),
+    "apgp_prune_bounds_rows2": (ctypes.c_int, [_P, _I64, _P, _I64, _KP, _F64, _I32, ctypes.POINTER(_F64),
+                                               ctypes.POINTER(_F64), _P, _F64, _F64, ctypes.c_int, _P, _P, _I32, _P, _P]),
     "apgp_acquire_fantasy_work_len": (_I64, [_I64]),
     "apgp_acquire_fantasy": (ctypes.c_int, [_P, _I64, _I64, _P, _I64, _KP, _P, _I64, _I32, _P, _I64,
                                             _P, _P, _P, _I32, ctypes.POINTER(_F64), ctypes.POINTER(_F64), _P,
diff --git a/approxposterior_amd/csrc/prune_mm32.h b/approxposterior_amd/csrc/prune_mm32.h
--- a/approxposterior_amd/csrc/prune_mm32.h
+++ b/approxposterior_amd/csrc/prune_mm32.h
@@ -117,8 +117,121 @@
     }
 }
 
-template <int DPAD, bool PRE = false>
+__host__ __device__ inline long long pmm_srow(long long q, int s) {
+    return 32 * (q >> 1) + (s & 3) + 8 * (s >> 2) + 4 * (int)(q & 1);
+}
+__host__ __device__ inline long long pmm_stiles(long long n) {
+    const long long nrt_max = ((n + 15) / 16 + 2) / 2;
+    return (nrt_max + PMM_ROWS / 32 - 1) / (PMM_ROWS / 32);
+}
+#define PMM_SHDR 32
+
+template <int DPAD>
+__device__ __forceinline__ void pmm_put_row(unsigned char* tile, int srow, const float (&pe)[DPAD + 2], float alpha) {
+    using SH = PmmShape<DPAD>;
+    __bf16* xrow = (__bf16*)tile + srow * SH::PITCH;
+    pmm_store_row<DPAD>(xrow, pe, std::make_integer_sequence<int, 2 * SH::NI>{});
+    ((float*)(tile + 16 * SH::XPIECES))[srow] = alpha;
+    *(bf16x8*)(xrow + 16 * SH::NI) = bf16x8{(__bf16)0.0f, (__bf16)0.0f, (__bf16)0.0f, (__bf16)0.0f,
+                                            (__bf16)0.0f, (__bf16)0.0f, (__bf16)0.0f, (__bf16)0.0f};
+}
+
+template <int DPAD>
+__global__ __launch_bounds__(PR_THREADS) void pmm_pack_srows_kernel(const double* xs, long long n, unsigned char* rows) {
+    using SH = PmmShape<DPAD>;
+    constexpr int XS = DPAD + 2, NW = PR_THREADS / 64;
+    const double kappa = PR32_KAPPA;
+    __shared__ int wp[2][NW], wn[2][NW];
+    __shared__ double wmax[NW], wsal[NW];
+    const int tid = threadIdx.x, lane = tid & 63, w = tid >> 6;
+    double cen[DPAD];
+#pragma unroll
+    for (int d = 0; d < DPAD; ++d) cen[d] = xs[d];
+    int cnt = 0;
+    for (long long i = tid; i < n; i += PR_THREADS) cnt += xs[i * XS + DPAD] < 0.0 ? 0 : 1;
+    for (int o = 32; o > 0; o >>= 1) cnt += __shfl_xor(cnt, o);
+    if (lane == 0) wp[0][w] = cnt;
+    __syncthreads();
+    long long np = 0;
+#pragma unroll
+    for (int i = 0; i < NW; ++i) np += wp[0][i];
+    __syncthreads();
+    const long long nn = n - np, gp = (np + 15) / 16, gn = (nn + 15) / 16;
+    unsigned char* img = rows + PMM_SHDR;
+    double sal = 0.0, bm2 = 0.0;
+    long long base_p = 0, base_n = 0;
+    const long long nround = (n + PR_THREADS - 1) / PR_THREADS;
+    for (long long rd = 0; rd < nround; ++rd) {
+        const long long i = rd * PR_THREADS + tid;
+        const bool in = i < n;
+        const f64x2* src = (const f64x2*)(xs + (in ? i : 0) * XS);
+        f64x2 pre[XS / 2];
+#pragma unroll
+        for (int j = 0; j < XS / 2; ++j) pre[j] = src[j];
+        const double alpha = pre[DPAD / 2].x;
+        const bool neg = in && alpha < 0.0, pos = in && !neg;
+        const unsigned long long mp = __ballot(pos), mn = __ballot(neg), below = (1ull << lane) - 1ull;
+        const int b = (int)(rd & 1);
+        if (lane == 0) { wp[b][w] = __popcll(mp); wn[b][w] = __popcll(mn); }
+        __syncthreads();
+        long long k = pos ? base_p : base_n;
+#pragma unroll
+        for (int j = 0; j < NW; ++j) {
+            if (j < w) k += pos ? wp[b][j] : wn[b][j];
+            base_p += wp[b][j];
+            base_n += wn[b][j];
+        }
+        k += __popcll((pos ? mp : mn) & below);
+        if (in) {
+            float pe[DPAD + 2];
+            double n2 = 0.0, b2 = 0.0;
+#pragma unroll
+            for (int d = 0; d < DPAD; ++d) {
+                const double x = (d & 1) ? pre[d >> 1].y : pre[d >> 1].x;
+                const double df = x - cen[d];
+                b2 = fma(df, df, b2);
+                const float bf = (float)(df * kappa);
+                n2 = fma((double)bf, (double)bf, n2);
+                pe[d + 2] = 2.0f * bf;
+            }
+            bm2 = fmax(bm2, b2);
+            sal += fabs(alpha);
+            pe[0] = -(float)n2;
+            pe[1] = 1.0f;
+            const long long r = pmm_srow((pos ? 0 : gp) + (k >> 4), (int)(k & 15));
+            pmm_put_row<DPAD>(img + r / PMM_ROWS * (16ll * SH::PIECES), (int)(r % PMM_ROWS), pe, (float)alpha);
+        }
+    }
+    for (long long r = tid; r < pmm_stiles(n) * PMM_ROWS; r += PR_THREADS) {
+        const int rr = (int)(r & 31), s = (rr & 3) + 4 * (rr >> 3);
+        const long long q = 2 * (r >> 5) + ((rr >> 2) & 1);
+        const bool empty = q < gp ? 16 * q + s >= np : q < gp + gn ? 16 * (q - gp) + s >= nn : true;
+        if (empty) {
+            float pe[DPAD + 2];
+#pragma unroll
+            for (int d = 0; d < DPAD; ++d) pe[d + 2] = 0.0f;
+            pe[0] = -0.0f;
+            pe[1] = 1.0f;
+            pmm_put_row<DPAD>(img + r / PMM_ROWS * (16ll * SH::PIECES), (int)(r % PMM_ROWS), pe, 0.0f);
+        }
+    }
+    for (int o = 32; o > 0; o >>= 1) { bm2 = fmax(bm2, __shfl_xor(bm2, o)); sal += __shfl_xor(sal, o); }
+    if (lane == 0) { wmax[w] = bm2; wsal[w] = sal; }
+    __syncthreads();
+    if (tid == 0) {
+        sal = 0.0;
+#pragma unroll
+        for (int i = 0; i < NW; ++i) { bm2 = fmax(bm2, wmax[i]); sal += wsal[i]; }
+        ((double*)rows)[0] = bm2;
+        ((double*)rows)[1] = sal;
+        ((long long*)rows)[2] = (gp + gn + 1) / 2;
+        ((long long*)rows)[3] = 0;
+    }
+}
+
+template <int DPAD, bool PRE = false, bool SGN = false>
 __global__ __launch_bounds__(PR_THREADS, PMM_G <= 4 ? 2 : 1) void prune_bound_mm32_kernel(PruneArgs a) {
+    static_assert(PRE || !SGN, "the sign-sorted rows come as a stream only");
     using SH = PmmShape<DPAD>;
     constexpr int XS = DPAD + 2;
     constexpr int K = SH::K, NI = SH::NI, PITCH = SH::PITCH, G = PMM_G;
@@ -174,10 +287,12 @@
     double accm[G], accs[G], sal = 0.0, bm2 = 0.0;
 #pragma unroll
     for (int g = 0; g < G; ++g) { accm[g] = 0.0; accs[g] = 0.0; }
-    const long long ntile = (a.n + PMM_ROWS - 1) / PMM_ROWS;
-    auto consume = [&](int xo, int ao) {
+    long long nrt = 0;
+    if constexpr (SGN) nrt = ((const long long*)a.prune_rows)[2];
+    const long long ntile = SGN ? (nrt + PMM_ROWS / 32 - 1) / (PMM_ROWS / 32) : (a.n + PMM_ROWS - 1) / PMM_ROWS;
+    auto consume = [&](int xo, int ao, int nr) {
 #pragma unroll 1
-        for (int rt = 0; rt < PMM_ROWS / 32; ++rt) {
+        for (int rt = 0; rt < (SGN ? nr : PMM_ROWS / 32); ++rt) {
             const __bf16* xr = xt + xo + (rt * 32 + l32) * PITCH + 8 * h;
             bf16x8 pop[NI];
 #pragma unroll
@@ -201,10 +316,10 @@
                 for (int r = 0; r < 16; ++r) {
                     const float k = __builtin_amdgcn_exp2f(cur[r]);
                     ps = fmaf(k, al[r], ps);
-                    pS = fmaf(k, fabsf(al[r]), pS);
+                    if constexpr (!SGN) pS = fmaf(k, fabsf(al[r]), pS);
                 }
                 accm[g] += (double)ps;
-                accs[g] += (double)pS;
+                accs[g] += (double)(SGN ? fabsf(ps) : pS);
                 cur = nxt;
             }
         }
@@ -212,7 +327,7 @@
     if constexpr (PRE) {
         typedef unsigned int u32x4 __attribute__((ext_vector_type(4)));
         constexpr int NPC = SH::PIECES, NL = (NPC + PR_THREADS - 1) / PR_THREADS;
-        const u32x4* img = (const u32x4*)((const unsigned char*)a.prune_rows + 16);
+        const u32x4* img = (const u32x4*)((const unsigned char*)a.prune_rows + (SGN ? PMM_SHDR : 16));
         u32x4 pre[NL];
         auto fetch = [&](long long ti) {
             const u32x4* src = img + ti * NPC;
@@ -238,7 +353,8 @@
         for (long long ti = 0; ti < ntile; ++ti) {
             const int b = (int)(ti & 1);
             fetch(ti + 1 < ntile ? ti + 1 : ntile - 1);
-            consume(b * PMM_ROWS * PITCH, b * PMM_ROWS);
+            const long long left = nrt - ti * (PMM_ROWS / 32);
+            consume(b * PMM_ROWS * PITCH, b * PMM_ROWS, left < PMM_ROWS / 32 ? (int)left : PMM_ROWS / 32);
             put(b ^ 1);
             __syncthreads();
         }
@@ -276,7 +392,7 @@
             }
             __syncthreads();
             if (ti + 1 < ntile) fetch(ti + 1);
-            consume(0, 0);
+            consume(0, 0, PMM_ROWS / 32);
             __syncthreads();
         }
         for (int o = 32; o > 0; o >>= 1) { bm2 = fmax(bm2, __shfl_xor(bm2, o)); sal += __shfl_xor(sal, o); }
diff --git a/approxposterior_amd/csrc/sweep.hip b/approxposterior_amd/csrc/sweep.hip
--- a/approxposterior_amd/csrc/sweep.hip
+++ b/approxposterior_amd/csrc/sweep.hip
@@ -1327,6 +1327,7 @@
     const long long* blk_count;
     double* est;
     const void* prune_rows;
+    int rows_kind;
 };
 
 template <int DPAD>
@@ -1813,17 +1814,21 @@
     return 0;
 }
 
+static inline bool pr_rows_kind_ok(const void* prune_rows, int rows_kind) {
+    return rows_kind == APGP_PRUNE_ROWS_SPLIT || (rows_kind == APGP_PRUNE_ROWS_SIGNED && prune_rows != NULL);
+}
+
 template <class Kern>
 static PruneArgs pr_args(const double* T, int64_t m, const double* xs, int64_t n, const uint8_t* mask, const Kern& kern,
                          double mean, int32_t kind, const double* lo, const double* hi, double zeta, double ybest,
-                         double* bmin, double* part_u, long long* part_i, const void* prune_rows) {
+                         double* bmin, double* part_u, long long* part_i, const void* prune_rows, int rows_kind) {
     PruneArgs p;
     p.T = T; p.xs = xs; p.mask = mask; p.bmin = bmin; p.part_u = part_u; p.part_i = part_i;
     p.m = m; p.ncb = pr_ncb(m); p.n = n;
     p.kind = kind; p.mean = mean; p.zeta = zeta; p.ybest = ybest;
     apgp_fill_kernel(p, kern);
     apgp_fill_box(p, p.ndim, lo, hi);
-    p.blk_list = NULL; p.blk_count = NULL; p.est = NULL; p.prune_rows = prune_rows;
+    p.blk_list = NULL; p.blk_count = NULL; p.est = NULL; p.prune_rows = prune_rows; p.rows_kind = rows_kind;
     return p;
 }
 
@@ -1834,7 +1839,9 @@
     if (coarse) {
         if constexpr (DPAD <= 8) {
             const dim3 mm_grid = grid_of(PMM_G / 2);
-            if (p.prune_rows)
+            if (p.prune_rows && p.rows_kind == APGP_PRUNE_ROWS_SIGNED)
+                hipLaunchKernelGGL((prune_bound_mm32_kernel<DPAD, true, true>), mm_grid, dim3(PR_THREADS), 0, s, p);
+            else if (p.prune_rows)
                 hipLaunchKernelGGL((prune_bound_mm32_kernel<DPAD, true>), mm_grid, dim3(PR_THREADS), 0, s, p);
             else
                 hipLaunchKernelGGL((prune_bound_mm32_kernel<DPAD, false>), mm_grid, dim3(PR_THREADS), 0, s, p);
@@ -1849,7 +1856,8 @@
 }
 
 template <int DPAD>
-static int launch_pruned(const SweepArgs& a, hipStream_t s, bool solve, void* part, const void* prune_rows) {
+static int launch_pruned(const SweepArgs& a, hipStream_t s, bool solve, void* part, const void* prune_rows,
+                         int rows_kind) {
     const int rc = s2_prepare_device<DPAD>();
     if (rc != 0) return rc;
     const long long ncb = pr_ncb(a.m);
@@ -1859,7 +1867,7 @@
     long long* counts = seeds + PR_SEED;
     const bool coarse = a.lin_coef == 0.0;
     PruneArgs p = pr_args(a.T, a.m, a.xs, a.n, a.mask, a, a.mean, a.kind, a.has_box ? a.lo : NULL, a.has_box ? a.hi : NULL,
-                          a.zeta, a.ybest, bmin, a.part_u, a.part_i, prune_rows);
+                          a.zeta, a.ybest, bmin, a.part_u, a.part_i, prune_rows, rows_kind);
     if (coarse) p.est = (double*)(counts + 8);
     launch_bound<DPAD>(p, s, coarse);
     hipLaunchKernelGGL(prune_seed_kernel, dim3(1), dim3(1024), 0, s, coarse ? (const double*)p.est : (const double*)bmin, ncb,
@@ -1893,8 +1901,9 @@
                         const double* xs, int64_t n, const apgp_kernel_t* kern, double mean,
                         int32_t kind, const double* lo, const double* hi, const uint8_t* mask,
                         double zeta, double ybest, double* mu, double* var, double* u, void* part,
-                        apgp_best_t* best, const void* prune_rows, void* stream) {
+                        apgp_best_t* best, const void* prune_rows, int rows_kind, void* stream) {
     APGP_CHECK_ARG(T && packed_linv && xs && kern, "null pointer");
+    APGP_CHECK_ARG(pr_rows_kind_ok(prune_rows, rows_kind), "rows_kind: SPLIT, or SIGNED with its stream");
     APGP_CHECK_ARG(m >= 1 && m <= APGP_MAX_M && n >= 1 && n <= APGP_MAX_N, "m >= 1 and n >= 1 required");
     APGP_CHECK_ARG(kind >= APGP_UTIL_AGP && kind <= APGP_UTIL_NONE, "unknown utility kind");
     APGP_CHECK_ARG(kind == APGP_UTIL_NONE || best, "best required for an acquisition");
@@ -1932,7 +1941,7 @@
     const bool prune = pr_mode > 0 && kind != APGP_UTIL_NONE && !mu && !var && !u && part &&
                        m >= (pr_mode == 1 ? pr_min_m(n) : (int64_t)pr_mode);
     const int rc = apgp_by_dpad(kc.dpad, [&](auto dp) {
-        return prune ? launch_pruned<decltype(dp)::value>(a, s, solve, part, prune_rows)
+        return prune ? launch_pruned<decltype(dp)::value>(a, s, solve, part, prune_rows, rows_kind)
                      : launch_sweep<decltype(dp)::value>(a, s, solve);
     });
     if (rc != 0) return rc;
@@ -1948,7 +1957,7 @@
                             double zeta, double ybest, double* mu, double* var, double* u, void* part,
                             apgp_best_t* best, void* stream) {
     return acquire_impl(false, T, m, idx_offset, packed_linv, xs, n, kern, mean, kind, lo, hi, mask, zeta, ybest,
-                        mu, var, u, part, best, NULL, stream);
+                        mu, var, u, part, best, NULL, APGP_PRUNE_ROWS_SPLIT, stream);
 }
 
 extern "C" int apgp_acquire_rows(const double* T, int64_t m, int64_t idx_offset, const double* packed_linv,
@@ -1957,7 +1966,16 @@
                                  double zeta, double ybest, double* mu, double* var, double* u, void* part,
                                  apgp_best_t* best, const void* prune_rows, void* stream) {
     return acquire_impl(false, T, m, idx_offset, packed_linv, xs, n, kern, mean, kind, lo, hi, mask, zeta, ybest,
-                        mu, var, u, part, best, prune_rows, stream);
+                        mu, var, u, part, best, prune_rows, APGP_PRUNE_ROWS_SPLIT, stream);
+}
+
+extern "C" int apgp_acquire_rows2(const double* T, int64_t m, int64_t idx_offset, const double* packed_linv,
+                                  const double* xs, int64_t n, const apgp_kernel_t* kern, double mean,
+                                  int32_t kind, const double* lo, const double* hi, const uint8_t* mask,
+                                  double zeta, double ybest, double* mu, double* var, double* u, void* part,
+                                  apgp_best_t* best, const void* prune_rows, int32_t rows_kind, void* stream) {
+    return acquire_impl(false, T, m, idx_offset, packed_linv, xs, n, kern, mean, kind, lo, hi, mask, zeta, ybest,
+                        mu, var, u, part, best, prune_rows, rows_kind, stream);
 }
 
 extern "C" int64_t apgp_prune_rows_len(int64_t n, int32_t ndim) {
@@ -1986,10 +2004,36 @@
     return 0;
 }
 
+extern "C" int64_t apgp_prune_srows_len(int64_t n, int32_t ndim) {
+    if (n < 0 || n > APGP_MAX_N || ndim < 1 || ndim > APGP_MAX_DIM) return -1;
+    const int dpad = apgp_dpad(ndim);
+    if (n == 0 || dpad > 8) return 0;
+    return apgp_by_dpad(dpad, [&](auto dp) -> int64_t {
+        if constexpr (decltype(dp)::value <= 8)
+            return PMM_SHDR / 8 + pmm_stiles(n) * 2 * PmmShape<decltype(dp)::value>::PIECES;
+        else return 0;
+    });
+}
+
+extern "C" int apgp_pack_prune_srows(const double* xs, int64_t n, const apgp_kernel_t* kern, void* rows, void* stream) {
+    APGP_CHECK_ARG(xs && kern && rows, "null pointer");
+    APGP_CHECK_ARG(n >= 1 && n <= APGP_MAX_N, "n >= 1 required");
+    KernConst kc;
+    APGP_CHECK_ARG(apgp_make_kernconst(kern, &kc) == 0, "kernel parameters");
+    APGP_CHECK_ARG(kc.dpad <= 8, "no sign-sorted rows beyond 8 dimensions (apgp_prune_srows_len is 0)");
+    apgp_by_dpad(kc.dpad, [&](auto dp) {
+        if constexpr (decltype(dp)::value <= 8)
+            hipLaunchKernelGGL(pmm_pack_srows_kernel<decltype(dp)::value>, dim3(1), dim3(PR_THREADS), 0, (hipStream_t)stream,
+                               xs, (long long)n, (unsigned char*)rows);
+    });
+    APGP_CHECK_LAUNCH();
+    return 0;
+}
+
 static int prune_bounds_impl(const char* who, const double* T, int64_t m, const double* xs, int64_t n,
                              const apgp_kernel_t* kern, double mean, int32_t kind, const double* lo, const double* hi,
                              const uint8_t* mask, double zeta, double ybest, int coarse, double* bmin_out,
-                             const void* prune_rows, void* stream) {
+                             const void* prune_rows, int rows_kind, double* est_out, void* stream) {
 #define PB_CHECK_ARG(cond, msg)                                     \
     do {                                                            \
         if (!(cond)) {                                              \
@@ -2001,11 +2045,13 @@
     PB_CHECK_ARG(m >= 1 && m <= APGP_MAX_M && n >= 1 && n <= APGP_MAX_N, "m >= 1 and n >= 1 required");
     PB_CHECK_ARG(kind >= APGP_UTIL_AGP && kind < APGP_UTIL_NONE, "unknown utility kind");
     PB_CHECK_ARG((lo == NULL) == (hi == NULL), "lo and hi must be given together");
+    PB_CHECK_ARG(pr_rows_kind_ok(prune_rows, rows_kind), "rows_kind: SPLIT, or SIGNED with its stream");
     KernConst kc;
     PB_CHECK_ARG(apgp_make_kernconst(kern, &kc) == 0, "kernel parameters");
     PB_CHECK_ARG(!coarse || kc.lin_coef == 0.0, "the coarse bound takes pure squared-exponential kernels only");
 #undef PB_CHECK_ARG
-    const PruneArgs p = pr_args(T, m, xs, n, mask, kc, mean, kind, lo, hi, zeta, ybest, bmin_out, NULL, NULL, prune_rows);
+    PruneArgs p = pr_args(T, m, xs, n, mask, kc, mean, kind, lo, hi, zeta, ybest, bmin_out, NULL, NULL, prune_rows, rows_kind);
+    if (coarse) p.est = est_out;
     hipStream_t s = (hipStream_t)stream;
     apgp_by_dpad(kc.dpad, [&](auto dp) { launch_bound<decltype(dp)::value>(p, s, coarse != 0); });
     APGP_CHECK_LAUNCH();
@@ -2016,7 +2062,7 @@
                                  double mean, int32_t kind, const double* lo, const double* hi, const uint8_t* mask,
                                  double zeta, double ybest, int coarse, double* bmin_out, void* stream) {
     return prune_bounds_impl(__func__, T, m, xs, n, kern, mean, kind, lo, hi, mask, zeta, ybest, coarse, bmin_out, NULL,
-                             stream);
+                             APGP_PRUNE_ROWS_SPLIT, NULL, stream);
 }
 
 extern "C" int apgp_prune_bounds_rows(const double* T, int64_t m, const double* xs, int64_t n, const apgp_kernel_t* kern,
@@ -2024,7 +2070,15 @@
                                       double zeta, double ybest, int coarse, double* bmin_out, const void* prune_rows,
                                       void* stream) {
     return prune_bounds_impl(__func__, T, m, xs, n, kern, mean, kind, lo, hi, mask, zeta, ybest, coarse, bmin_out,
-                             prune_rows, stream);
+                             prune_rows, APGP_PRUNE_ROWS_SPLIT, NULL, stream);
+}
+
+extern "C" int apgp_prune_bounds_rows2(const double* T, int64_t m, const double* xs, int64_t n, const apgp_kernel_t* kern,
+                                       double mean, int32_t kind, const double* lo, const double* hi, const uint8_t* mask,
+                                       double zeta, double ybest, int coarse, double* bmin_out, const void* prune_rows,
+                                       int32_t rows_kind, double* est_out, void* stream) {
+    return prune_bounds_impl(__func__, T, m, xs, n, kern, mean, kind, lo, hi, mask, zeta, ybest, coarse, bmin_out,
+                             prune_rows, rows_kind, est_out, stream);
 }
 
 extern "C" int apgp_sweep_prune_seeds(const double* bmin, int64_t ncb, int64_t* seeds, int64_t* counts, void* stream) {
@@ -2042,7 +2096,7 @@
                                   double zeta, double ybest, double* mu, double* var, double* u, void* part,
                                   apgp_best_t* best, void* stream) {
     return acquire_impl(true, T, m, idx_offset, packed_lsolve, xs, n, kern, mean, kind, lo, hi, mask, zeta, ybest,
-                        mu, var, u, part, best, NULL, stream);
+                        mu, var, u, part, best, NULL, APGP_PRUNE_ROWS_SPLIT, stream);
 }
 
 extern "C" int apgp_acquire_solve_rows(const double* T, int64_t m, int64_t idx_offset, const double* packed_lsolve,
@@ -2051,7 +2105,16 @@
                                        double zeta, double ybest, double* mu, double* var, double* u, void* part,
                                        apgp_best_t* best, const void* prune_rows, void* stream) {
     return acquire_impl(true, T, m, idx_offset, packed_lsolve, xs, n, kern, mean, kind, lo, hi, mask, zeta, ybest,
-                        mu, var, u, part, best, prune_rows, stream);
+                        mu, var, u, part, best, prune_rows, APGP_PRUNE_ROWS_SPLIT, stream);
+}
+
+extern "C" int apgp_acquire_solve_rows2(const double* T, int64_t m, int64_t idx_offset, const double* packed_lsolve,
+                                        const double* xs, int64_t n, const apgp_kernel_t* kern, double mean,
+                                        int32_t kind, const double* lo, const double* hi, const uint8_t* mask,
+                                        double zeta, double ybest, double* mu, double* var, double* u, void* part,
+                                        apgp_best_t* best, const void* prune_rows, int32_t rows_kind, void* stream) {
+    return acquire_impl(true, T, m, idx_offset, packed_lsolve, xs, n, kern, mean, kind, lo, hi, mask, zeta, ybest,
+                        mu, var, u, part, best, prune_rows, rows_kind, stream);
 }
 
 #define FT_THREADS 256
diff --git a/approxposterior_amd/gp.py b/approxposterior_amd/gp.py
--- a/approxposterior_amd/gp.py
+++ b/approxposterior_amd/gp.py
@@ -401,6 +401,7 @@
         self.seed_park = None
         self.seed_first = None
         self.seed_parts = None
+        self.prune_signed = True
         self.sweep_prune_stats = False
         self.last_prune_counts = None
         self._computed = False
@@ -437,6 +438,7 @@
         self._work = None
         self._xs = None
         self._prune_rows = None
+        self._prune_srows = None
         self._xs_key = None
         for key in ("nll", "one", "mean", "pgrad"):
             self._replays.pop(key, None)
@@ -649,7 +651,7 @@
             ks, o = r.data
             self._kernel_struct(ks)
             self._alpha = self._packed = self._packed_solve = self._work = self._xs = self._xs_key = None
-            self._prune_rows = None
+            self._prune_rows = self._prune_srows = None
             self._computed = False
             r.args[4] = float(self.mean.value)
             try:
@@ -788,7 +790,7 @@
                     self._ztz_host = self._trsv(st, self._y_d, float(self.mean.value), 0, self._z, ztz, "forward",
                                                 retry_ss=ztz)
                 self._alpha = None
-                self._xs = self._prune_rows = None
+                self._xs = self._prune_rows = self._prune_srows = None
                 self._alpha_y = np.array(y, copy=True)
                 self._alpha_mean = self.mean.value
             if need_alpha and self._alpha is None:
@@ -800,7 +802,7 @@
                                "apgp_winv_apply(backward)")
                 else:
                     self._trsv(st, self._z, 0.0, 1, self._alpha, torch.empty(1, dtype=torch.float64, device=dev), "backward")
-                self._xs = self._prune_rows = None
+                self._xs = self._prune_rows = self._prune_srows = None
         return self._ztz_host
 
     def log_likelihood(self, y, quiet=False):
@@ -979,6 +981,17 @@
                 self._prune_rows = torch.empty(rows_len, dtype=torch.float64, device=dev)
                 _lib.check(lib.apgp_pack_prune_rows(self._xs.data_ptr(), n, ctypes.byref(ks),
                                                     self._prune_rows.data_ptr(), st), "apgp_pack_prune_rows")
+            srows_len = int(lib.apgp_prune_srows_len(n, ks.ndim))
+            self._prune_srows = None
+            if srows_len > 0:
+                self._prune_srows = torch.empty(srows_len, dtype=torch.float64, device=dev)
+                _lib.check(lib.apgp_pack_prune_srows(self._xs.data_ptr(), n, ctypes.byref(ks),
+                                                     self._prune_srows.data_ptr(), st), "apgp_pack_prune_srows")
+
+    def _prune_stream(self):
+        if self.prune_signed and self._prune_srows is not None:
+            return self._prune_srows.data_ptr(), _lib.PRUNE_ROWS_SIGNED
+        return _ptr(self._prune_rows), _lib.PRUNE_ROWS_SPLIT
 
     def predict(self, y, t, return_cov=True, return_var=False, cache=True, **kwargs):
         if (self._computed and not self.kernel.dirty and type(t) is np.ndarray and t.dtype == _F64
@@ -1180,7 +1193,7 @@
                 e0.record()
             args = (self._xs.data_ptr(), n, ctypes.byref(ks), float(self.mean.value), kind_id, lo, hi, _ptr(mask_d),
                     float(zeta), float(np.max(y)), _ptr(mu), _ptr(var), _ptr(u), part.data_ptr(), best.data_ptr(),
-                    _ptr(self._prune_rows), st)
+                    *self._prune_stream(), st)
             prune_was = None if self.sweep_prune is None else lib.apgp_set_sweep_prune(int(self.sweep_prune))
             rowsplit_was = None if self.seed_rowsplit is None else lib.apgp_set_seed_rowsplit(int(self.seed_rowsplit))
             park_was = None if self.seed_park is None else lib.apgp_set_seed_park(int(self.seed_park))
@@ -1188,11 +1201,11 @@
             parts_was = None if self.seed_parts is None else lib.apgp_set_seed_parts(int(self.seed_parts))
             try:
                 if use_solve:
-                    _lib.check(lib.apgp_acquire_solve_rows(T.data_ptr(), m, int(idx_offset),
-                                                           self._packed_solve.data_ptr(), *args), "apgp_acquire_solve_rows")
+                    _lib.check(lib.apgp_acquire_solve_rows2(T.data_ptr(), m, int(idx_offset),
+                                                            self._packed_solve.data_ptr(), *args), "apgp_acquire_solve_rows2")
                 else:
-                    _lib.check(lib.apgp_acquire_rows(T.data_ptr(), m, int(idx_offset), self._packed.data_ptr(), *args),
-                               "apgp_acquire_rows")
+                    _lib.check(lib.apgp_acquire_rows2(T.data_ptr(), m, int(idx_offset), self._packed.data_ptr(), *args),
+                               "apgp_acquire_rows2")
             finally:
                 if prune_was is not None:
                     lib.apgp_set_sweep_prune(prune_was)
@@ -1251,11 +1264,11 @@
         with self._on(torch, dev):
             self._ensure_xs(y)
             bmin = torch.empty((m + 63) // 64, dtype=torch.float64, device=dev)
-            _lib.check(lib.apgp_prune_bounds_rows(T.data_ptr(), m, self._xs.data_ptr(), len(self._x), ctypes.byref(ks),
-                                                  float(self.mean.value), kind_id, lo, hi, _ptr(mask_d), float(zeta),
-                                                  float(np.max(y)), int(bool(coarse)), bmin.data_ptr(),
-                                                  _ptr(self._prune_rows), self._stream(torch)),
-                       "apgp_prune_bounds_rows")
+            _lib.check(lib.apgp_prune_bounds_rows2(T.data_ptr(), m, self._xs.data_ptr(), len(self._x), ctypes.byref(ks),
+                                                   float(self.mean.value), kind_id, lo, hi, _ptr(mask_d), float(zeta),
+                                                   float(np.max(y)), int(bool(coarse)), bmin.data_ptr(),
+                                                   *self._prune_stream(), None, self._stream(torch)),
+                       "apgp_prune_bounds_rows2")
         return bmin.cpu().numpy()
 
     def nelder_mead_search(self, y, starts, kind, bounds=None, zeta=0.01, options=None, trace=False):
diff --git a/include/apgp.h b/include/apgp.h
--- a/include/apgp.h
+++ b/include/apgp.h
@@ -151,6 +151,30 @@
                            const double* lo , const double* hi , const uint8_t* mask,
                            double zeta, double ybest, int coarse, double* bmin_out, const void* prune_rows,
                            void* stream);
+
+#define APGP_PRUNE_ROWS_SPLIT 0
+#define APGP_PRUNE_ROWS_SIGNED 1
+int64_t apgp_prune_srows_len(int64_t n, int32_t ndim);
+int apgp_pack_prune_srows(const double* xs, int64_t n, const apgp_kernel_t* kern , void* rows, void* stream);
+int apgp_acquire_rows2(const double* T, int64_t m, int64_t idx_offset,
+                       const double* packed_linv, const double* xs, int64_t n,
+                       const apgp_kernel_t* kern , double mean, int32_t kind,
+                       const double* lo , const double* hi ,
+                       const uint8_t* mask, double zeta, double ybest,
+                       double* mu, double* var, double* u,
+                       void* part, apgp_best_t* best, const void* prune_rows, int32_t rows_kind, void* stream);
+int apgp_acquire_solve_rows2(const double* T, int64_t m, int64_t idx_offset,
+                             const double* packed_lsolve, const double* xs, int64_t n,
+                             const apgp_kernel_t* kern , double mean, int32_t kind,
+                             const double* lo , const double* hi ,
+                             const uint8_t* mask, double zeta, double ybest,
+                             double* mu, double* var, double* u,
+                             void* part, apgp_best_t* best, const void* prune_rows, int32_t rows_kind, void* stream);
+int apgp_prune_bounds_rows2(const double* T, int64_t m, const double* xs, int64_t n,
+                            const apgp_kernel_t* kern , double mean, int32_t kind,
+                            const double* lo , const double* hi , const uint8_t* mask,
+                            double zeta, double ybest, int coarse, double* bmin_out, const void* prune_rows,
+                            int32_t rows_kind, double* est_out, void* stream);
 
 #define APGP_MAX_FANTASY 32
 int64_t apgp_acquire_fantasy_work_len(int64_t m);
```

After: 924.4 million, median of 6. 6.5% higher.
